# ishine/TTS-3

Measured on AMD Instinct MI355X. Metric: audio samples/sec + RTF, HiFiGAN-v1 22.05kHz 80-mel, batch 32 @ 1/2/4/8 GPU, higher is better.
Workload: dtype fp32 (power-of-2 scaled fp16 hi/lo split on fp16 MFMA, fp32 accumulate); 1 GPU; HiFiGAN-v1 22.05kHz inference, [32,80,1024] mel per GPU (replicate pad 5), fp32; model=HiFiGAN-v1 (hifigan_config.py generator_model_params), global_batch=32, seq_len=1024, parallelism=dp1 (utterance sharding; no collectives)

## Files before the change

### tts-3_amd/csrc/abi.cpp

```cpp
#include <cmath>
#include <cstdio>
#include <cstring>
#include <new>
#include <string>
#include <vector>

#include "fft_attn.hpp"
#include "forward_tts.hpp"
#include "glow.hpp"
#include "handoff.hpp"
#include "hifigan.hpp"
#include "mas.hpp"
#include "melgan.hpp"
#include "stft.hpp"
#include "text.hpp"
#include "vits.hpp"
#include "tts_mi355x.h"

namespace {
thread_local std::string g_last_error;

template <class F>
int guarded(F&& f) {
  try {
    g_last_error.clear();
    f();
    return TTS_OK;
  } catch (const tts::Error& e) {
    g_last_error = e.what();
    return e.code;
  } catch (const std::bad_alloc&) {
    g_last_error = "host allocation failed";
    return TTS_ERR_OOM;
  } catch (const std::exception& e) {
    g_last_error = e.what();
    return TTS_ERR_INVALID;
  } catch (...) {
    g_last_error = "unknown error";
    return TTS_ERR_INVALID;
  }
}

void export_records(const tts::Profiler& prof, TtsLaunchRecord* records, int max_records, int* n_records) {
  *n_records = (int)prof.recs.size();
  for (int i = 0; i < (int)prof.recs.size() && i < max_records && records; ++i) {
    const auto& r = prof.recs[i];
    std::memset(records[i].name, 0, sizeof(records[i].name));
    std::strncpy(records[i].name, r.name.c_str(), sizeof(records[i].name) - 1);
    records[i].flops = r.flops;
    records[i].bytes = r.bytes;
    float ms = 0.f;
    TTS_HIP_CHECK(hipEventElapsedTime(&ms, r.a, r.b));
    records[i].ms = ms;
  }
}

tts::DeviceBuffer to_device(const float* host, size_t n) {
  tts::DeviceBuffer b;
  int dev = 0;
  TTS_HIP_CHECK(hipGetDevice(&dev));
  b.grow(dev, n * sizeof(float), "operand");
  if (host && n) TTS_HIP_CHECK(hipMemcpy(b.as<>(), host, n * sizeof(float), hipMemcpyHostToDevice));
  return b;
}

template <class Cfg, class Validate, class Shapes>
int num_weights(const Cfg* cfg, Validate validate, Shapes shapes) {
  int n = -1;
  int st = guarded([&] {
    TTS_REQUIRE(cfg, 1, "NULL cfg");
    validate(*cfg);
    n = (int)shapes(*cfg).size();
  });
  return st == TTS_OK ? n : -st;
}

template <class Cfg, class Validate, class Shapes>
int64_t weight_numel(const Cfg* cfg, int idx, Validate validate, Shapes shapes) {
  int64_t n = -1;
  guarded([&] {
    TTS_REQUIRE(cfg, 1, "NULL cfg");
    validate(*cfg);
    auto s = shapes(*cfg);
    TTS_REQUIRE(idx >= 0 && idx < (int)s.size(), 1, "weight index out of range");
    n = s[idx];
  });
  return n;
}

template <class T, class Cfg, class W>
int create(const Cfg* cfg, const W* host_weights, int device, void** handle) {
  return guarded([&] {
    TTS_REQUIRE(cfg && host_weights && handle, 1, "NULL argument");
    *handle = nullptr;
    *handle = new T(*cfg, host_weights, device);
  });
}

template <class T>
int destroy(void* handle) {
  return guarded([&] { delete static_cast<T*>(handle); });
}

template <class T, class Body>
int profiled(void* handle, void* hip_stream, TtsLaunchRecord* records, int max_records, int* n_records, Body body) {
  return guarded([&] {
    TTS_REQUIRE(handle && n_records, 1, "NULL argument");
    auto* h = static_cast<T*>(handle);
    auto s = static_cast<hipStream_t>(hip_stream);
    tts::Profiler prof;
    {
      tts::DeviceGuard g(h->device());
      body(*h, s, &prof);
      TTS_HIP_CHECK(hipStreamSynchronize(s));
    }
    export_records(prof, records, max_records, n_records);
  });
}
}

extern "C" {

const char* tts_last_error(void) { return g_last_error.c_str(); }
int tts_abi_version(void) { return 115; }
const char* tts_build_target(void) { return "gfx950"; }

int tts_hifigan_num_weights(const TtsHifiganCfg* cfg) {
  return num_weights(cfg, tts::hifigan_validate, tts::hifigan_weight_shapes);
}

int64_t tts_hifigan_weight_numel(const TtsHifiganCfg* cfg, int idx) {
  return weight_numel(cfg, idx, tts::hifigan_validate, tts::hifigan_weight_shapes);
}

int tts_hifigan_create(const TtsHifiganCfg* cfg, const float* const* host_weights, int device,
                       void** handle) {
  return create<tts::Hifigan>(cfg, host_weights, device, handle);
}

int tts_hifigan_destroy(void* handle) { return destroy<tts::Hifigan>(handle); }

int64_t tts_hifigan_output_length(const void* handle, int T, int pad) {
  if (!handle) return -1;
  return static_cast<const tts::Hifigan*>(handle)->out_len(T, pad);
}

int64_t tts_hifigan_workspace_bytes(const void* handle, int B, int T, int pad) {
  if (!handle) return -1;
  return static_cast<const tts::Hifigan*>(handle)->workspace_bytes(B, T, pad);
}

int tts_hifigan_reserve(void* handle, int B, int T, int pad) {
  return guarded([&] {
    TTS_REQUIRE(handle, 1, "NULL handle");
    TTS_REQUIRE(B >= 1 && T >= 1 && pad >= 0, 1, "bad shape");
    static_cast<tts::Hifigan*>(handle)->reserve(B, T, pad);
  });
}

int tts_hifigan_forward(void* handle, const float* d_mel, int B, int C, int T, int pad,
                        const float* d_g, float* d_wav, void* hip_stream) {
  return guarded([&] {
    TTS_REQUIRE(handle, 1, "NULL handle");
    static_cast<tts::Hifigan*>(handle)->forward(d_mel, B, C, T, pad, d_g, d_wav,
                                                static_cast<hipStream_t>(hip_stream), nullptr);
  });
}

int tts_hifigan_forward_profiled(void* handle, const float* d_mel, int B, int C, int T, int pad,
                                 const float* d_g, float* d_wav, void* hip_stream,
                                 TtsLaunchRecord* records, int max_records, int* n_records) {
  auto body = [&](tts::Hifigan& h, hipStream_t s, tts::Profiler* prof) {
    h.forward(d_mel, B, C, T, pad, d_g, d_wav, s, prof);
  };
  return profiled<tts::Hifigan>(handle, hip_stream, records, max_records, n_records, body);
}

static std::vector<int64_t> glow_encoder_shapes(const TtsGlowEncoderCfg& c) {
  return tts::glow_encoder_weight_shapes(c);
}

int tts_glow_encoder_num_weights(const TtsGlowEncoderCfg* cfg) {
  return num_weights(cfg, tts::glow_encoder_validate, glow_encoder_shapes);
}

int64_t tts_glow_encoder_weight_numel(const TtsGlowEncoderCfg* cfg, int idx) {
  return weight_numel(cfg, idx, tts::glow_encoder_validate, glow_encoder_shapes);
}

int tts_glow_encoder_create(const TtsGlowEncoderCfg* cfg, const float* const* host_weights, int device,
                            void** handle) {
  return create<tts::GlowEncoder>(cfg, host_weights, device, handle);
}

int tts_glow_encoder_destroy(void* handle) { return destroy<tts::GlowEncoder>(handle); }

int tts_glow_encoder_forward(void* handle, const int64_t* d_tokens, const int64_t* d_lengths, const float* d_g,
                             int B, int T, float* d_x_m, float* d_x_logs, float* d_logw, float* d_x_mask,
                             void* hip_stream) {
  return guarded([&] {
    TTS_REQUIRE(handle, 1, "NULL handle");
    static_cast<tts::GlowEncoder*>(handle)->forward(d_tokens, d_lengths, d_g, B, T, d_x_m, d_x_logs, d_logw,
                                                    d_x_mask, static_cast<hipStream_t>(hip_stream));
  });
}

int tts_glow_encoder_forward_profiled(void* handle, const int64_t* d_tokens, const int64_t* d_lengths,
                                      const float* d_g, int B, int T, float* d_x_m, float* d_x_logs, float* d_logw,
                                      float* d_x_mask,
                                      void* hip_stream, TtsLaunchRecord* records, int max_records,
                                      int* n_records) {
  auto body = [&](tts::GlowEncoder& h, hipStream_t s, tts::Profiler* prof) {
    h.forward(d_tokens, d_lengths, d_g, B, T, d_x_m, d_x_logs, d_logw, d_x_mask, s, prof);
  };
  return profiled<tts::GlowEncoder>(handle, hip_stream, records, max_records, n_records, body);
}

int tts_glow_durations(const float* d_logw, const float* d_x_mask, int B, int T_x, float length_scale,
                       float* d_w_ceil, int64_t* d_y_lengths, float* d_o_attn_dur, void* hip_stream) {
  return guarded([&] {
    TTS_REQUIRE(d_logw && d_x_mask && d_w_ceil && d_y_lengths, 1, "NULL argument");
    TTS_REQUIRE(B >= 1 && T_x >= 1, 1, "batch and token count must be >= 1");
    tts::launch_durations(d_logw, d_x_mask, d_w_ceil, d_y_lengths, d_o_attn_dur, B, T_x, length_scale,
                          static_cast<hipStream_t>(hip_stream));
    TTS_HIP_CHECK(hipGetLastError());
  });
}

int tts_glow_expand(const float* d_w_ceil, const float* d_x_mask, const int64_t* d_y_lengths,
                    const float* d_o_mean, const float* d_o_log_scale, const float* d_noise, float noise_scale,
                    int B, int C, int T_x, int T_y, float* d_z, float* d_y_mask, float* d_y_mean,
                    float* d_y_log_scale, float* d_attn, void* hip_stream) {
  return guarded([&] {
    TTS_REQUIRE(d_w_ceil && d_x_mask && d_y_lengths && d_o_mean && d_z && d_y_mask, 1, "NULL argument");
    TTS_REQUIRE(B >= 1 && C >= 1 && T_x >= 1 && T_y >= 1, 1, "bad expand shape");
    tts::ExpandArgs a{};
    a.w_ceil = d_w_ceil; a.x_mask = d_x_mask; a.y_len = d_y_lengths; a.o_mean = d_o_mean;
    a.o_log_scale = d_o_log_scale; a.noise = d_noise; a.noise_scale = noise_scale;
    a.C = C; a.T_x = T_x; a.T_y = T_y;
    a.z = d_z; a.y_mask = d_y_mask; a.y_mean = d_y_mean; a.y_log_scale = d_y_log_scale; a.attn = d_attn;
    tts::launch_expand(a, B, static_cast<hipStream_t>(hip_stream));
    TTS_HIP_CHECK(hipGetLastError());
  });
}

int tts_glow_mas_logp(const float* d_o_mean, const float* d_o_log_scale, const float* d_z, int B, int C, int T_en,
                      int T_de, float* d_logp, void* hip_stream) {
  return guarded([&] {
    TTS_REQUIRE(d_o_mean && d_z && d_logp, 1, "NULL argument");
    TTS_REQUIRE(B >= 1 && C >= 1 && T_en >= 1 && T_de >= 1, 1, "bad logp shape");
    tts::launch_mas_logp(d_o_mean, d_o_log_scale, d_z, B, C, T_en, T_de, d_logp, static_cast<hipStream_t>(hip_stream));
  });
}

int64_t tts_maximum_path_workspace_bytes(int B, int T_en, int T_de) {
  if (B < 1 || T_en < 1 || T_de < 1 || T_en > tts::MAS_MAX_TEN) return -1;
  return (int64_t)tts::mas_workspace_bytes(B, T_en, T_de);
}

int tts_maximum_path(const float* d_value, const float* d_mask, const int64_t* d_t_x, const int64_t* d_t_y, int B,
                     int T_en, int T_de, void* d_workspace, float* d_path, float* d_durations, float* d_log_dur,
                     void* hip_stream) {
  return guarded([&] {
    TTS_REQUIRE(d_value && d_t_x && d_t_y && d_workspace, 1, "NULL argument");
    TTS_REQUIRE(B >= 1 && T_en >= 1 && T_de >= 1, 1, "bad maximum_path shape");
    tts::launch_maximum_path(d_value, d_mask, d_t_x, d_t_y, B, T_en, T_de, d_workspace, d_path, d_durations, d_log_dur,
                             static_cast<hipStream_t>(hip_stream));
  });
}

int tts_vits_text_encoder_num_weights(const TtsVitsTextEncoderCfg* cfg) {
  return num_weights(cfg, tts::vits_text_encoder_validate, tts::vits_text_encoder_weight_shapes);
}

int64_t tts_vits_text_encoder_weight_numel(const TtsVitsTextEncoderCfg* cfg, int idx) {
  return weight_numel(cfg, idx, tts::vits_text_encoder_validate, tts::vits_text_encoder_weight_shapes);
}

int tts_vits_text_encoder_create(const TtsVitsTextEncoderCfg* cfg, const float* const* host_weights, int device,
                                 void** handle) {
  return create<tts::VitsTextEncoder>(cfg, host_weights, device, handle);
}

int tts_vits_text_encoder_destroy(void* handle) { return destroy<tts::VitsTextEncoder>(handle); }

int tts_vits_text_encoder_forward(void* handle, const int64_t* d_tokens, const int64_t* d_lengths,
                                  const float* d_lang_emb, int B, int T, float* d_x, float* d_m, float* d_logs,
                                  float* d_x_mask, void* hip_stream) {
  return guarded([&] {
    TTS_REQUIRE(handle, 1, "NULL handle");
    static_cast<tts::VitsTextEncoder*>(handle)->forward(d_tokens, d_lengths, d_lang_emb, B, T, d_x, d_m, d_logs,
                                                        d_x_mask, static_cast<hipStream_t>(hip_stream));
  });
}

int tts_vits_text_encoder_forward_profiled(void* handle, const int64_t* d_tokens, const int64_t* d_lengths,
                                           const float* d_lang_emb, int B, int T, float* d_x, float* d_m,
                                           float* d_logs, float* d_x_mask, void* hip_stream,
                                           TtsLaunchRecord* records, int max_records, int* n_records) {
  auto body = [&](tts::VitsTextEncoder& h, hipStream_t s, tts::Profiler* prof) {
    h.forward(d_tokens, d_lengths, d_lang_emb, B, T, d_x, d_m, d_logs, d_x_mask, s, prof);
  };
  return profiled<tts::VitsTextEncoder>(handle, hip_stream, records, max_records, n_records, body);
}

int tts_vits_sdp_num_weights(const TtsVitsSdpCfg* cfg) {
  return num_weights(cfg, tts::vits_sdp_validate, tts::vits_sdp_weight_shapes);
}

int64_t tts_vits_sdp_weight_numel(const TtsVitsSdpCfg* cfg, int idx) {
  return weight_numel(cfg, idx, tts::vits_sdp_validate, tts::vits_sdp_weight_shapes);
}

int tts_vits_sdp_create(const TtsVitsSdpCfg* cfg, const float* const* host_weights, int device, void** handle) {
  return create<tts::VitsSdp>(cfg, host_weights, device, handle);
}

int tts_vits_sdp_destroy(void* handle) { return destroy<tts::VitsSdp>(handle); }

int tts_vits_sdp_reverse(void* handle, const float* d_x, const float* d_x_mask, const float* d_g,
                         const float* d_lang_emb, const float* d_noise, float noise_scale, int B, int T,
                         float* d_logw, void* hip_stream) {
  return guarded([&] {
    TTS_REQUIRE(handle, 1, "NULL handle");
    static_cast<tts::VitsSdp*>(handle)->reverse(d_x, d_x_mask, d_g, d_lang_emb, d_noise, noise_scale, B, T, d_logw,
                                                static_cast<hipStream_t>(hip_stream));
  });
}

int tts_vits_sdp_reverse_profiled(void* handle, const float* d_x, const float* d_x_mask, const float* d_g,
                                  const float* d_lang_emb, const float* d_noise, float noise_scale, int B, int T,
                                  float* d_logw, void* hip_stream, TtsLaunchRecord* records, int max_records,
                                  int* n_records) {
  auto body = [&](tts::VitsSdp& h, hipStream_t s, tts::Profiler* prof) {
    h.reverse(d_x, d_x_mask, d_g, d_lang_emb, d_noise, noise_scale, B, T, d_logw, s, prof);
  };
  return profiled<tts::VitsSdp>(handle, hip_stream, records, max_records, n_records, body);
}

int tts_vits_dp_num_weights(const TtsVitsDpCfg* cfg) {
  return num_weights(cfg, tts::vits_dp_validate, tts::vits_dp_weight_shapes);
}

int64_t tts_vits_dp_weight_numel(const TtsVitsDpCfg* cfg, int idx) {
  return weight_numel(cfg, idx, tts::vits_dp_validate, tts::vits_dp_weight_shapes);
}

int tts_vits_dp_create(const TtsVitsDpCfg* cfg, const float* const* host_weights, int device, void** handle) {
  return create<tts::VitsDp>(cfg, host_weights, device, handle);
}

int tts_vits_dp_destroy(void* handle) { return destroy<tts::VitsDp>(handle); }

int tts_vits_dp_forward(void* handle, const float* d_x, const float* d_x_mask, const float* d_g,
                        const float* d_lang_emb, int B, int T, float* d_logw, void* hip_stream) {
  return guarded([&] {
    TTS_REQUIRE(handle, 1, "NULL handle");
    static_cast<tts::VitsDp*>(handle)->forward(d_x, d_x_mask, d_g, d_lang_emb, B, T, d_logw,
                                               static_cast<hipStream_t>(hip_stream));
  });
}

int tts_vits_dp_forward_profiled(void* handle, const float* d_x, const float* d_x_mask, const float* d_g,
                                 const float* d_lang_emb, int B, int T, float* d_logw, void* hip_stream,
                                 TtsLaunchRecord* records, int max_records, int* n_records) {
  auto body = [&](tts::VitsDp& h, hipStream_t s, tts::Profiler* prof) {
    h.forward(d_x, d_x_mask, d_g, d_lang_emb, B, T, d_logw, s, prof);
  };
  return profiled<tts::VitsDp>(handle, hip_stream, records, max_records, n_records, body);
}

int tts_vits_durations(const float* d_logw, const float* d_x_mask, int B, int T_x, float length_scale,
                       float* d_w_ceil, int64_t* d_y_lengths, void* hip_stream) {
  return guarded([&] {
    TTS_REQUIRE(d_logw && d_x_mask && d_w_ceil && d_y_lengths, 1, "NULL argument");
    TTS_REQUIRE(B >= 1 && T_x >= 1, 1, "batch and token count must be >= 1");
    tts::launch_durations(d_logw, d_x_mask, d_w_ceil, d_y_lengths, nullptr, B, T_x, length_scale,
                          static_cast<hipStream_t>(hip_stream), 1);
    TTS_HIP_CHECK(hipGetLastError());
  });
}

int tts_vits_expand(const float* d_w_ceil, const float* d_x_mask, const int64_t* d_y_lengths, const float* d_m_p,
                    const float* d_logs_p, const float* d_noise, float noise_scale, int B, int C, int T_x, int T_y,
                    float* d_z_p, float* d_y_mask, float* d_m_p_out, float* d_logs_p_out, float* d_attn,
                    void* hip_stream) {
  return guarded([&] {
    TTS_REQUIRE(d_w_ceil && d_x_mask && d_y_lengths && d_m_p && d_logs_p && d_z_p && d_y_mask, 1, "NULL argument");
    TTS_REQUIRE(B >= 1 && C >= 1 && T_x >= 1 && T_y >= 1, 1, "bad expand shape");
    tts::ExpandArgs a{};
    a.w_ceil = d_w_ceil; a.x_mask = d_x_mask; a.y_len = d_y_lengths; a.o_mean = d_m_p;
    a.o_log_scale = d_logs_p; a.noise = d_noise; a.noise_scale = noise_scale;
    a.C = C; a.T_x = T_x; a.T_y = T_y;
    a.z = d_z_p; a.y_mask = d_y_mask; a.y_mean = d_m_p_out; a.y_log_scale = d_logs_p_out; a.attn = d_attn;
    a.vits = 1;
    tts::launch_expand(a, B, static_cast<hipStream_t>(hip_stream));
    TTS_HIP_CHECK(hipGetLastError());
  });
}

int tts_vits_durations_given(const float* d_durations, int64_t dur_bstride, int B, int T_x, float* d_w_ceil,
                             int64_t* d_y_lengths, void* hip_stream) {
  return guarded([&] {
    TTS_REQUIRE(d_durations && d_w_ceil && d_y_lengths, 1, "NULL argument");
    TTS_REQUIRE(B >= 1 && T_x >= 1 && (dur_bstride == 0 || dur_bstride >= T_x), 1, "bad durations shape");
    tts::launch_given_durations(d_durations, dur_bstride, d_w_ceil, d_y_lengths, B, T_x,
                                static_cast<hipStream_t>(hip_stream));
  });
}

int tts_vits_mask_slice(const float* d_z, const float* d_y_mask, int B, int C, int T, int T_out, float* d_out,
                        void* hip_stream) {
  return guarded([&] {
    TTS_REQUIRE(d_z && d_y_mask && d_out, 1, "NULL argument");
    tts::launch_mask_slice(d_z, d_y_mask, d_out, B, C, T, T_out, static_cast<hipStream_t>(hip_stream));
  });
}

int tts_vits_upsample_z(const float* d_z, const int64_t* d_y_lengths, int B, int C, int T, double factor, int T2,
                        float* d_z2, float* d_y_mask2, void* hip_stream) {
  return guarded([&] {
    TTS_REQUIRE(d_z && d_z2 && (d_y_lengths || !d_y_mask2), 1, "NULL argument");
    TTS_REQUIRE(factor > 0.0 && T2 == (int)std::floor((double)T * factor), 1,
                "upsample_z: T2 must be floor(T * factor) (F.interpolate's output length)");
    tts::launch_upsample_z(d_z, d_y_lengths, d_z2, d_y_mask2, B, C, T, T2, factor,
                           static_cast<hipStream_t>(hip_stream));
  });
}

int tts_embedding_rows(const float* d_table, int num, int dim, const int64_t* d_ids, int64_t id_stride, int B,
                       float* d_out, void* hip_stream) {
  return guarded([&] {
    TTS_REQUIRE(d_table && d_ids && d_out, 1, "NULL argument");
    tts::launch_embedding_rows(d_table, d_ids, id_stride, d_out, B, dim, num, static_cast<hipStream_t>(hip_stream));
  });
}

int tts_l2_normalize_rows(const float* d_in, int B, int C, float* d_out, void* hip_stream) {
  return guarded([&] {
    TTS_REQUIRE(d_in && d_out, 1, "NULL argument");
    tts::launch_l2_normalize(d_in, d_out, B, C, static_cast<hipStream_t>(hip_stream));
  });
}

namespace {
tts::AudioNormDev to_dev(const TtsAudioNormCfg* c) {
  tts::AudioNormDev d{};
  if (!c || !c->signal_norm) return d;
  TTS_REQUIRE((c->d_mel_mean == nullptr) == (c->d_mel_scale == nullptr), 1,
              "mel_scaler needs both d_mel_mean and d_mel_scale");
  d.signal_norm = 1;
  d.symmetric_norm = c->symmetric_norm;
  d.clip_norm = c->clip_norm;
  d.max_norm = (float)c->max_norm;
  d.two_max_norm = (float)(2.0 * c->max_norm);
  d.min_level_db = (float)c->min_level_db;
  d.neg_min_level_db = (float)(-c->min_level_db);
  d.ref_level_db = (float)c->ref_level_db;
  d.mean = c->d_mel_mean;
  d.scale = c->d_mel_scale;
  return d;
}
}

int tts_mel_handoff(const float* d_in, int B, int T, int C, int time_major, const TtsAudioNormCfg* denorm,
                    const TtsAudioNormCfg* norm, int T_out, float src_scale, float* d_out, void* hip_stream) {
  return guarded([&] {
    TTS_REQUIRE(d_in && d_out, 1, "NULL argument");
    TTS_REQUIRE(B >= 1 && T >= 1 && C >= 1 && T_out >= 1, 1, "bad hand-off shape");
    TTS_REQUIRE(C <= 65535 && B <= 65535, 3, "hand-off: C and B must be <= 65535");
    tts::HandoffArgs a{};
    a.in = d_in; a.out = d_out; a.T = T; a.C = C; a.T_out = T_out; a.time_major = time_major ? 1 : 0;
    a.src_scale = src_scale;
    a.de = to_dev(denorm);
    a.no = to_dev(norm);
    tts::launch_handoff(a, B, static_cast<hipStream_t>(hip_stream));
    TTS_HIP_CHECK(hipGetLastError());
  });
}

int tts_wav_to_int16(const float* d_wav, int B, int64_t n, const int64_t* d_lengths, unsigned* d_scratch,
                     int16_t* d_out, void* hip_stream) {
  return guarded([&] {
    TTS_REQUIRE(d_wav && d_scratch && d_out, 1, "NULL argument");
    TTS_REQUIRE(B >= 1 && B <= 65535 && n >= 1, 1, "bad wav shape");
    tts::launch_wav_int16(d_wav, B, n, d_lengths, d_scratch, d_out, static_cast<hipStream_t>(hip_stream));
    TTS_HIP_CHECK(hipGetLastError());
  });
}

int tts_glow_decoder_num_weights(const TtsGlowDecoderCfg* cfg) {
  return num_weights(cfg, tts::glow_validate, tts::glow_weight_shapes);
}

int64_t tts_glow_decoder_weight_numel(const TtsGlowDecoderCfg* cfg, int idx) {
  return weight_numel(cfg, idx, tts::glow_validate, tts::glow_weight_shapes);
}

int tts_glow_decoder_create(const TtsGlowDecoderCfg* cfg, const float* const* host_weights,
                            int device, void** handle) {
  return create<tts::GlowDecoder>(cfg, host_weights, device, handle);
}

int tts_glow_decoder_destroy(void* handle) { return destroy<tts::GlowDecoder>(handle); }

int tts_glow_decoder_forward(void* handle, const float* d_x, const float* d_mask, const float* d_g, int B,
                             int C, int T, int reverse, float* d_y, float* d_logdet, void* hip_stream) {
  return guarded([&] {
    TTS_REQUIRE(handle, 1, "NULL handle");
    TTS_REQUIRE(reverse == 0 || reverse == 1, 1, "reverse must be 0 or 1");
    auto* h = static_cast<tts::GlowDecoder*>(handle);
    if (reverse) h->reverse(d_x, d_mask, d_g, B, C, T, d_y, static_cast<hipStream_t>(hip_stream));
    else h->forward(d_x, d_mask, d_g, B, C, T, d_y, d_logdet, static_cast<hipStream_t>(hip_stream));
  });
}

int tts_glow_decoder_forward_profiled(void* handle, const float* d_x, const float* d_mask, const float* d_g,
                                      int B, int C, int T, int reverse, float* d_y, float* d_logdet,
                                      void* hip_stream, TtsLaunchRecord* records, int max_records, int* n_records) {
  auto body = [&](tts::GlowDecoder& h, hipStream_t s, tts::Profiler* prof) {
    TTS_REQUIRE(reverse == 0 || reverse == 1, 1, "reverse must be 0 or 1");
    if (reverse) h.reverse(d_x, d_mask, d_g, B, C, T, d_y, s, prof);
    else h.forward(d_x, d_mask, d_g, B, C, T, d_y, d_logdet, s, prof);
  };
  return profiled<tts::GlowDecoder>(handle, hip_stream, records, max_records, n_records, body);
}

int tts_vits_flow_num_weights(const TtsVitsFlowCfg* cfg) {
  return num_weights(cfg, tts::vits_flow_validate, tts::vits_flow_weight_shapes);
}

int64_t tts_vits_flow_weight_numel(const TtsVitsFlowCfg* cfg, int idx) {
  return weight_numel(cfg, idx, tts::vits_flow_validate, tts::vits_flow_weight_shapes);
}

int tts_vits_flow_create(const TtsVitsFlowCfg* cfg, const float* const* host_weights, int device, void** handle) {
  return create<tts::VitsFlow>(cfg, host_weights, device, handle);
}

int tts_vits_flow_destroy(void* handle) { return destroy<tts::VitsFlow>(handle); }

int tts_vits_flow_forward(void* handle, const float* d_x, const float* d_mask, const float* d_g, int B, int C,
                          int T, int reverse, float* d_y, void* hip_stream) {
  return guarded([&] {
    TTS_REQUIRE(handle, 1, "NULL handle");
    TTS_REQUIRE(reverse == 0 || reverse == 1, 1, "reverse must be 0 or 1");
    auto* h = static_cast<tts::VitsFlow*>(handle);
    if (reverse) h->reverse(d_x, d_mask, d_g, B, C, T, d_y, static_cast<hipStream_t>(hip_stream));
    else h->forward(d_x, d_mask, d_g, B, C, T, d_y, static_cast<hipStream_t>(hip_stream));
  });
}

int tts_vits_flow_forward_profiled(void* handle, const float* d_x, const float* d_mask, const float* d_g, int B,
                                   int C, int T, int reverse, float* d_y, void* hip_stream,
                                   TtsLaunchRecord* records, int max_records, int* n_records) {
  auto body = [&](tts::VitsFlow& h, hipStream_t s, tts::Profiler* prof) {
    TTS_REQUIRE(reverse == 0 || reverse == 1, 1, "reverse must be 0 or 1");
    if (reverse) h.reverse(d_x, d_mask, d_g, B, C, T, d_y, s, prof);
    else h.forward(d_x, d_mask, d_g, B, C, T, d_y, s, prof);
  };
  return profiled<tts::VitsFlow>(handle, hip_stream, records, max_records, n_records, body);
}

int tts_vits_posterior_num_weights(const TtsVitsPosteriorCfg* cfg) {
  return num_weights(cfg, tts::vits_posterior_validate, tts::vits_posterior_weight_shapes);
}

int64_t tts_vits_posterior_weight_numel(const TtsVitsPosteriorCfg* cfg, int idx) {
  return weight_numel(cfg, idx, tts::vits_posterior_validate, tts::vits_posterior_weight_shapes);
}

int tts_vits_posterior_create(const TtsVitsPosteriorCfg* cfg, const float* const* host_weights, int device,
                              void** handle) {
  return create<tts::VitsPosterior>(cfg, host_weights, device, handle);
}

int tts_vits_posterior_destroy(void* handle) { return destroy<tts::VitsPosterior>(handle); }

int tts_vits_posterior_forward(void* handle, const float* d_x, const float* d_mask, const float* d_g,
                               const float* d_eps, int B, int C, int T, float* d_z, float* d_m, float* d_logs,
                               void* hip_stream) {
  return guarded([&] {
    TTS_REQUIRE(handle, 1, "NULL handle");
    static_cast<tts::VitsPosterior*>(handle)->forward(d_x, d_mask, d_g, d_eps, B, C, T, d_z, d_m, d_logs,
                                                      static_cast<hipStream_t>(hip_stream));
  });
}

int tts_vits_posterior_forward_profiled(void* handle, const float* d_x, const float* d_mask, const float* d_g,
                                        const float* d_eps, int B, int C, int T, float* d_z, float* d_m,
                                        float* d_logs, void* hip_stream, TtsLaunchRecord* records,
                                        int max_records, int* n_records) {
  auto body = [&](tts::VitsPosterior& h, hipStream_t s, tts::Profiler* prof) {
    h.forward(d_x, d_mask, d_g, d_eps, B, C, T, d_z, d_m, d_logs, s, prof);
  };
  return profiled<tts::VitsPosterior>(handle, hip_stream, records, max_records, n_records, body);
}

int tts_stft_create(const TtsStftCfg* cfg, const float* h_window, int device, void** handle) {
  return create<tts::Stft>(cfg, h_window, device, handle);
}

int tts_stft_destroy(void* handle) { return destroy<tts::Stft>(handle); }

int tts_stft_num_frames(const TtsStftCfg* cfg, int64_t N) {
  int n = -1;
  int st = guarded([&] {
    TTS_REQUIRE(cfg, 1, "NULL cfg");
    n = tts::stft_num_frames(*cfg, N);
  });
  return st == TTS_OK ? n : -st;
}

int tts_stft_forward(void* handle, const float* d_wav, int B, int64_t N, int64_t wav_bstride, float* d_spec,
                     void* hip_stream) {
  return guarded([&] {
    TTS_REQUIRE(handle, 1, "NULL handle");
    static_cast<tts::Stft*>(handle)->forward(d_wav, B, N, wav_bstride, d_spec, static_cast<hipStream_t>(hip_stream));
  });
}

int tts_stft_forward_profiled(void* handle, const float* d_wav, int B, int64_t N, int64_t wav_bstride,
                              float* d_spec, void* hip_stream, TtsLaunchRecord* records, int max_records,
                              int* n_records) {
  auto body = [&](tts::Stft& h, hipStream_t s, tts::Profiler* prof) {
    h.forward(d_wav, B, N, wav_bstride, d_spec, s, prof);
  };
  return profiled<tts::Stft>(handle, hip_stream, records, max_records, n_records, body);
}

static void op_conv1d_impl(const TtsConv1dDesc* d, const float* d_x, const float* h_w, const float* h_b,
                           const float* d_res, float* d_y, float* d_z, int tile, int reps, float* ms,
                           void* hip_stream) {
  TTS_REQUIRE(d && d_x && h_w && h_b, 1, "NULL argument");
  TTS_REQUIRE(d->B >= 1 && d->Cin >= 1 && d->Cout >= 1 && d->Tin >= 1 && d->K >= 1 && d->dil >= 1, 1,
              "bad conv1d shape");
  TTS_REQUIRE((d->K % 2) == 1, 3, "conv1d: only odd kernel sizes ('same' padding)");
  TTS_REQUIRE(d->zmode >= 0 && d->zmode <= 3, 1, "bad zmode");
  TTS_REQUIRE(d->zmode == 0 ? d_y != nullptr : d_z != nullptr, 1, "missing output pointer");
  const int mode = d->math_mode;
  TTS_REQUIRE(mode >= tts::MATH_FP32 && mode <= tts::MATH_LAST, 1, "unknown math_mode");
  if (tile < 0) tile = tts::conv_tile_for(mode, d->Cout, d->K, d->Cin, d->dil, d_res != nullptr);
  const tts::ConvTile t = tts::conv_tile(mode, tile);
  std::vector<float> packed(tts::packed_conv_numel(mode, d->Cout, d->Cin, d->K, t));
  const int w_exp = tts::pack_conv(mode, h_w, d->Cout, d->Cin, d->K, t, packed.data());
  std::vector<float> bias((size_t)tts::ceil_div(d->Cout, t.BM) * t.BM, 0.f);
  std::memcpy(bias.data(), h_b, sizeof(float) * d->Cout);
  const tts::DeviceBuffer w = to_device(packed.data(), packed.size()), b = to_device(bias.data(), bias.size());
  tts::Conv1dArgs a{};
  a.x = d_x; a.w = w.as<>(); a.bias = b.as<>(); a.res = d_res; a.y = d_y; a.z = d_z; a.cvec = nullptr;
  a.Cin = d->Cin; a.Cout = d->Cout; a.Tin = d->Tin; a.Tout = d->Tin + 2 * d->rep_pad;
  a.dil = d->dil; a.pad = d->dil * (d->K - 1) / 2; a.rep_pad = d->rep_pad;
  a.n_chunks = tts::ceil_div(d->Cin, t.CK);
  a.in_slope = d->in_slope; a.out_slope = d->out_slope; a.zmode = d->zmode; a.zdiv = d->zdiv;
  a.w_exp = w_exp;
  auto s = static_cast<hipStream_t>(hip_stream);
  tts::DeviceBuffer slots;
  if (mode == tts::MATH_FP32_F16X3) {
    slots = to_device(nullptr, (size_t)d->B * 64);
    TTS_HIP_CHECK(hipMemsetAsync(slots.as<>(), 0, (size_t)d->B * 64 * sizeof(float), s));
    tts::launch_amax(d_x, (int64_t)d->Cin * d->Tin, d->B, slots.as<unsigned>(), s);
    a.amax_in = slots.as<unsigned>();
  }
  if (reps <= 0) {
    tts::launch_conv(mode, a, d->B, d->K, tile, s);
  } else {
    tts::launch_conv(mode, a, d->B, d->K, tile, s);
    hipEvent_t e0, e1;
    TTS_HIP_CHECK(hipEventCreate(&e0));
    TTS_HIP_CHECK(hipEventCreate(&e1));
    TTS_HIP_CHECK(hipEventRecord(e0, s));
    for (int r = 0; r < reps; ++r) tts::launch_conv(mode, a, d->B, d->K, tile, s);
    TTS_HIP_CHECK(hipEventRecord(e1, s));
    TTS_HIP_CHECK(hipEventSynchronize(e1));
    float total = 0.f;
    TTS_HIP_CHECK(hipEventElapsedTime(&total, e0, e1));
    (void)hipEventDestroy(e0);
    (void)hipEventDestroy(e1);
    if (ms) *ms = total / reps;
  }
  TTS_HIP_CHECK(hipStreamSynchronize(s));
}

int tts_op_conv1d(const TtsConv1dDesc* d, const float* d_x, const float* h_w, const float* h_b,
                  const float* d_res, float* d_y, float* d_z, void* hip_stream) {
  return guarded([&] { op_conv1d_impl(d, d_x, h_w, h_b, d_res, d_y, d_z, -1, 0, nullptr, hip_stream); });
}

int tts_op_conv1d_bench(const TtsConv1dDesc* d, const float* d_x, const float* h_w, const float* h_b,
                        const float* d_res, float* d_y, float* d_z, int tile, int reps, float* ms,
                        void* hip_stream) {
  return guarded([&] { op_conv1d_impl(d, d_x, h_w, h_b, d_res, d_y, d_z, tile, reps, ms, hip_stream); });
}

int tts_op_conv1d_num_tiles(int math_mode) {
  if (math_mode < tts::MATH_FP32 || math_mode > tts::MATH_LAST) {
    g_last_error = "unknown math_mode";
    return -TTS_ERR_INVALID;
  }
  return tts::conv_num_tiles(math_mode);
}

int tts_op_conv_transpose1d(const float* d_x, int B, int Cin, int Tin, const float* h_w,
                            const float* h_b, int Cout, int K, int stride, float in_slope,
                            int math_mode, float* d_y, void* hip_stream) {
  return guarded([&] {
    TTS_REQUIRE(d_x && h_w && h_b && d_y, 1, "NULL argument");
    TTS_REQUIRE(B >= 1 && Cin >= 1 && Cout >= 1 && Tin >= 1, 1, "bad conv_transpose1d shape");
    TTS_REQUIRE(K == 2 * stride, 3, "conv_transpose1d: requires kernel_size == 2*stride");
    TTS_REQUIRE(stride == 2 || stride == 4 || stride == 8, 3, "conv_transpose1d: stride must be 2, 4 or 8");
    TTS_REQUIRE(math_mode >= tts::MATH_FP32 && math_mode <= tts::MATH_LAST, 1, "unknown math_mode");
    auto s = static_cast<hipStream_t>(hip_stream);
    if (tts::is_split_mode(math_mode)) {
      const int tile = tts::conv_tile_for(math_mode, stride * Cout, 2, Cin, 1, false);
      const tts::ConvTile t = tts::conv_tile(math_mode, tile);
      std::vector<float> packed(tts::packed_conv_numel(math_mode, stride * Cout, Cin, 2, t));
      const int w_exp = tts::pack_convT_split(math_mode, h_w, Cin, Cout, stride, t, packed.data());
      std::vector<float> bias((size_t)tts::ceil_div(stride * Cout, t.BM) * t.BM, 0.f);
      for (int co = 0; co < Cout; ++co)
        for (int ph = 0; ph < stride; ++ph) bias[(size_t)co * stride + ph] = h_b[co];
      const tts::DeviceBuffer w = to_device(packed.data(), packed.size()), b = to_device(bias.data(), bias.size());
      tts::Conv1dArgs a{};
      a.x = d_x; a.w = w.as<>(); a.bias = b.as<>(); a.y = d_y;
      a.Cin = Cin; a.Cout = stride * Cout; a.Tin = Tin; a.Tout = Tin + 1;
      a.dil = 1; a.pad = 1; a.n_chunks = tts::ceil_div(Cin, t.CK);
      a.in_slope = in_slope; a.out_slope = 1.f; a.zdiv = 1.f; a.w_exp = w_exp; a.ups = stride;
      tts::DeviceBuffer slots;
      if (math_mode == tts::MATH_FP32_F16X3) {
        slots = to_device(nullptr, (size_t)B * 64);
        TTS_HIP_CHECK(hipMemsetAsync(slots.as<>(), 0, (size_t)B * 64 * sizeof(float), s));
        tts::launch_amax(d_x, (int64_t)Cin * Tin, B, slots.as<unsigned>(), s);
        a.amax_in = slots.as<unsigned>();
      }
      tts::launch_conv(math_mode, a, B, 2, tile, s);
      TTS_HIP_CHECK(hipStreamSynchronize(s));
      return;
    }
    const int tile = tts::convT_tile_for(Cout, stride);
    const tts::ConvTile t = tts::convT_tile(tile, stride);
    std::vector<float> packed(tts::packed_convT_numel(Cin, Cout, stride, t));
    tts::pack_convT(h_w, Cin, Cout, stride, t, packed.data());
    std::vector<float> bias((size_t)tts::ceil_div(Cout, t.BM) * t.BM, 0.f);
    std::memcpy(bias.data(), h_b, sizeof(float) * Cout);
    const tts::DeviceBuffer w = to_device(packed.data(), packed.size()), b = to_device(bias.data(), bias.size());
    tts::ConvTArgs a{};
    a.x = d_x; a.w = w.as<>(); a.bias = b.as<>(); a.y = d_y;
    a.Cin = Cin; a.Cout = Cout; a.Tin = Tin; a.n_chunks = tts::ceil_div(Cin, t.CK); a.in_slope = in_slope;
    tts::launch_convT(a, B, stride, tile, s);
    TTS_HIP_CHECK(hipStreamSynchronize(s));
  });
}

int tts_op_conv_post(const float* d_z, int B, int Cin, int T, const float* h_w, const float* h_b,
                     float in_slope, float* d_y, void* hip_stream) {
  return guarded([&] {
    TTS_REQUIRE(d_z && h_w && d_y, 1, "NULL argument");
    TTS_REQUIRE(B >= 1 && Cin >= 1 && T >= 1, 1, "bad conv_post shape");
    const tts::DeviceBuffer w = to_device(h_w, (size_t)Cin * 7);
    tts::PostArgs a{};
    a.z = d_z; a.w = w.as<>(); a.bias = h_b ? h_b[0] : 0.f; a.y = d_y; a.Cin = Cin; a.T = T; a.in_slope = in_slope;
    auto s = static_cast<hipStream_t>(hip_stream);
    tts::launch_conv_post(a, B, s);
    TTS_HIP_CHECK(hipStreamSynchronize(s));
  });
}

int tts_melgan_num_weights(const TtsMelganCfg* cfg) {
  return num_weights(cfg, [](const TtsMelganCfg&) {}, tts::melgan_weight_shapes);
}

int64_t tts_melgan_weight_numel(const TtsMelganCfg* cfg, int idx) {
  return weight_numel(cfg, idx, [](const TtsMelganCfg&) {}, tts::melgan_weight_shapes);
}

int tts_melgan_create(const TtsMelganCfg* cfg, const float* const* host_weights, int device, void** handle) {
  return create<tts::Melgan>(cfg, host_weights, device, handle);
}

int tts_melgan_destroy(void* handle) { return destroy<tts::Melgan>(handle); }

int64_t tts_melgan_output_length(const void* handle, int T, int pad, int synth) {
  int64_t n = -1;
  int st = guarded([&] {
    TTS_REQUIRE(handle, 1, "NULL handle");
    n = static_cast<const tts::Melgan*>(handle)->out_len(T, pad, synth);
  });
  return st == TTS_OK ? n : -st;
}

int64_t tts_melgan_workspace_bytes(const void* handle, int B, int T, int pad) {
  int64_t n = -1;
  int st = guarded([&] {
    TTS_REQUIRE(handle, 1, "NULL handle");
    n = static_cast<const tts::Melgan*>(handle)->workspace_bytes(B, T, pad);
  });
  return st == TTS_OK ? n : -st;
}

int tts_melgan_forward(void* handle, const float* d_mel, int B, int C, int T, int pad, int synth, float* d_out,
                       void* hip_stream) {
  return guarded([&] {
    TTS_REQUIRE(handle, 1, "NULL handle");
    static_cast<tts::Melgan*>(handle)->forward(d_mel, B, C, T, pad, synth, d_out, static_cast<hipStream_t>(hip_stream));
  });
}

int tts_melgan_forward_profiled(void* handle, const float* d_mel, int B, int C, int T, int pad, int synth,
                                float* d_out, void* hip_stream, TtsLaunchRecord* records, int max_records,
                                int* n_records) {
  auto body = [&](tts::Melgan& h, hipStream_t s, tts::Profiler* prof) {
    h.forward(d_mel, B, C, T, pad, synth, d_out, s, prof);
  };
  return profiled<tts::Melgan>(handle, hip_stream, records, max_records, n_records, body);
}

int tts_op_melgan_block(const float* d_x, int B, int C, int L, int dilation, const float* h_w1, const float* h_b1,
                        const float* h_w2, const float* h_b2, const float* h_ws, const float* h_bs, int math_mode,
                        float* d_out, void* hip_stream) {
  return guarded([&] {
    TTS_REQUIRE(d_x && h_w1 && h_b1 && h_w2 && h_b2 && h_ws && h_bs && d_out, 1, "NULL argument");
    TTS_REQUIRE(math_mode >= tts::MATH_FP32 && math_mode <= tts::MATH_LAST, 1, "unknown math_mode");
    TTS_REQUIRE(B >= 1 && C >= 1 && L >= 1 && dilation >= 1, 1, "bad melgan block shape");
    const int mode = math_mode == tts::MATH_BF16 ? tts::MATH_BF16 : tts::MATH_FP32_X6;
    TTS_REQUIRE(C <= tts::kMelganMaxC, 3, "melgan block: channels must lie in [1, 256]");
    const int64_t n1 = tts::packed_melgan_a1_numel16(mode, C), n2 = tts::packed_melgan_a2_numel16(mode, C);
    const size_t nb = (size_t)32 * tts::melgan_mblocks(C);
    std::vector<float> a1((size_t)n1 / 2), a2((size_t)n2 / 2), bias1(nb), bias2(nb);
    tts::pack_melgan_block(mode, h_w1, h_b1, h_w2, h_b2, h_ws, h_bs, C, reinterpret_cast<uint16_t*>(a1.data()),
                           reinterpret_cast<uint16_t*>(a2.data()), bias1.data(), bias2.data());
    const tts::DeviceBuffer da1 = to_device(a1.data(), a1.size()), da2 = to_device(a2.data(), a2.size());
    const tts::DeviceBuffer db1 = to_device(bias1.data(), nb), db2 = to_device(bias2.data(), nb);
    tts::MelganBlockArgs a{};
    a.x = d_x; a.y = d_out; a.a1 = da1.as<>(); a.a2 = da2.as<>(); a.bias1 = db1.as<>(); a.bias2 = db2.as<>();
    a.a1_bytes = (unsigned)(n1 * 2); a.a2_bytes = (unsigned)(n2 * 2);
    a.C = C; a.L = L; a.dil = dilation;
    auto s = static_cast<hipStream_t>(hip_stream);
    tts::launch_melgan_block(mode, a, B, s);
    TTS_HIP_CHECK(hipStreamSynchronize(s));
  });
}

int tts_op_melgan_block_tile(void) { return tts::kMelganBlockTile; }

int tts_pqmf_synthesis(const float* d_x, int B, int bands, int L, const float* d_G, int taps, float* d_out,
                       void* hip_stream) {
  return guarded([&] {
    tts::launch_pqmf_synthesis(d_x, B, bands, L, d_G, taps, d_out, static_cast<hipStream_t>(hip_stream));
  });
}

int tts_op_mha(const float* d_qkv, const int64_t* d_key_lengths, int B, int E, int heads, int T, int math_mode,
               float* d_out, void* hip_stream) {
  return guarded([&] {
    TTS_REQUIRE(d_qkv && d_out, 1, "NULL argument");
    TTS_REQUIRE(math_mode >= tts::MATH_FP32 && math_mode <= tts::MATH_LAST, 1, "unknown math_mode");
    const int mode = math_mode == tts::MATH_BF16 ? tts::MATH_BF16 : tts::MATH_FP32_X6;
    tts::launch_mha(mode, d_qkv, d_key_lengths, d_out, B, E, heads, T, static_cast<hipStream_t>(hip_stream));
  });
}

int tts_op_mha_tile(void) { return tts::kMhaTile; }

int tts_forward_tts_num_weights(const TtsForwardTtsCfg* cfg) {
  return num_weights(cfg, tts::forward_tts_validate, tts::forward_tts_weight_shapes);
}

int64_t tts_forward_tts_weight_numel(const TtsForwardTtsCfg* cfg, int idx) {
  return weight_numel(cfg, idx, tts::forward_tts_validate, tts::forward_tts_weight_shapes);
}

int tts_forward_tts_create(const TtsForwardTtsCfg* cfg, const float* const* host_weights, int device, void** handle) {
  return create<tts::ForwardTts>(cfg, host_weights, device, handle);
}

int tts_forward_tts_destroy(void* handle) { return destroy<tts::ForwardTts>(handle); }

int tts_forward_tts_encode(void* handle, const int64_t* d_tokens, const int64_t* d_x_lengths,
                           const int64_t* d_speaker_ids, const float* d_given_durations, int B, int T_en,
                           float length_scale, float* d_o_en, float* d_x_mask, float* d_durations_log, float* d_pitch,
                           float* d_durations, int64_t* d_y_lengths, void* hip_stream) {
  return guarded([&] {
    TTS_REQUIRE(handle, 1, "NULL handle");
    static_cast<tts::ForwardTts*>(handle)->encode(d_tokens, d_x_lengths, d_speaker_ids, d_given_durations, B, T_en,
                                                  length_scale, d_o_en, d_x_mask, d_durations_log, d_pitch,
                                                  d_durations, d_y_lengths, static_cast<hipStream_t>(hip_stream));
  });
}

int tts_forward_tts_encode_profiled(void* handle, const int64_t* d_tokens, const int64_t* d_x_lengths,
                                    const int64_t* d_speaker_ids, const float* d_given_durations, int B, int T_en,
                                    float length_scale, float* d_o_en, float* d_x_mask, float* d_durations_log,
                                    float* d_pitch, float* d_durations, int64_t* d_y_lengths, void* hip_stream,
                                    TtsLaunchRecord* records, int max_records, int* n_records) {
  auto body = [&](tts::ForwardTts& h, hipStream_t s, tts::Profiler* prof) {
    h.encode(d_tokens, d_x_lengths, d_speaker_ids, d_given_durations, B, T_en, length_scale, d_o_en, d_x_mask,
             d_durations_log, d_pitch, d_durations, d_y_lengths, s, prof);
  };
  return profiled<tts::ForwardTts>(handle, hip_stream, records, max_records, n_records, body);
}

int tts_forward_tts_decode(void* handle, const float* d_o_en, const float* d_durations, const float* d_x_mask,
                           const int64_t* d_y_lengths, int B, int T_en, int T_de, int mask_decoder_keys, float* d_out,
                           float* d_attn, float* d_y_mask, void* hip_stream) {
  return guarded([&] {
    TTS_REQUIRE(handle, 1, "NULL handle");
    static_cast<tts::ForwardTts*>(handle)->decode(d_o_en, d_durations, d_x_mask, d_y_lengths, B, T_en, T_de,
                                                  mask_decoder_keys != 0, d_out, d_attn, d_y_mask,
                                                  static_cast<hipStream_t>(hip_stream));
  });
}

int tts_forward_tts_decode_profiled(void* handle, const float* d_o_en, const float* d_durations, const float* d_x_mask,
                                    const int64_t* d_y_lengths, int B, int T_en, int T_de, int mask_decoder_keys,
                                    float* d_out, float* d_attn, float* d_y_mask, void* hip_stream,
                                    TtsLaunchRecord* records, int max_records, int* n_records) {
  auto body = [&](tts::ForwardTts& h, hipStream_t s, tts::Profiler* prof) {
    h.decode(d_o_en, d_durations, d_x_mask, d_y_lengths, B, T_en, T_de, mask_decoder_keys != 0, d_out, d_attn,
             d_y_mask, s, prof);
  };
  return profiled<tts::ForwardTts>(handle, hip_stream, records, max_records, n_records, body);
}

int tts_forward_tts_block(void* handle, int decoder, const float* d_x, const int64_t* d_key_lengths, int B, int T,
                          float* d_y, void* hip_stream) {
  return guarded([&] {
    TTS_REQUIRE(handle, 1, "NULL handle");
    static_cast<tts::ForwardTts*>(handle)->block(decoder != 0, d_x, d_key_lengths, B, T, d_y,
                                                 static_cast<hipStream_t>(hip_stream));
  });
}

}
```

### tts-3_amd/csrc/common.hpp

```cpp
#pragma once

#include <hip/hip_runtime.h>

#include <cstdint>
#include <stdexcept>
#include <string>

namespace tts {

struct Error : std::runtime_error {
  int code;
  Error(int c, const std::string& m) : std::runtime_error(m), code(c) {}
};

#define TTS_HIP_CHECK(expr)                                                               \
  do {                                                                                    \
    hipError_t _e = (expr);                                                               \
    if (_e != hipSuccess)                                                                 \
      throw ::tts::Error(2, std::string(#expr) + " failed: " + hipGetErrorString(_e));    \
  } while (0)

#define TTS_REQUIRE(cond, code, msg)                    \
  do {                                                  \
    if (!(cond)) throw ::tts::Error((code), (msg));     \
  } while (0)

typedef float f32x4 __attribute__((ext_vector_type(4)));
typedef float f32x16 __attribute__((ext_vector_type(16)));

__device__ __forceinline__ float lrelu(float x, float slope) { return x > 0.f ? x : x * slope; }

constexpr int kPlaneXB16 = 1;
constexpr int kPlaneYB16 = 2;

struct Conv1dArgs {
  const float* x;
  const float* w;
  const float* bias;
  const float* res;
  float* y;
  float* z;
  const float* cvec;
  const float* mask;
  int64_t x_bstride;
  int Cin, Cout, Tin, Tout;
  int dil, pad, rep_pad;
  int n_chunks;
  float in_slope, out_slope;
  int zmode;
  float zdiv;
  const unsigned* amax_in;
  unsigned* amax_out;
  int w_exp;
  int ups;
  int64_t o_bstride;
  int64_t cvec_bstride;
  int mask_res;
  int wn_rows;
  int gate;
  int planes;
};

constexpr int kSplitGateTile = 20;
constexpr int kSplitWinoTile = 21;
bool wino_supported(int mode, int Cout, int Cin, int K, int dil);
bool wino_enabled();
void launch_wino(int mode, const Conv1dArgs& a, int B, int K, hipStream_t s);
inline int gate_row_order(int rho, int H) {
  const int j = rho / 128, r = rho % 128;
  return r < 64 ? 64 * j + r : H + 64 * j + (r - 64);
}

struct ResPairArgs {
  Conv1dArgs c1;
  Conv1dArgs c2;
  const float* post_w;
  float post_bias;
  float post_slope;
  float* wav;
};
bool resblock_pair_supported(int mode, int C, int K, int dil);
bool resblock_pair_preferred(int mode, int C, int K, int dil);
bool resblock_pair128(int mode, int C, int K);
void launch_resblock_pair(int mode, const ResPairArgs& a, int B, int K, int C, hipStream_t s);

struct ResBlock3Args {
  const float* x;
  const unsigned* amax_in;
  const float* w[6];
  const float* bias[6];
  int w_exp[6];
  int dil[3];
  float* z;
  int zmode;
  float zdiv;
  unsigned* amax_out;
  int T;
  int planes;
};
bool resblock3_supported(int mode, int C, int K, const int* dil);
void launch_resblock3(int mode, const ResBlock3Args& a, int B, int C, int K, hipStream_t s);
bool resblock2_supported(int mode, int C, int K, const int* dil);
bool resblock2_preferred(int mode, int C, int K, const int* dil);
int resblock2_geo64(int mode);
void launch_resblock2(int mode, const ResBlock3Args& a, int B, int C, int K, int geo64, hipStream_t s);

struct ConvTile {
  int BM, BN, TM, TN, CK;
  int PD = 1;
  int WINO = 0;
};

struct ConvTArgs {
  const float* x;
  const float* w;
  const float* bias;
  float* y;
  int Cin, Cout, Tin;
  int n_chunks;
  float in_slope;
  unsigned* amax_out;
  const float* cvec;
};

struct PostArgs {
  const float* z;
  const float* w;
  float bias;
  float* y;
  int Cin, T;
  float in_slope;
  int z_b16;
};

int conv1d_tile_for(int Cout, int K, int Cin, int dil, bool res);
ConvTile conv1d_tile(int idx);
int conv1d_num_tiles();
void launch_conv1d(const Conv1dArgs& a, int B, int K, int tile_idx, hipStream_t s);
int convT_tile_for(int Cout, int U);
ConvTile convT_tile(int idx, int U);
void launch_convT(const ConvTArgs& a, int B, int U, int tile_idx, hipStream_t s);
void launch_conv_post(const PostArgs& a, int B, hipStream_t s);
void launch_mel_window(const float* mel, int B, int C, int T, int pad, int64_t w0, int W, float* out, hipStream_t s);
void launch_cond_vec(const float* g, const float* Wc, const float* bc, float* cvec, int B, int Cc,
                     int C0, hipStream_t s);

constexpr int MATH_FP32 = 0;
constexpr int MATH_FP32_X6 = 1;
constexpr int MATH_FP32_F16X3 = 2;
constexpr int MATH_BF16 = 3;
constexpr int MATH_LAST = MATH_BF16;

ConvTile conv1d_split_tile(int mode, int idx);
int conv1d_split_num_tiles(int mode);
int conv1d_split_tile_for(int mode, int Cout, int K, int Cin, int dil, bool res);
void launch_conv1d_split(int mode, const Conv1dArgs& a, int B, int K, int tile_idx, hipStream_t s);
bool convT_res_supported(int mode, const Conv1dArgs& a);
void launch_convT_res(int mode, const Conv1dArgs& a, int B, hipStream_t s);
void launch_amax(const float* x, int64_t n, int B, unsigned* slots, hipStream_t s, int64_t stride = 0);

inline bool is_split_mode(int mode) { return mode == MATH_FP32_X6 || mode == MATH_FP32_F16X3 || mode == MATH_BF16; }
inline ConvTile conv_tile(int mode, int idx) {
  return is_split_mode(mode) ? conv1d_split_tile(mode, idx) : conv1d_tile(idx);
}
inline int conv_tile_for(int mode, int Cout, int K, int Cin, int dil, bool res) {
  return is_split_mode(mode) ? conv1d_split_tile_for(mode, Cout, K, Cin, dil, res)
                             : conv1d_tile_for(Cout, K, Cin, dil, res);
}
inline int conv_num_tiles(int mode) { return is_split_mode(mode) ? conv1d_split_num_tiles(mode) : conv1d_num_tiles(); }
inline void launch_conv(int mode, const Conv1dArgs& a, int B, int K, int tile, hipStream_t s) {
  if (is_split_mode(mode)) launch_conv1d_split(mode, a, B, K, tile, s);
  else launch_conv1d(a, B, K, tile, s);
}

void pack_conv1d(const float* w, int Cout, int Cin, int K, const ConvTile& t, float* out);
int64_t packed_conv1d_numel(int Cout, int Cin, int K, const ConvTile& t);
void pack_convT(const float* w, int Cin, int Cout, int U, const ConvTile& t, float* out);
int64_t packed_convT_numel(int Cin, int Cout, int U, const ConvTile& t);
__host__ __device__ constexpr int quad_pos(int q) { return q == 1 ? 2 : (q == 2 ? 1 : q); }
int pack_conv1d_split(int mode, const float* w, int Cout, int Cin, int K, const ConvTile& t, float* out,
                      bool quad_perm = true);
int64_t packed_conv1d_split_numel(int mode, int Cout, int Cin, int K, const ConvTile& t);
int pack_convT_split(int mode, const float* w, int Cin, int Cout, int U, const ConvTile& t, float* out);
int pack_conv1d_wino(int mode, const float* w, int Cout, int Cin, int K, const ConvTile& t, float* out);
inline int64_t packed_conv_numel(int mode, int Cout, int Cin, int K, const ConvTile& t) {
  if (t.WINO) return packed_conv1d_split_numel(mode, Cout, Cin, 7 * ((K + 3) / 4), t);
  return is_split_mode(mode) ? packed_conv1d_split_numel(mode, Cout, Cin, K, t) : packed_conv1d_numel(Cout, Cin, K, t);
}
inline int pack_conv(int mode, const float* w, int Cout, int Cin, int K, const ConvTile& t, float* out) {
  if (t.WINO) return pack_conv1d_wino(mode, w, Cout, Cin, K, t, out);
  if (is_split_mode(mode)) return pack_conv1d_split(mode, w, Cout, Cin, K, t, out);
  pack_conv1d(w, Cout, Cin, K, t, out);
  return 0;
}

inline int ceil_div(int a, int b) { return (a + b - 1) / b; }

}
```

### tts-3_amd/csrc/conv_device.hpp

```cpp
#pragma once

#include "common.hpp"

namespace tts {

typedef __amdgpu_buffer_rsrc_t rsrc_t;
typedef unsigned u32x4_t __attribute__((ext_vector_type(4)));
typedef unsigned u32x2_t __attribute__((ext_vector_type(2)));
typedef float f32x2 __attribute__((ext_vector_type(2)));
constexpr unsigned OOB_OFF = 0x80000000u;

#ifndef ACT_ABLATE
#define ACT_ABLATE 0
#endif
__device__ __forceinline__ unsigned act_range(unsigned bytes) {
  return (ACT_ABLATE && bytes != 0xFFFFFFFFu && bytes > 65536u) ? 65536u : bytes;
}
__device__ __forceinline__ rsrc_t make_rsrc(const void* p, unsigned bytes) {
  return __builtin_amdgcn_make_buffer_rsrc(const_cast<void*>(p), (short)0, (int)act_range(bytes), 0x00020000);
}
__device__ __forceinline__ float bload(rsrc_t r, unsigned voff, unsigned soff) {
  return __builtin_bit_cast(float, __builtin_amdgcn_raw_buffer_load_b32(r, (int)voff, (int)soff, 0));
}
__device__ __forceinline__ f32x4 bload4(rsrc_t r, unsigned voff, unsigned soff) {
  return __builtin_bit_cast(f32x4, __builtin_amdgcn_raw_buffer_load_b128(r, (int)voff, (int)soff, 0));
}
#ifndef TTS_ST_POL
#define TTS_ST_POL 0
#endif
#ifndef TTS_LDX_POL
#define TTS_LDX_POL 0
#endif
template <int POL = TTS_LDX_POL>
__device__ __forceinline__ float bload_x(rsrc_t r, unsigned voff, unsigned soff) {
  return __builtin_bit_cast(float, __builtin_amdgcn_raw_buffer_load_b32(r, (int)voff, (int)soff, POL));
}
__device__ __forceinline__ void bstore(rsrc_t r, float v, unsigned voff, unsigned soff) {
  __builtin_amdgcn_raw_buffer_store_b32(__builtin_bit_cast(unsigned, v), r, (int)voff, (int)soff, TTS_ST_POL);
}
__device__ __forceinline__ unsigned short f32_to_bf16_bits(float v) {
  return __builtin_bit_cast(unsigned short, (__bf16)v);
}
__device__ __forceinline__ float bf16_bits_to_f32(unsigned b) { return __builtin_bit_cast(float, b << 16); }
__device__ __forceinline__ float bf16_round(float v) { return bf16_bits_to_f32(f32_to_bf16_bits(v)); }
template <bool B16>
struct PlaneT {
  static constexpr unsigned ES = 4u;
  __device__ static __forceinline__ float ld(rsrc_t r, unsigned voff, unsigned soff) { return bload(r, voff, soff); }
  __device__ static __forceinline__ void st(rsrc_t r, float v, unsigned voff, unsigned soff) { bstore(r, v, voff, soff); }
  __device__ static __forceinline__ float rt(float v) { return v; }
};
template <>
struct PlaneT<true> {
  static constexpr unsigned ES = 2u;
  __device__ static __forceinline__ float ld(rsrc_t r, unsigned voff, unsigned soff) {
    return bf16_bits_to_f32((unsigned)__builtin_amdgcn_raw_buffer_load_b16(r, (int)voff, (int)soff, 0));
  }
  __device__ static __forceinline__ void st(rsrc_t r, float v, unsigned voff, unsigned soff) {
    __builtin_amdgcn_raw_buffer_store_b16(f32_to_bf16_bits(v), r, (int)voff, (int)soff, TTS_ST_POL);
  }
  __device__ static __forceinline__ float rt(float v) { return bf16_round(v); }
};
template <bool B16>
__device__ __forceinline__ const void* plane_at(const float* p, size_t e) {
  return reinterpret_cast<const char*>(p) + e * PlaneT<B16>::ES;
}
template <bool B16>
__device__ __forceinline__ f32x4 pload4(rsrc_t r, unsigned voff, unsigned soff) {
  if constexpr (B16) {
    const u32x2_t w = __builtin_bit_cast(u32x2_t, __builtin_amdgcn_raw_buffer_load_b64(r, (int)voff, (int)soff, 0));
    return f32x4{bf16_bits_to_f32(w[0] & 0xffffu), bf16_bits_to_f32(w[0] >> 16), bf16_bits_to_f32(w[1] & 0xffffu),
                 bf16_bits_to_f32(w[1] >> 16)};
  } else {
    return bload4(r, voff, soff);
  }
}
template <bool B16>
__device__ __forceinline__ void pstore4(rsrc_t r, f32x4 v, unsigned voff, unsigned soff) {
  if constexpr (B16) {
    const u32x2_t w = {(unsigned)f32_to_bf16_bits(v[0]) | ((unsigned)f32_to_bf16_bits(v[1]) << 16),
                       (unsigned)f32_to_bf16_bits(v[2]) | ((unsigned)f32_to_bf16_bits(v[3]) << 16)};
    __builtin_amdgcn_raw_buffer_store_b64(__builtin_bit_cast(u32x2_t, w), r, (int)voff, (int)soff, TTS_ST_POL);
  } else {
    __builtin_amdgcn_raw_buffer_store_b128(__builtin_bit_cast(u32x4_t, v), r, (int)voff, (int)soff, TTS_ST_POL);
  }
}

__device__ __forceinline__ void lds_dma_b128(const void* base, unsigned bytes, unsigned voff, const void* lds) {
  const unsigned long long p = reinterpret_cast<unsigned long long>(base);
  const u32x4_t d = {(unsigned)__builtin_amdgcn_readfirstlane((int)(unsigned)p),
                     (unsigned)__builtin_amdgcn_readfirstlane((int)((unsigned)(p >> 32) & 0xffffu)),
                     (unsigned)__builtin_amdgcn_readfirstlane((int)act_range(bytes)), 0x00020000u};
  const unsigned m =
      (unsigned)__builtin_amdgcn_readfirstlane((int)(unsigned)(unsigned long)(__attribute__((address_space(3))) const void*)lds);
#pragma clang diagnostic push
#pragma clang diagnostic ignored "-Winline-asm"
  asm volatile("s_mov_b32 m0, %2\n\ts_nop 0\n\tbuffer_load_dwordx4 %0, %1, 0 offen lds" ::"v"(voff), "s"(d), "s"(m)
               : "memory", "m0");
#pragma clang diagnostic pop
}

__device__ __forceinline__ void l2_touch_dma(const void* base, unsigned bytes, unsigned voff, const void* lds) {
  const unsigned long long p = reinterpret_cast<unsigned long long>(base);
  const u32x4_t d = {(unsigned)__builtin_amdgcn_readfirstlane((int)(unsigned)p),
                     (unsigned)__builtin_amdgcn_readfirstlane((int)((unsigned)(p >> 32) & 0xffffu)),
                     (unsigned)__builtin_amdgcn_readfirstlane((int)act_range(bytes)), 0x00020000u};
  const unsigned m =
      (unsigned)__builtin_amdgcn_readfirstlane((int)(unsigned)(unsigned long)(__attribute__((address_space(3))) const void*)lds);
#pragma clang diagnostic push
#pragma clang diagnostic ignored "-Winline-asm"
  asm volatile("s_mov_b32 m0, %2\n\ts_nop 0\n\tbuffer_load_dword %0, %1, 0 offen lds" ::"v"(voff), "s"(d), "s"(m)
               : "memory", "m0");
#pragma clang diagnostic pop
}

__device__ __forceinline__ float lrelu2(float x, float slope) { return fmaxf(x, x * slope); }
__device__ __forceinline__ int wave_id() { return __builtin_amdgcn_readfirstlane((int)(threadIdx.x >> 6)); }

__device__ __forceinline__ int xlds_off(int g, int r, int q, int xrows) {
  return (g * xrows + r) * 8 + 4 * (q ^ ((r >> 3) & 1));
}

template <int CTRL, int ROWS>
__device__ __forceinline__ float dpp_max_step(float v) {
  const int o = __builtin_amdgcn_update_dpp(__builtin_bit_cast(int, v), __builtin_bit_cast(int, v), CTRL, ROWS, 0xF, false);
  return fmaxf(v, __builtin_bit_cast(float, o));
}
__device__ __forceinline__ float wave_max(float v) {
  v = dpp_max_step<0xB1, 0xF>(v);
  v = dpp_max_step<0x4E, 0xF>(v);
  v = dpp_max_step<0x141, 0xF>(v);
  v = dpp_max_step<0x140, 0xF>(v);
  v = dpp_max_step<0x142, 0xA>(v);
  v = dpp_max_step<0x143, 0xC>(v);
  return __builtin_bit_cast(float, __builtin_amdgcn_readlane(__builtin_bit_cast(int, v), 63));
}

__device__ __forceinline__ void publish_amax(unsigned* slots, int b, float v) {
  v = wave_max(v);
  if ((threadIdx.x & 63) == 0) atomicMax(slots + (size_t)b * 64 + (blockIdx.x & 63), __float_as_uint(v));
}

__device__ __forceinline__ void publish_amax_block(unsigned* slots, int b, float v) {
  __shared__ float red[4];
  v = wave_max(v);
  if ((threadIdx.x & 63) == 0) red[threadIdx.x >> 6] = v;
  __syncthreads();
  if (threadIdx.x == 0)
    atomicMax(slots + (size_t)b * 64 + (blockIdx.x & 63),
              __float_as_uint(fmaxf(fmaxf(red[0], red[1]), fmaxf(red[2], red[3]))));
}

template <int TM, int TN, bool RES, int ZM, bool AMAX, bool YB = false>
__device__ __forceinline__ void conv_epilogue_impl(const Conv1dArgs& a, const f32x16 (&acc)[TM][TN], int b,
                                                   int tbase, int cobase, int lane, int tend,
                                                   const float* sbias, int sbase) {
  using PY = PlaneT<YB>;
  const int half = lane >> 5;
  const int l32 = lane & 31;
  const int Cout = a.Cout;
  const int Tout = a.Tout;
  const unsigned plane = (unsigned)Cout * (unsigned)Tout * PY::ES;
  const size_t item = (size_t)b * (a.o_bstride ? a.o_bstride : (int64_t)Cout * Tout);
  const rsrc_t rres = make_rsrc(RES ? plane_at<YB>(a.res, item) : a.bias, RES ? plane : 0u);
  const rsrc_t rz = make_rsrc(ZM >= 2 ? plane_at<YB>(a.z, item) : a.bias, ZM >= 2 ? plane : 0u);
  const rsrc_t rout = make_rsrc(plane_at<YB>(a.zmode == 0 ? a.y : a.z, item), plane);
  const rsrc_t rcv = make_rsrc(a.cvec ? a.cvec + (size_t)b * (a.cvec_bstride ? a.cvec_bstride : (int64_t)Cout) : a.bias,
                               a.cvec ? (unsigned)Cout * 4u : 0u);
  const rsrc_t rmask = make_rsrc(a.mask ? a.mask + (size_t)b * Tout : a.bias, a.mask ? (unsigned)Tout * 4u : 0u);
  const rsrc_t rbias = make_rsrc(a.bias, (unsigned)Cout * 4u);
  const bool has_mask = a.mask != nullptr;
  const bool mask_res = RES && a.mask_res && has_mask;
  const float oslope = a.out_slope;
  const float zdiv = a.zdiv;
  const unsigned rowb = (unsigned)Tout * PY::ES;
  float vmax = 0.f;
#pragma unroll
  for (int m = 0; m < TM; ++m) {
    float bv[16];
#pragma unroll
    for (int r = 0; r < 16; ++r) {
      const unsigned co = (unsigned)(cobase + m * 32 + (r & 3) + 8 * (r >> 2) + 4 * half);
      bv[r] = sbias ? sbias[(int)co - sbase] : bload(rbias, co * 4u, 0u) + bload(rcv, co * 4u, 0u);
    }
#pragma unroll
    for (int n = 0; n < TN; ++n) {
      const int t = tbase + n * 32 + l32;
      const int row0 = cobase + m * 32 + 4 * half;
      const bool tok = t < Tout && t < tend;
      const unsigned voff = tok ? ((unsigned)row0 * (unsigned)Tout + (unsigned)t) * PY::ES : OOB_OFF;
      const float mv = has_mask ? bload(rmask, (tok ? (unsigned)t * 4u : OOB_OFF), 0u) : 1.f;
      const float mv2 = mask_res ? mv : 1.f;
      unsigned vo[16];
      float rv[16], zv[16];
#pragma unroll
      for (int r = 0; r < 16; ++r) {
        vo[r] = voff + (unsigned)((r & 3) + 8 * (r >> 2)) * rowb;
        if (RES) rv[r] = PY::ld(rres, vo[r], 0u);
        if (ZM >= 2) zv[r] = PY::ld(rz, vo[r], 0u);
      }
      float vm = 0.f;
#pragma unroll
      for (int r = 0; r < 16; ++r) {
        float v = (acc[m][n][r] + bv[r]) * mv;
        v = lrelu2(v, oslope);
        if (RES) v = (v + rv[r]) * mv2;
        if (ZM == 2) v = zv[r] + v;
        if (ZM == 3) v = (zv[r] + v) / zdiv;
        if (AMAX) vm = fmaxf(vm, fabsf(v));
        PY::st(rout, v, vo[r], 0u);
      }
      if (AMAX && tok) vmax = fmaxf(vmax, vm);
    }
  }
  if (AMAX && a.amax_out) publish_amax(a.amax_out, b, vmax);
}

template <int TM, int TN, bool AMAX>
__device__ __forceinline__ void conv_epilogue_wn(const Conv1dArgs& args, const f32x16 (&acc)[TM][TN], int b,
                                                 int tbase, int cobase, int lane, const float* sbias, int sbase) {
  const Conv1dArgs a = args;
  const int half = lane >> 5;
  const int l32 = lane & 31;
  const int H = a.wn_rows;
  const int T = a.Tout;
  const size_t item = (size_t)b * H * T;
  const unsigned plane = (unsigned)H * (unsigned)T * 4u;
  const rsrc_t rh = make_rsrc(a.y + item, plane);
  const rsrc_t rsk = make_rsrc(a.z + item, plane);
  const rsrc_t rmask = make_rsrc(a.mask + (size_t)b * T, (unsigned)T * 4u);
  const rsrc_t rbias = make_rsrc(a.bias, (unsigned)(2 * H) * 4u);
  const bool first = a.zmode == 1;
  const unsigned rowb = (unsigned)T * 4u;
  float vmax = 0.f;
#pragma unroll
  for (int m = 0; m < TM; ++m) {
    const int rb0 = cobase + m * 32;
    if (rb0 >= 2 * H) continue;
    const bool hrow = rb0 < H;
    float bv[16];
#pragma unroll
    for (int r = 0; r < 16; ++r) {
      const unsigned co = (unsigned)(rb0 + (r & 3) + 8 * (r >> 2) + 4 * half);
      bv[r] = sbias ? sbias[(int)co - sbase] : bload(rbias, co * 4u, 0u);
    }
    const rsrc_t rdst = hrow ? rh : rsk;
    const int prow0 = (hrow ? rb0 : rb0 - H) + 4 * half;
#pragma unroll
    for (int n = 0; n < TN; ++n) {
      const int t = tbase + n * 32 + l32;
      const bool tok = t < T;
      const unsigned voff = tok ? ((unsigned)prow0 * (unsigned)T + (unsigned)t) * 4u : OOB_OFF;
      const float mv = bload(rmask, tok ? (unsigned)t * 4u : OOB_OFF, 0u);
      float ov[16];
#pragma unroll
      for (int r = 0; r < 16; ++r)
        ov[r] = (hrow || !first) ? bload(rdst, voff + (unsigned)((r & 3) + 8 * (r >> 2)) * rowb, 0u) : 0.f;
      float vm = 0.f;
#pragma unroll
      for (int r = 0; r < 16; ++r) {
        const float v = acc[m][n][r] + bv[r];
        float o;
        if (hrow) {
          o = (ov[r] + v) * mv;
          vm = fmaxf(vm, fabsf(o));
        } else {
          o = first ? v : ov[r] + v;
        }
        bstore(rdst, o, voff + (unsigned)((r & 3) + 8 * (r >> 2)) * rowb, 0u);
      }
      if (AMAX && tok) vmax = fmaxf(vmax, vm);
    }
  }
  if (AMAX && a.amax_out) publish_amax(a.amax_out, b, vmax);
}

template <int TM, int TN, bool AMAX, bool YB = false>
__device__ __forceinline__ void convT_epilogue(const Conv1dArgs& a, const f32x16 (&acc)[TM][TN], int b, int tbase,
                                               int cobase, int lane, const float* sb = nullptr,
                                               const float* scv = nullptr, int sbase = 0) {
  using PY = PlaneT<YB>;
  const int half = lane >> 5;
  const int l32 = lane & 31;
  const int U = a.ups;
  const int lgU = __builtin_ctz(U);
  const int Cr = a.Cout >> lgU;
  const int Tin = a.Tin;
  const int To = Tin << lgU;
  const unsigned plane = (unsigned)Cr * (unsigned)To * PY::ES;
  const rsrc_t rout = make_rsrc(plane_at<YB>(a.y, (size_t)b * Cr * To), plane);
  const rsrc_t rbias = make_rsrc(a.bias, (unsigned)a.Cout * 4u);
  const rsrc_t rcv = make_rsrc(a.cvec ? a.cvec + (size_t)b * Cr : a.bias, a.cvec ? (unsigned)Cr * 4u : 0u);
  float vmax = 0.f;
#pragma unroll
  for (int m = 0; m < TM; ++m) {
    float bv[16], cv[16];
#pragma unroll
    for (int r = 0; r < 16; ++r) {
      const unsigned rho = (unsigned)(cobase + m * 32 + (r & 3) + 8 * (r >> 2) + 4 * half);
      bv[r] = sb ? sb[(int)rho - sbase] : bload(rbias, rho * 4u, 0u);
      cv[r] = sb ? scv[(int)rho - sbase] : bload(rcv, (rho >> lgU) * 4u, 0u);
    }
#pragma unroll
    for (int n = 0; n < TN; ++n) {
      const int mm = tbase + n * 32 + l32;
      if (U == 8) {
#pragma unroll
        for (int i = 0; i < 4; ++i) {
          const int rho = cobase + m * 32 + 8 * i + 4 * half;
          const int co = rho >> 3;
          const int t0 = (mm << 3) + 4 * half - 4;
          const unsigned off = (t0 >= 0 && t0 < To) ? ((unsigned)co * (unsigned)To + (unsigned)t0) * PY::ES : OOB_OFF;
          f32x4 v;
#pragma unroll
          for (int j = 0; j < 4; ++j) {
            v[j] = (acc[m][n][4 * i + j] + bv[4 * i + j]) + cv[4 * i + j];
            if (AMAX && off != OOB_OFF && co < Cr) vmax = fmaxf(vmax, fabsf(v[j]));
          }
          pstore4<YB>(rout, v, off, 0u);
        }
        continue;
      }
      if (U == 2) {
#pragma unroll
        for (int r = 0; r < 16; r += 2) {
          const int rho = cobase + m * 32 + (r & 3) + 8 * (r >> 2) + 4 * half;
          const int co = rho >> 1;
          const int t = 2 * mm - 1;
          const float v0 = (acc[m][n][r] + bv[r]) + cv[r];
          const float v1 = (acc[m][n][r + 1] + bv[r + 1]) + cv[r + 1];
          const unsigned rowoff = (unsigned)co * (unsigned)To;
          if (!YB && t >= 0 && t + 1 < To) {
            if (AMAX && co < Cr) vmax = fmaxf(vmax, fmaxf(fabsf(v0), fabsf(v1)));
            const f32x2 v = {v0, v1};
            __builtin_amdgcn_raw_buffer_store_b64(__builtin_bit_cast(u32x2_t, v), rout, (int)((rowoff + (unsigned)t) * 4u), 0, TTS_ST_POL);
          } else {
            const unsigned off0 = (t >= 0 && t < To) ? (rowoff + (unsigned)t) * PY::ES : OOB_OFF;
            const unsigned off1 = (t + 1 >= 0 && t + 1 < To) ? (rowoff + (unsigned)t + 1u) * PY::ES : OOB_OFF;
            if (AMAX && co < Cr) {
              if (off0 != OOB_OFF) vmax = fmaxf(vmax, fabsf(v0));
              if (off1 != OOB_OFF) vmax = fmaxf(vmax, fabsf(v1));
            }
            PY::st(rout, v0, off0, 0u);
            PY::st(rout, v1, off1, 0u);
          }
        }
        continue;
      }
#pragma unroll
      for (int r = 0; r < 16; ++r) {
        const int rho = cobase + m * 32 + (r & 3) + 8 * (r >> 2) + 4 * half;
        const int co = rho >> lgU;
        const int t = (mm << lgU) + (rho & (U - 1)) - (U >> 1);
        const unsigned off = (t >= 0 && t < To) ? ((unsigned)co * (unsigned)To + (unsigned)t) * PY::ES : OOB_OFF;
        const float v = (acc[m][n][r] + bv[r]) + cv[r];
        if (AMAX && off != OOB_OFF && co < Cr) vmax = fmaxf(vmax, fabsf(v));
        PY::st(rout, v, off, 0u);
      }
    }
  }
  if (AMAX && a.amax_out) publish_amax(a.amax_out, b, vmax);
}

template <int TM, int TN, bool AMAX = false, bool YB = false>
__device__ __forceinline__ void conv_epilogue(const Conv1dArgs& args, const f32x16 (&acc)[TM][TN], int b,
                                              int tbase, int cobase, int lane, int tend = 0x7fffffff,
                                              const float* sbias = nullptr, int sbase = 0) {
  const Conv1dArgs a = args;
  const int zm = a.zmode <= 1 ? 0 : a.zmode;
#define TTS_EPI(RES, ZM) conv_epilogue_impl<TM, TN, RES, ZM, AMAX, YB>(a, acc, b, tbase, cobase, lane, tend, sbias, sbase)
  if (a.res) {
    if (zm == 0) TTS_EPI(true, 0);
    else if (zm == 2) TTS_EPI(true, 2);
    else TTS_EPI(true, 3);
  } else {
    if (zm == 0) TTS_EPI(false, 0);
    else if (zm == 2) TTS_EPI(false, 2);
    else TTS_EPI(false, 3);
  }
#undef TTS_EPI
}

}
```

### tts-3_amd/csrc/hifigan.cpp

```cpp
#include "hifigan.hpp"

#include <algorithm>
#include <cmath>
#include <cstdlib>
#include <vector>

namespace tts {

namespace {
bool valid_conv_k(int k) { return k == 1 || k == 3 || k == 5 || k == 7 || k == 11; }
}

std::vector<int64_t> hifigan_weight_shapes(const TtsHifiganCfg& c) {
  std::vector<int64_t> n;
  const int C0 = c.upsample_initial_channel;
  n.push_back((int64_t)C0 * c.in_channels * 7);
  n.push_back(C0);
  for (int i = 0; i < c.num_upsamples; ++i) {
    const int ci = C0 >> i, co = C0 >> (i + 1);
    n.push_back((int64_t)ci * co * c.upsample_kernel_sizes[i]);
    n.push_back(co);
  }
  for (int i = 0; i < c.num_upsamples; ++i) {
    const int ch = C0 >> (i + 1);
    for (int j = 0; j < c.num_kernels; ++j) {
      const int k = c.resblock_kernel_sizes[j];
      const int nconv = (c.resblock_type == 1) ? 6 : 2;
      for (int m = 0; m < nconv; ++m) {
        n.push_back((int64_t)ch * ch * k);
        n.push_back(ch);
      }
    }
  }
  const int cl = C0 >> c.num_upsamples;
  n.push_back((int64_t)c.out_channels * cl * 7);
  if (c.conv_post_bias) n.push_back(c.out_channels);
  if (c.cond_channels > 0) {
    n.push_back((int64_t)C0 * c.cond_channels);
    n.push_back(C0);
  }
  if (c.cond_in_each_up_layer) {
    for (int i = 0; i < c.num_upsamples; ++i) {
      n.push_back((int64_t)(C0 >> (i + 1)) * c.cond_channels);
      n.push_back(C0 >> (i + 1));
    }
  }
  return n;
}

void hifigan_validate(const TtsHifiganCfg& c) {
  TTS_REQUIRE(c.in_channels >= 1, 1, "in_channels must be >= 1");
  TTS_REQUIRE(c.out_channels == 1, 3, "only out_channels == 1 is implemented");
  TTS_REQUIRE(c.resblock_type == 1 || c.resblock_type == 2, 1, "resblock_type must be '1' or '2'");
  TTS_REQUIRE(c.num_kernels >= 1 && c.num_kernels <= TTS_MAX_KERNELS, 1, "bad num_kernels");
  TTS_REQUIRE(c.num_upsamples >= 1 && c.num_upsamples <= TTS_MAX_UPSAMPLES, 1, "bad num_upsamples");
  const int need_d = c.resblock_type == 1 ? 3 : 2;
  TTS_REQUIRE(c.num_dilations >= need_d && c.num_dilations <= TTS_MAX_DILATIONS, 1,
              "resblock_dilation_sizes too short for the resblock type");
  for (int j = 0; j < c.num_kernels; ++j) {
    TTS_REQUIRE(valid_conv_k(c.resblock_kernel_sizes[j]), 3,
                "resblock kernel size " + std::to_string(c.resblock_kernel_sizes[j]) +
                    " not implemented (1,3,5,7,11)");
    for (int m = 0; m < need_d; ++m) {
      const int d = c.resblock_dilation_sizes[j][m];
      TTS_REQUIRE(d >= 1 && (c.resblock_kernel_sizes[j] - 1) * d <= 96, 3,
                  "resblock (kernel_size-1)*dilation must be <= 96");
    }
  }
  int C = c.upsample_initial_channel;
  for (int i = 0; i < c.num_upsamples; ++i) {
    const int u = c.upsample_factors[i];
    TTS_REQUIRE(u == 2 || u == 4 || u == 8, 3, "upsample factor must be 2, 4 or 8");
    TTS_REQUIRE(c.upsample_kernel_sizes[i] == 2 * u, 3,
                "upsample kernel size must equal 2*factor (polyphase kernel)");
    C >>= 1;
    TTS_REQUIRE(C >= 1, 1, "upsample_initial_channel too small for the number of upsamples");
  }
  TTS_REQUIRE(c.inference_padding >= 0, 1, "inference_padding must be >= 0");
  TTS_REQUIRE(c.cond_channels >= 0, 1, "cond_channels must be >= 0");
  TTS_REQUIRE(!c.cond_in_each_up_layer || c.cond_channels > 0, 1, "cond_in_each_up_layer needs cond_channels > 0");
  TTS_REQUIRE(c.math_mode >= MATH_FP32 && c.math_mode <= MATH_LAST, 1, "unknown math_mode");
}

Hifigan::Hifigan(const TtsHifiganCfg& cfg, const float* const* hw, int device)
    : cfg_(cfg), device_(device) {
  hifigan_validate(cfg_);
  DeviceGuard g(device_);
  const auto shapes = hifigan_weight_shapes(cfg_);
  for (size_t i = 0; i < shapes.size(); ++i)
    TTS_REQUIRE(hw[i] != nullptr, 1, "weight pointer " + std::to_string(i) + " is NULL");

  const int C0 = cfg_.upsample_initial_channel;
  const int mode = cfg_.math_mode;
  const char* nf = std::getenv("TTS_MI355X_NO_PAIR_FUSION");
  const bool pair_fusion = !(nf && nf[0] == '1');
  const char* pf = std::getenv("TTS_MI355X_POST_FUSION");
  post_fusion_ = !(pf && pf[0] == '0');
  const char* ms = std::getenv("TTS_MI355X_MRF_STREAMS");
  nbs_ = ms ? std::max(1, std::min(std::atoi(ms), cfg.num_kernels)) : cfg.num_kernels;
  nbs_env_ = ms != nullptr;
  const char* sb = std::getenv("TTS_MI355X_SUBBATCH");
  n_lanes_ = sb ? std::max(1, std::min(std::atoi(sb), 8)) : 2;
  rb2_geo64_ = resblock2_geo64(mode);
  const char* bp = std::getenv("TTS_MI355X_BF16_PLANES");
  planes16_ = mode == MATH_BF16 && !(bp && bp[0] == '0') && cfg_.num_upsamples >= 1 &&
              cfg_.upsample_factors[0] % 8 == 0;
  size_t wi = 0;
  std::vector<std::pair<const float*, const float*>> src;
  auto add_conv = [&](int Cin, int Cout, int K, int dil, const char* fam, bool res, int lmode, bool pair128 = false) {
    ConvLayer L;
    L.Cin = Cin; L.Cout = Cout; L.K = K; L.dil = dil; L.pad = dil * (K - 1) / 2;
    L.mode = lmode;
    L.tile = conv_tile_for(lmode, Cout, K, Cin, dil, res);
    if (pair128) {
      L.tile = 7;
      L.name = std::string(fam) + "_k" + std::to_string(K) + "_c" + std::to_string(Cout);
      return L;
    }
    const bool wino_k3 = [] {
      const char* e = std::getenv("TTS_MI355X_WINO_K3");
      return e && e[0] == '1';
    }();
    const bool k_ok = K >= 7 || (K == 3 && Cout >= 256 && wino_k3);
    if (std::string(fam) == "mrf_conv" && k_ok && wino_enabled() && wino_supported(lmode, Cout, Cin, K, dil)) {
      L.tile = kSplitWinoTile;
      fam = "mrf_wino";
    }
    L.name = std::string(fam) + "_k" + std::to_string(K) + "_c" + std::to_string(Cout);
    return L;
  };

  pre_ = add_conv(cfg_.in_channels, C0, 7, 1, "conv_pre", false, mode);
  src.push_back({hw[wi], hw[wi + 1]}); wi += 2;
  for (int i = 0; i < cfg_.num_upsamples; ++i) {
    ConvTLayer L;
    L.Cin = C0 >> i; L.Cout = C0 >> (i + 1); L.U = cfg_.upsample_factors[i];
    L.mode = mode;
    L.tile = is_split_mode(mode) ? conv_tile_for(mode, L.U * L.Cout, 2, L.Cin, 1, false) : convT_tile_for(L.Cout, L.U);
    L.name = "ups_u" + std::to_string(L.U) + "_c" + std::to_string(L.Cout);
    ups_.push_back(L);
  }
  std::vector<std::pair<const float*, const float*>> usrc;
  for (int i = 0; i < cfg_.num_upsamples; ++i) { usrc.push_back({hw[wi], hw[wi + 1]}); wi += 2; }

  for (int i = 0; i < cfg_.num_upsamples; ++i) {
    const int ch = C0 >> (i + 1);
    for (int j = 0; j < cfg_.num_kernels; ++j) {
      const int k = cfg_.resblock_kernel_sizes[j];
      ResBlock rb;
      if (cfg_.resblock_type == 1) {
        const float* w1[3]; const float* b1[3]; const float* w2[3]; const float* b2[3];
        for (int m = 0; m < 3; ++m) { w1[m] = hw[wi]; b1[m] = hw[wi + 1]; wi += 2; }
        for (int m = 0; m < 3; ++m) { w2[m] = hw[wi]; b2[m] = hw[wi + 1]; wi += 2; }
        rb.fused = pair_fusion;
        const bool p128 = pair_fusion && resblock_pair128(mode, ch, k);
        bool tiles_ok = true;
        for (int m = 0; m < 3; ++m) {
          rb.convs.push_back(add_conv(ch, ch, k, cfg_.resblock_dilation_sizes[j][m], "mrf_conv", false, mode, p128));
          src.push_back({w1[m], b1[m]});
          rb.convs.push_back(add_conv(ch, ch, k, 1, "mrf_conv", true, mode, p128));
          src.push_back({w2[m], b2[m]});
          for (int c = 0; c < 2; ++c) {
            const ConvTile t = conv_tile(mode, rb.convs[2 * m + c].tile);
            const int dil = rb.convs[2 * m].dil;
            tiles_ok = tiles_ok && !t.WINO && t.CK % 16 == 0 && ch % t.CK == 0 && ch % t.BM == 0;
            rb.fused = rb.fused && !t.WINO && t.CK == 16 && ceil_div(ch, t.BM) * t.BM == ch &&
                       resblock_pair_preferred(mode, ch, k, dil);
          }
        }
        rb.fused3 = pair_fusion && tiles_ok;
      } else {
        bool tiles_ok = true;
        for (int m = 0; m < 2; ++m) {
          rb.convs.push_back(add_conv(ch, ch, k, cfg_.resblock_dilation_sizes[j][m], "mrf_conv", true, mode));
          src.push_back({hw[wi], hw[wi + 1]}); wi += 2;
          const ConvTile t = conv_tile(mode, rb.convs[m].tile);
          tiles_ok = tiles_ok && !t.WINO && t.CK % 16 == 0 && ch % t.CK == 0 && ch % t.BM == 0;
        }
        rb.fused2 = pair_fusion && tiles_ok;
      }
      if (rb.fused2 || (cfg_.resblock_type == 1 && rb.fused3)) {
        const int policy = [] {
          const char* e = std::getenv("TTS_MI355X_RESBLOCK3");
          if (!e) return 1 << 30;
          if (std::string(e) == "all") return 1 << 30;
          return std::atoi(e);
        }();
        const std::string wk = [] {
          const char* e = std::getenv("TTS_MI355X_RB1_WHOLE_K");
          return std::string(e ? e : "");
        }();
        const bool k_ok = k == 3 || wk.find(std::to_string(k)) != std::string::npos;
        if (cfg_.resblock_type == 1)
          rb.fused3 = ch <= policy && k_ok && resblock3_supported(mode, ch, k, cfg_.resblock_dilation_sizes[j]);
        else
          rb.fused2 = ch <= policy && resblock2_preferred(mode, ch, k, cfg_.resblock_dilation_sizes[j]);
      }
      res_.push_back(rb);
    }
  }
  const float* post_w = hw[wi]; wi += 1;
  post_bias_ = cfg_.conv_post_bias ? hw[wi][0] : 0.f;
  if (cfg_.conv_post_bias) wi += 1;

  HostArena arena;
  std::vector<ConvLayer*> convs;
  convs.push_back(&pre_);
  for (auto& rb : res_) for (auto& c : rb.convs) convs.push_back(&c);
  for (size_t i = 0; i < convs.size(); ++i) {
    ConvLayer& c = *convs[i];
    arena.put_conv(c, c.mode, conv_tile(c.mode, c.tile), src[i].first, src[i].second);
  }
  for (size_t i = 0; i < ups_.size(); ++i) {
    auto& u = ups_[i];
    if (is_split_mode(u.mode)) {
      const ConvTile t = conv_tile(u.mode, u.tile);
      u.n_chunks = ceil_div(u.Cin, t.CK);
      const size_t o = arena.alloc(packed_conv_numel(u.mode, u.U * u.Cout, u.Cin, 2, t), &u.w);
      u.w_exp = pack_convT_split(u.mode, usrc[i].first, u.Cin, u.Cout, u.U, t, arena.at(o));
      std::vector<float> bias((size_t)u.U * u.Cout);
      for (int co = 0; co < u.Cout; ++co)
        for (int ph = 0; ph < u.U; ++ph) bias[(size_t)co * u.U + ph] = usrc[i].second[co];
      arena.put_bias(bias.data(), u.U * u.Cout, t, &u.b);
    } else {
      const ConvTile t = convT_tile(u.tile, u.U);
      u.n_chunks = ceil_div(u.Cin, t.CK);
      const size_t o = arena.alloc(packed_convT_numel(u.Cin, u.Cout, u.U, t), &u.w);
      pack_convT(usrc[i].first, u.Cin, u.Cout, u.U, t, arena.at(o));
      arena.put_bias(usrc[i].second, u.Cout, t, &u.b);
    }
  }
  arena.put(post_w, (size_t)(C0 >> cfg_.num_upsamples) * 7, &post_wd_);
  if (cfg_.cond_channels > 0) {
    arena.put(hw[wi], (size_t)C0 * cfg_.cond_channels, &cond_wd_);
    arena.put(hw[wi + 1], C0, &cond_bd_);
    wi += 2;
  }
  if (cfg_.cond_in_each_up_layer) {
    up_cond_.resize(cfg_.num_upsamples);
    for (int i = 0; i < cfg_.num_upsamples; ++i) {
      const size_t ci = C0 >> (i + 1);
      arena.put(hw[wi], ci * cfg_.cond_channels, &up_cond_[i].first);
      arena.put(hw[wi + 1], ci, &up_cond_[i].second);
      wi += 2;
    }
  }
  arena.upload(device_, arena_);
  hop_ = 1;
  for (int i = 0; i < cfg_.num_upsamples; ++i) hop_ *= cfg_.upsample_factors[i];
}

Hifigan::~Hifigan() {
  DeviceGuard g(device_);
  for (Lane& ln : lanes_) {
    for (hipStream_t st : ln.branch) (void)hipStreamDestroy(st);
    if (ln.own) (void)hipStreamDestroy(ln.own);
    for (hipEvent_t e : ln.ev_z) (void)hipEventDestroy(e);
    if (ln.ev_ups) (void)hipEventDestroy(ln.ev_ups);
    if (ln.ev_done) (void)hipEventDestroy(ln.ev_done);
  }
  if (ev_start_) (void)hipEventDestroy(ev_start_);
}

int64_t Hifigan::out_len(int T, int pad) const { return (int64_t)hop_ * (T + 2 * pad); }

int64_t Hifigan::plane_floats(int B, int T, int pad) const {
  const int64_t L = T + 2 * pad;
  int64_t best = (int64_t)cfg_.upsample_initial_channel * L;
  int64_t len = L;
  for (int i = 0; i < cfg_.num_upsamples; ++i) {
    len *= cfg_.upsample_factors[i];
    const int64_t c = (int64_t)(cfg_.upsample_initial_channel >> (i + 1)) * len;
    if (c > best) best = c;
  }
  return ((best * B + 63) / 64) * 64;
}

int Hifigan::n_planes(int nbs) const { return 2 + 2 * nbs; }

int Hifigan::split_nbs() const { return nbs_env_ ? nbs_ : 1; }

void Hifigan::ensure_lanes() {
  if (!lanes_.empty()) return;
  auto stream = [] {
    hipStream_t st;
    TTS_HIP_CHECK(hipStreamCreateWithFlags(&st, hipStreamNonBlocking));
    return st;
  };
  auto event = [] {
    hipEvent_t e;
    TTS_HIP_CHECK(hipEventCreateWithFlags(&e, hipEventDisableTiming));
    return e;
  };
  lanes_.resize(n_lanes_);
  for (int i = 0; i < n_lanes_; ++i) {
    Lane& ln = lanes_[i];
    if (i > 0) ln.own = stream();
    for (int j = 1; j < nbs_; ++j) ln.branch.push_back(stream());
    ln.ev_ups = event();
    ln.ev_done = event();
    for (int j = 0; j < cfg_.num_kernels; ++j) ln.ev_z.push_back(event());
  }
  ev_start_ = event();
}

int64_t Hifigan::lane_bytes(int B, int64_t L, int nbs) const {
  const int64_t cond = cond_floats(B);
  const int64_t amax = cfg_.math_mode == MATH_FP32_F16X3 ? (int64_t)amax_groups() * B * 64 : 0;
  return ((n_planes(nbs) * plane_floats(B, (int)L, 0) + cond + amax + 63) / 64 * 64) * (int64_t)sizeof(float);
}

int Hifigan::amax_groups() const { return 2 + cfg_.num_upsamples * (2 + cfg_.num_kernels * 6); }
int Hifigan::stage_group(int i) const { return 2 + i * (2 + cfg_.num_kernels * 6); }

int64_t Hifigan::cond_floats(int B) const {
  if (cfg_.cond_channels <= 0) return 0;
  int64_t n = (((int64_t)B * cfg_.upsample_initial_channel + 63) / 64) * 64;
  if (cfg_.cond_in_each_up_layer)
    for (int i = 0; i < cfg_.num_upsamples; ++i)
      n += (((int64_t)B * (cfg_.upsample_initial_channel >> (i + 1)) + 63) / 64) * 64;
  return n;
}

int Hifigan::window_halo() const {
  double r = 3.0, rate = 1.0;
  for (int i = 0; i < cfg_.num_upsamples; ++i) {
    r += 1.5 / rate;
    rate *= cfg_.upsample_factors[i];
    int widest = 0;
    for (int j = 0; j < cfg_.num_kernels; ++j) {
      const int h = (cfg_.resblock_kernel_sizes[j] - 1) / 2;
      int w = 0;
      for (int m = 0; m < (cfg_.resblock_type == 1 ? 3 : 2); ++m)
        w += h * cfg_.resblock_dilation_sizes[j][m] + (cfg_.resblock_type == 1 ? h : 0);
      widest = std::max(widest, w);
    }
    r += widest / rate;
  }
  r += 3.0 / rate;
  return (int)std::ceil(r) + 2;
}

int64_t Hifigan::max_window_frames() const {
  int64_t cr = cfg_.upsample_initial_channel, rate = 1;
  for (int i = 0; i < cfg_.num_upsamples; ++i) {
    rate *= cfg_.upsample_factors[i];
    cr = std::max(cr, (int64_t)(cfg_.upsample_initial_channel >> (i + 1)) * rate);
  }
  return ((int64_t(1) << 29) - 1) / cr;
}

int64_t Hifigan::window_payload() const {
  const char* e = std::getenv("TTS_MI355X_WINDOW_FRAMES");
  const int64_t cap = max_window_frames() - 2 * window_halo();
  if (e && std::atoll(e) > 0) return std::min<int64_t>(std::atoll(e), cap);
  return cap;
}

bool Hifigan::windowed(int64_t L) const {
  const char* e = std::getenv("TTS_MI355X_WINDOW_FRAMES");
  return L > max_window_frames() || (e && std::atoll(e) > 0 && L > std::atoll(e));
}

int64_t Hifigan::plain_workspace_bytes(int B, int64_t L, bool window) const {
  const int nl = std::min(n_lanes_, B);
  if (window || nl == 1) return lane_bytes(B, L, nbs_);
  int64_t lanes = 0;
  for (int i = 0; i < nl; ++i) lanes += lane_bytes(lane_batch(B, i), L, split_nbs());
  return std::max(lane_bytes(B, L, 1), lanes);
}

int64_t Hifigan::window_buffer_bytes(int B, int64_t W) const {
  return ((((int64_t)B * cfg_.in_channels * W + 63) / 64) * 64 + (int64_t)B * hop_ * W) * (int64_t)sizeof(float);
}

int64_t Hifigan::workspace_bytes(int B, int T, int pad) const {
  const int64_t L = (int64_t)T + 2 * pad;
  if (!windowed(L)) return plain_workspace_bytes(B, L, false);
  const int64_t W = std::min<int64_t>(L, window_payload() + 2 * window_halo());
  return plain_workspace_bytes(B, W, true) + window_buffer_bytes(B, W);
}

void Hifigan::reserve_plain(int B, int64_t L, bool window) {
  const int64_t need = plain_workspace_bytes(B, L, window);
  ws_.grow(device_, (size_t)need, "workspace");
}

void Hifigan::reserve(int B, int T, int pad) {
  const int64_t L = (int64_t)T + 2 * pad;
  if (!windowed(L)) {
    reserve_plain(B, L);
    return;
  }
  const int64_t W = std::min<int64_t>(L, window_payload() + 2 * window_halo());
  reserve_plain(B, W, true);
  win_.grow(device_, (size_t)window_buffer_bytes(B, W), "window buffers");
}

void Hifigan::forward(const float* mel, int B, int C, int T, int pad, const float* gvec, float* wav,
                      hipStream_t s, Profiler* prof) {
  TTS_REQUIRE(mel && wav, 1, "NULL input/output pointer");
  TTS_REQUIRE(B >= 1, 1, "batch must be >= 1");
  TTS_REQUIRE(C == cfg_.in_channels, 1,
              "mel has " + std::to_string(C) + " channels, generator expects " + std::to_string(cfg_.in_channels));
  TTS_REQUIRE(T >= 1, 1, "T must be >= 1");
  TTS_REQUIRE(pad >= 0, 1, "pad must be >= 0");
  TTS_REQUIRE(cfg_.cond_channels == 0 || gvec != nullptr, 1, "cond_channels > 0 requires g");
  const int64_t L = (int64_t)T + 2 * pad;
  if (!windowed(L)) {
    DeviceGuard dg(device_);
    reserve_plain(B, L);
    if (prof) {
      forward_plain(mel, B, C, T, pad, gvec, wav, s, prof, ws_.as<>(), nullptr);
      return;
    }
    ensure_lanes();
    const int nl = std::min(n_lanes_, B);
    for (Lane& ln : lanes_) ln.nbs = nl > 1 ? split_nbs() : nbs_;
    if (nl == 1) {
      forward_plain(mel, B, C, T, pad, gvec, wav, s, nullptr, ws_.as<>(), &lanes_[0]);
      return;
    }
    TTS_HIP_CHECK(hipEventRecord(ev_start_, s));
    float* ws = ws_.as<>();
    int b0 = 0;
    for (int i = 0; i < nl; ++i) {
      const int Bi = lane_batch(B, i);
      Lane& ln = lanes_[i];
      const hipStream_t si = i == 0 ? s : ln.own;
      if (i > 0) TTS_HIP_CHECK(hipStreamWaitEvent(si, ev_start_, 0));
      forward_plain(mel + (int64_t)b0 * C * T, Bi, C, T, pad,
                    gvec ? gvec + (int64_t)b0 * cfg_.cond_channels : nullptr, wav + (int64_t)b0 * out_len(T, pad), si,
                    nullptr, ws, &ln);
      if (i > 0) {
        TTS_HIP_CHECK(hipEventRecord(ln.ev_done, si));
        TTS_HIP_CHECK(hipStreamWaitEvent(s, ln.ev_done, 0));
      }
      ws += lane_bytes(Bi, L, ln.nbs) / (int64_t)sizeof(float);
      b0 += Bi;
    }
    return;
  }
  DeviceGuard dg(device_);
  reserve(B, T, pad);
  const int h = window_halo();
  const int64_t P = window_payload();
  TTS_REQUIRE(P >= 1, 3, "window payload must be >= 1 frame");
  const int64_t Wmax = std::min<int64_t>(L, P + 2 * h);
  float* melw = win_.as<>();
  float* outw = melw + (((int64_t)B * C * Wmax + 63) / 64) * 64;
  for (int64_t s0 = 0; s0 < L; s0 += P) {
    const int64_t s1 = std::min(L, s0 + P);
    const int64_t w0 = std::max<int64_t>(0, s0 - h), w1 = std::min(L, s1 + h);
    const int W = (int)(w1 - w0);
    run(prof, s, "mel_window", 0.0, 8.0 * B * C * (double)W,
        [&] { launch_mel_window(mel, B, C, T, pad, w0, W, melw, s); });
    if (!prof) {
      ensure_lanes();
      lanes_[0].nbs = nbs_;
    }
    forward_plain(melw, B, C, W, 0, gvec, outw, s, prof, ws_.as<>(), prof ? nullptr : &lanes_[0]);
    TTS_HIP_CHECK(hipMemcpy2DAsync(wav + hop_ * s0, sizeof(float) * hop_ * L, outw + hop_ * (s0 - w0),
                                   sizeof(float) * hop_ * W, sizeof(float) * hop_ * (s1 - s0), B,
                                   hipMemcpyDeviceToDevice, s));
  }
}

void Hifigan::forward_plain(const float* mel, int B, int C, int T, int pad, const float* gvec, float* wav,
                            hipStream_t s, Profiler* prof, float* ws, Lane* lane) {
  DeviceGuard g(device_);

  const int64_t plane = plane_floats(B, T, pad);
  float* bufZ = ws;
  float* bufO = ws + plane;
  const int np = n_planes(lane ? lane->nbs : 1);
  float* cvec = cfg_.cond_channels > 0 ? ws + np * plane : nullptr;
  const bool h3 = cfg_.math_mode == MATH_FP32_F16X3;
  unsigned* amax = h3 ? reinterpret_cast<unsigned*>(ws + np * plane + cond_floats(B)) : nullptr;
  const int nbs = lane ? lane->nbs : 1;
  const bool conc = nbs > 1;
  const int K = cfg_.num_kernels;
  auto bstream = [&](int j) { return std::max(0, j - (K - nbs)); };
  auto slots = [&](int grp) -> unsigned* { return amax ? amax + (size_t)grp * B * 64 : nullptr; };
  if (h3) TTS_HIP_CHECK(hipMemsetAsync(amax, 0, (size_t)amax_groups() * B * 64 * sizeof(unsigned), s));

  const int L = T + 2 * pad;
  const int C0 = cfg_.upsample_initial_channel;
  bool post_done = false;
  if (cvec) {
    run(prof, s, "cond_layer", 2.0 * B * C0 * cfg_.cond_channels, 4.0 * (B * cfg_.cond_channels + C0 * cfg_.cond_channels + B * C0),
        [&] { launch_cond_vec(gvec, cond_wd_, cond_bd_, cvec, B, cfg_.cond_channels, C0, s); });
  }

  auto conv = [&](const ConvLayer& Ld, const float* x, int Tin, int Tout, int rep, float in_slope,
                  float out_slope, const float* res, float* y, int zmode, const float* cv,
                  const unsigned* amax_in = nullptr, unsigned* amax_out = nullptr, hipStream_t st = nullptr) {
    if (!st) st = s;
    Conv1dArgs a{};
    a.amax_in = amax_in; a.amax_out = amax_out; a.w_exp = Ld.w_exp;
    a.x = x; a.w = Ld.w; a.bias = Ld.b; a.res = res; a.y = y; a.z = bufZ; a.cvec = cv;
    a.Cin = Ld.Cin; a.Cout = Ld.Cout; a.Tin = Tin; a.Tout = Tout;
    a.dil = Ld.dil; a.pad = Ld.pad; a.rep_pad = rep; a.n_chunks = Ld.n_chunks;
    a.in_slope = in_slope; a.out_slope = out_slope; a.zmode = zmode; a.zdiv = (float)cfg_.num_kernels;
    a.planes = planes16_ ? (x == mel ? kPlaneYB16 : kPlaneXB16 | kPlaneYB16) : 0;
    const double ex = (planes16_ && x != mel) ? 2.0 : 4.0, ey = planes16_ ? 2.0 : 4.0;
    const double flops = 2.0 * B * Ld.Cout * (double)Ld.Cin * Ld.K * Tout;
    double bytes = ex * B * Ld.Cin * Tin + 4.0 * Ld.Cout * Ld.Cin * Ld.K + ey * B * Ld.Cout * Tout;
    if (res) bytes += ey * B * Ld.Cout * (double)Tout;
    if (zmode >= 2) bytes += ey * B * Ld.Cout * (double)Tout;
    run(prof, st, Ld.name.c_str(), flops, bytes, [&] { launch_conv(Ld.mode, a, B, Ld.K, Ld.tile, st); });
  };

  if (h3)
    run(prof, s, "amax_mel", 0.0, 4.0 * B * C * (double)T,
        [&] { launch_amax(mel, (int64_t)C * T, B, slots(0), s); });
  conv(pre_, mel, T, L, pad, 1.f, 1.f, nullptr, bufZ, 0, cvec, slots(0), slots(1));

  int len = L;
  const float* cur = bufZ;
  float* upvec = cvec ? cvec + (((int64_t)B * C0 + 63) / 64) * 64 : nullptr;
  for (int i = 0; i < cfg_.num_upsamples; ++i) {
    const ConvTLayer& U = ups_[i];
    const int g0 = stage_group(i);
    const float* ucv = nullptr;
    if (cfg_.cond_in_each_up_layer) {
      const int ci = U.Cout;
      run(prof, s, "cond_up", 2.0 * B * ci * cfg_.cond_channels, 4.0 * (B * cfg_.cond_channels + ci * cfg_.cond_channels + B * ci),
          [&] { launch_cond_vec(gvec, up_cond_[i].first, up_cond_[i].second, upvec, B, cfg_.cond_channels, ci, s); });
      ucv = upvec;
      upvec += (((int64_t)B * ci + 63) / 64) * 64;
    }
    const unsigned* z_amax = slots(i == 0 ? 1 : stage_group(i - 1) + 1 + cfg_.num_kernels * 6);
    const int lout = len * U.U;
    const double uflops = 2.0 * B * U.Cout * (double)U.Cin * 2 * lout;
    const double es = planes16_ ? 2.0 : 4.0;
    const double ubytes = es * ((double)B * U.Cin * len + (double)B * U.Cout * lout) + 4.0 * U.Cin * U.Cout * 2 * U.U;
    if (is_split_mode(U.mode)) {
      Conv1dArgs a{};
      a.planes = planes16_ ? kPlaneXB16 | kPlaneYB16 : 0;
      a.x = cur; a.w = U.w; a.bias = U.b; a.y = bufO;
      a.Cin = U.Cin; a.Cout = U.U * U.Cout; a.Tin = len; a.Tout = len + 1;
      a.dil = 1; a.pad = 1; a.n_chunks = U.n_chunks;
      a.in_slope = 0.1f; a.out_slope = 1.f; a.zdiv = 1.f;
      a.amax_in = z_amax; a.amax_out = slots(g0); a.w_exp = U.w_exp; a.ups = U.U;
      a.cvec = ucv;
      run(prof, s, U.name.c_str(), uflops, ubytes, [&] { launch_conv(U.mode, a, B, 2, U.tile, s); });
    } else {
      ConvTArgs ta{};
      ta.x = cur; ta.w = U.w; ta.bias = U.b; ta.y = bufO;
      ta.Cin = U.Cin; ta.Cout = U.Cout; ta.Tin = len; ta.n_chunks = U.n_chunks; ta.in_slope = 0.1f;
      ta.cvec = ucv;
      run(prof, s, U.name.c_str(), uflops, ubytes, [&] { launch_convT(ta, B, U.U, U.tile, s); });
    }
    len = lout;
    if (conc) TTS_HIP_CHECK(hipEventRecord(lane->ev_ups, s));
    for (int j = 0; j < K; ++j) {
      const ResBlock& rb = res_[i * K + j];
      const int bj = conc ? bstream(j) : 0;
      const hipStream_t sj = bj > 0 ? lane->branch[bj - 1] : s;
      float* bufX = ws + (2 + 2 * bj) * plane;
      float* bufT = bufX + plane;
      if (bj > 0) TTS_HIP_CHECK(hipStreamWaitEvent(sj, lane->ev_ups, 0));
      auto zorder = [&] {
        if (bj > 0 && bstream(j - 1) != bj) TTS_HIP_CHECK(hipStreamWaitEvent(sj, lane->ev_z[j - 1], 0));
      };
      auto zdone = [&] {
        if (conc) TTS_HIP_CHECK(hipEventRecord(lane->ev_z[j], sj));
      };
      const int zlast = (cfg_.num_kernels == 1 || j == 0) ? 1 : (j == cfg_.num_kernels - 1 ? 3 : 2);
      const int gj = g0 + 1 + j * 6;
      const int gz = g0 + 1 + cfg_.num_kernels * 6;
      if (cfg_.resblock_type == 1 && rb.fused3) {
        ResBlock3Args ra{};
        ra.x = bufO; ra.amax_in = slots(g0);
        ra.planes = planes16_ ? kPlaneXB16 | kPlaneYB16 : 0;
        for (int c = 0; c < 6; ++c) { ra.w[c] = rb.convs[c].w; ra.bias[c] = rb.convs[c].b; ra.w_exp[c] = rb.convs[c].w_exp; }
        for (int m = 0; m < 3; ++m) ra.dil[m] = rb.convs[2 * m].dil;
        ra.z = bufZ; ra.zmode = zlast; ra.zdiv = (float)cfg_.num_kernels;
        ra.amax_out = j == cfg_.num_kernels - 1 ? slots(gz) : nullptr;
        ra.T = len;
        const ConvLayer& L1 = rb.convs[0];
        const double flops = 12.0 * B * L1.Cout * (double)L1.Cin * L1.K * len;
        const double bytes = (planes16_ ? 2.0 : 4.0) * B * L1.Cout * len * (zlast >= 2 ? 3 : 2) +
                             4.0 * 6.0 * L1.Cout * L1.Cin * L1.K;
        const std::string nm = "mrf_block_k" + std::to_string(L1.K) + "_c" + std::to_string(L1.Cout);
        zorder();
        run(prof, sj, nm.c_str(), flops, bytes, [&] { launch_resblock3(L1.mode, ra, B, L1.Cout, L1.K, sj); });
        zdone();
      } else if (cfg_.resblock_type == 1 && rb.fused) {
        for (int m = 0; m < 3; ++m) {
          const ConvLayer& L1 = rb.convs[2 * m];
          const ConvLayer& L2 = rb.convs[2 * m + 1];
          const float* xin = (m == 0) ? bufO : (m == 1 ? bufX : bufT);
          float* xout = (m == 1) ? bufT : bufX;
          const bool last = (m == 2);
          ResPairArgs pa{};
          Conv1dArgs& c1 = pa.c1;
          c1.x = xin; c1.w = L1.w; c1.bias = L1.b; c1.Cin = L1.Cin; c1.Cout = L1.Cout; c1.Tin = len; c1.Tout = len;
          c1.dil = L1.dil; c1.pad = L1.pad; c1.n_chunks = L1.n_chunks; c1.in_slope = 0.1f; c1.out_slope = 0.1f;
          c1.zdiv = 1.f; c1.w_exp = L1.w_exp;
          c1.planes = planes16_ ? kPlaneXB16 | kPlaneYB16 : 0;
          c1.amax_in = (m == 0) ? slots(g0) : slots(gj + 2 * m - 1);
          Conv1dArgs& c2 = pa.c2;
          c2.x = nullptr; c2.w = L2.w; c2.bias = L2.b; c2.res = xin; c2.y = xout; c2.z = bufZ;
          c2.Cin = L2.Cin; c2.Cout = L2.Cout; c2.Tin = len; c2.Tout = len; c2.dil = 1; c2.pad = L2.pad;
          c2.n_chunks = L2.n_chunks; c2.in_slope = 1.f; c2.out_slope = 1.f; c2.zmode = last ? zlast : 0;
          c2.zdiv = (float)cfg_.num_kernels; c2.w_exp = L2.w_exp;
          c2.planes = c1.planes;
          c2.amax_out = last ? (j == cfg_.num_kernels - 1 ? slots(gz) : nullptr) : slots(gj + 2 * m + 1);
          const bool post = last && zlast == 3 && i == cfg_.num_upsamples - 1 && post_fusion_ &&
                            cfg_.out_channels == 1;
          if (post) {
            pa.post_w = post_wd_; pa.post_bias = post_bias_; pa.post_slope = 0.01f; pa.wav = wav;
            c2.amax_out = nullptr;
            post_done = true;
          }
          double flops = 4.0 * B * L1.Cout * (double)L1.Cin * L1.K * len;
          const double es = planes16_ ? 2.0 : 4.0;
          double bytes = es * B * L1.Cout * len * (last ? (zlast >= 2 ? 4 : 3) : 3) + 4.0 * 2.0 * L1.Cout * L1.Cin * L1.K;
          if (post) {
            flops += 2.0 * B * len * (double)L1.Cout * 7;
            bytes += 4.0 * B * len - es * B * L1.Cout * len;
          }
          const std::string nm = std::string(post ? "mrf_pair_post_k" : "mrf_pair_k") + std::to_string(L1.K) +
                                 "_c" + std::to_string(L1.Cout);
          if (last) zorder();
          run(prof, sj, nm.c_str(), flops, bytes, [&] { launch_resblock_pair(L1.mode, pa, B, L1.K, L1.Cout, sj); });
          if (last) zdone();
        }
      } else if (cfg_.resblock_type == 1) {
        for (int m = 0; m < 3; ++m) {
          const float* xin = (m == 0) ? bufO : bufX;
          const unsigned* xin_amax = (m == 0) ? slots(g0) : slots(gj + 2 * m - 1);
          const bool last = (m == 2);
          conv(rb.convs[2 * m], xin, len, len, 0, 0.1f, 0.1f, nullptr, bufT, 0, nullptr, xin_amax, slots(gj + 2 * m),
               sj);
          if (last) zorder();
          conv(rb.convs[2 * m + 1], bufT, len, len, 0, 1.f, 1.f, xin, bufX, last ? zlast : 0, nullptr,
               slots(gj + 2 * m), last ? (j == cfg_.num_kernels - 1 ? slots(gz) : nullptr) : slots(gj + 2 * m + 1), sj);
          if (last) zdone();
        }
      } else if (rb.fused2) {
        ResBlock3Args ra{};
        ra.x = bufO; ra.amax_in = slots(g0);
        ra.planes = planes16_ ? kPlaneXB16 | kPlaneYB16 : 0;
        for (int c = 0; c < 2; ++c) {
          ra.w[c] = rb.convs[c].w; ra.bias[c] = rb.convs[c].b; ra.w_exp[c] = rb.convs[c].w_exp;
          ra.dil[c] = rb.convs[c].dil;
        }
        ra.z = bufZ; ra.zmode = zlast; ra.zdiv = (float)cfg_.num_kernels;
        ra.amax_out = j == cfg_.num_kernels - 1 ? slots(gz) : nullptr;
        ra.T = len;
        const ConvLayer& L1 = rb.convs[0];
        const double flops = 4.0 * B * L1.Cout * (double)L1.Cin * L1.K * len;
        const double bytes = (planes16_ ? 2.0 : 4.0) * B * L1.Cout * len * (zlast >= 2 ? 3 : 2) +
                             4.0 * 2.0 * L1.Cout * L1.Cin * L1.K;
        const std::string nm = "mrf_block2_k" + std::to_string(L1.K) + "_c" + std::to_string(L1.Cout);
        zorder();
        run(prof, sj, nm.c_str(), flops, bytes,
            [&] { launch_resblock2(L1.mode, ra, B, L1.Cout, L1.K, rb2_geo64_, sj); });
        zdone();
      } else {
        for (int m = 0; m < 2; ++m) {
          const float* xin = (m == 0) ? bufO : bufX;
          const unsigned* xin_amax = (m == 0) ? slots(g0) : slots(gj + m - 1);
          const bool last = (m == 1);
          if (last) zorder();
          conv(rb.convs[m], xin, len, len, 0, 0.1f, 1.f, xin, bufX, last ? zlast : 0, nullptr, xin_amax,
               last ? (j == cfg_.num_kernels - 1 ? slots(gz) : nullptr) : slots(gj + m), sj);
          if (last) zdone();
        }
      }
    }
    if (conc && bstream(K - 1) > 0) TTS_HIP_CHECK(hipStreamWaitEvent(s, lane->ev_z[K - 1], 0));
    cur = bufZ;
  }
  if (post_done) return;
  PostArgs pa{};
  pa.z = bufZ; pa.w = post_wd_; pa.bias = post_bias_; pa.y = wav;
  pa.Cin = C0 >> cfg_.num_upsamples; pa.T = len; pa.in_slope = 0.01f;
  pa.z_b16 = planes16_ ? 1 : 0;
  run(prof, s, "conv_post", 2.0 * B * len * (double)pa.Cin * 7,
      (planes16_ ? 2.0 : 4.0) * B * pa.Cin * len + 4.0 * B * len, [&] { launch_conv_post(pa, B, s); });
}

}
```

### tts-3_amd/csrc/hifigan.hpp

```cpp
#pragma once

#include <string>
#include <vector>

#include "arena.hpp"
#include "common.hpp"
#include "tts_mi355x.h"

namespace tts {

struct Profiler {
  struct Rec {
    std::string name;
    double flops, bytes;
    hipEvent_t a, b;
  };
  std::vector<Rec> recs;
  ~Profiler() {
    for (auto& r : recs) {
      (void)hipEventDestroy(r.a);
      (void)hipEventDestroy(r.b);
    }
  }
};

template <class F>
void run(Profiler* p, hipStream_t s, const char* name, double flops, double bytes, F&& launch) {
  if (!p) {
    launch();
    return;
  }
  Profiler::Rec r{name, flops, bytes, nullptr, nullptr};
  TTS_HIP_CHECK(hipEventCreate(&r.a));
  TTS_HIP_CHECK(hipEventCreate(&r.b));
  TTS_HIP_CHECK(hipEventRecord(r.a, s));
  launch();
  TTS_HIP_CHECK(hipEventRecord(r.b, s));
  p->recs.push_back(r);
}

std::vector<int64_t> hifigan_weight_shapes(const TtsHifiganCfg& c);
void hifigan_validate(const TtsHifiganCfg& c);

class Hifigan {
 public:
  Hifigan(const TtsHifiganCfg& cfg, const float* const* host_weights, int device);
  ~Hifigan();
  Hifigan(const Hifigan&) = delete;
  Hifigan& operator=(const Hifigan&) = delete;

  int64_t out_len(int T, int pad) const;
  int64_t workspace_bytes(int B, int T, int pad) const;
  void reserve(int B, int T, int pad);
  void forward(const float* mel, int B, int C, int T, int pad, const float* g, float* wav,
               hipStream_t s, Profiler* prof);
  int device() const { return device_; }
  int window_halo() const;
  int64_t max_window_frames() const;
  int64_t window_payload() const;

 private:
  struct ConvLayer : PackedConv {
    int mode = 0;
    std::string name;
  };
  struct ConvTLayer : PackedConv {
    int U = 0;
    int mode = 0;
    std::string name;
  };
  struct ResBlock {
    std::vector<ConvLayer> convs;
    bool fused = false;
    bool fused3 = false;
    bool fused2 = false;
  };

  struct Lane {
    hipStream_t own = nullptr;
    std::vector<hipStream_t> branch;
    hipEvent_t ev_ups = nullptr, ev_done = nullptr;
    std::vector<hipEvent_t> ev_z;
    int nbs = 1;
  };
  void forward_plain(const float* mel, int B, int C, int T, int pad, const float* g, float* wav, hipStream_t s,
                     Profiler* prof, float* ws, Lane* lane);
  void ensure_lanes();
  int64_t lane_bytes(int B, int64_t L, int nbs) const;
  int lane_batch(int B, int i) const { return B / n_lanes_ + (i < B % n_lanes_ ? 1 : 0); }
  bool windowed(int64_t L) const;
  int64_t plain_workspace_bytes(int B, int64_t L, bool window) const;
  int64_t window_buffer_bytes(int B, int64_t W) const;
  void reserve_plain(int B, int64_t L, bool window = false);
  int64_t plane_floats(int B, int T, int pad) const;
  int64_t cond_floats(int B) const;
  int amax_groups() const;
  int stage_group(int i) const;
  int n_planes(int nbs) const;
  int split_nbs() const;

  TtsHifiganCfg cfg_;
  int device_;
  int hop_ = 1;
  int rb2_geo64_ = 0;
  bool post_fusion_ = true;
  bool planes16_ = false;
  int nbs_ = 1;
  int n_lanes_ = 2;
  bool nbs_env_ = false;
  std::vector<Lane> lanes_;
  hipEvent_t ev_start_ = nullptr;
  ConvLayer pre_;
  std::vector<ConvTLayer> ups_;
  std::vector<ResBlock> res_;
  float post_bias_ = 0.f;
  float* post_wd_ = nullptr;
  float* cond_wd_ = nullptr;
  float* cond_bd_ = nullptr;
  std::vector<std::pair<float*, float*>> up_cond_;
  DeviceBuffer arena_, ws_;
  DeviceBuffer win_;
};

}
```

### tts-3_amd/csrc/kernels_conv_wino.hip

```cpp
#include <cmath>
#include <cstdlib>
#include <vector>

#include "wino8_kernel.hpp"

namespace tts {

bool wino_supported(int mode, int Cout, int Cin, int K, int dil) {
  bool m = mode == MATH_FP32_F16X3;
  if (mode == MATH_BF16) {
    const char* e = std::getenv("TTS_MI355X_WINO_BF16");
    m = !(e && e[0] == '0');
  }
  return m && Cout % 128 == 0 && Cin % 16 == 0 && (K == 3 || K == 7 || K == 11) && (dil == 1 || dil == 3 || dil == 5);
}

bool wino_enabled() {
  const char* e = std::getenv("TTS_MI355X_WINO");
  return !(e && e[0] == '0');
}


void launch_wino(int mode, const Conv1dArgs& a, int B, int K, hipStream_t s) {
  TTS_REQUIRE(wino_supported(mode, a.Cout, a.Cin, K, a.dil), 3, "conv1d(winograd): unsupported configuration");
  TTS_REQUIRE((int64_t)a.Cin * a.Tin * 4 < (int64_t(1) << 31) && (int64_t)a.Cout * a.Tout * 4 < (int64_t(1) << 31), 3,
              "conv1d: a batch item's channel plane exceeds 2 GiB");
  TTS_REQUIRE(a.planes == 0 || (mode == MATH_BF16 && a.Tin % 8 == 0), 3,
              "conv1d(winograd): bf16 planes need the bf16 scheme and T % 8 == 0");
  if (mode == MATH_BF16) {
    if (a.Tin % 4 == 0) wino8_detail::launch_s<SchemeB1>(a, B, K, s);
    else wino_detail::launch_wino_s<SchemeB1>(a, B, K, s);
  } else {
    if (a.Tin % 4 == 0) wino8_detail::launch_s<SchemeH3>(a, B, K, s);
    else wino_detail::launch_wino_s<SchemeH3>(a, B, K, s);
  }
  TTS_HIP_CHECK(hipGetLastError());
}

}
```

### tts-3_amd/csrc/split_device.hpp

```cpp
#pragma once

#include "conv_device.hpp"

namespace tts {

typedef __bf16 bf16x8 __attribute__((ext_vector_type(8)));
typedef _Float16 f16x8 __attribute__((ext_vector_type(8)));
typedef unsigned short u16x4 __attribute__((ext_vector_type(4)));
typedef unsigned u32x2 __attribute__((ext_vector_type(2)));

__device__ __forceinline__ unsigned short bf16_bits(__bf16 h) { return __builtin_bit_cast(unsigned short, h); }
__device__ __forceinline__ unsigned short f16_bits(_Float16 h) { return __builtin_bit_cast(unsigned short, h); }

struct SchemeX6 {
  static constexpr int NP = 3;
  static constexpr int ROWB = 112;
  static constexpr int NACC = 1;
  static constexpr int NPROD = 6;
  static constexpr int PA[6] = {2, 1, 0, 1, 0, 0};
  static constexpr int PB[6] = {0, 1, 2, 0, 1, 0};
  static constexpr int PACC[6] = {0, 0, 0, 0, 0, 0};
  static constexpr bool SCALED = false;
  __device__ static __forceinline__ void split(float x, unsigned short (&p)[3]) {
    const __bf16 a0 = (__bf16)x;
    const float r1 = x - (float)a0;
    const __bf16 a1 = (__bf16)r1;
    const float r2 = r1 - (float)a1;
    p[0] = bf16_bits(a0);
    p[1] = bf16_bits(a1);
    p[2] = bf16_bits((__bf16)r2);
  }
  __device__ static __forceinline__ void split2(float x0, float x1, unsigned (&w)[3]) {
    unsigned short a[3], b[3];
    split(x0, a);
    split(x1, b);
#pragma unroll
    for (int p = 0; p < 3; ++p) w[p] = (unsigned)a[p] | ((unsigned)b[p] << 16);
  }
  __device__ static __forceinline__ f32x16 mfma(f32x4 a, f32x4 b, f32x16 c) {
    return __builtin_amdgcn_mfma_f32_32x32x16_bf16(__builtin_bit_cast(bf16x8, a), __builtin_bit_cast(bf16x8, b), c, 0, 0, 0);
  }
};

struct SchemeH3 {
  static constexpr int NP = 2;
  static constexpr int ROWB = 80;
  static constexpr int NACC = 1;
  static constexpr int NPROD = 3;
  static constexpr int PA[3] = {1, 0, 0};
  static constexpr int PB[3] = {0, 1, 0};
  static constexpr int PACC[3] = {0, 0, 0};
  static constexpr bool SCALED = true;
  __device__ static __forceinline__ void split(float x, unsigned short (&p)[2]) {
    const _Float16 h = (_Float16)x;
    p[0] = f16_bits(h);
    p[1] = f16_bits((_Float16)(x - (float)h));
  }
  __device__ static __forceinline__ void split2(float x0, float x1, unsigned (&w)[2]) {
    typedef float f2 __attribute__((ext_vector_type(2)));
    typedef _Float16 h2 __attribute__((ext_vector_type(2)));
    const h2 h = __builtin_convertvector((f2){x0, x1}, h2);
    const unsigned hb = __builtin_bit_cast(unsigned, h);
    float r0, r1;
    asm("v_fma_mix_f32 %0, -%1, 1.0, %2 op_sel_hi:[1,0,0]" : "=v"(r0) : "v"(hb), "v"(x0));
    asm("v_fma_mix_f32 %0, -%1, 1.0, %2 op_sel:[1,0,0] op_sel_hi:[1,0,0]" : "=v"(r1) : "v"(hb), "v"(x1));
    w[0] = hb;
    w[1] = __builtin_bit_cast(unsigned, __builtin_convertvector((f2){r0, r1}, h2));
  }
  __device__ static __forceinline__ f32x16 mfma(f32x4 a, f32x4 b, f32x16 c) {
    return __builtin_amdgcn_mfma_f32_32x32x16_f16(__builtin_bit_cast(f16x8, a), __builtin_bit_cast(f16x8, b), c, 0, 0, 0);
  }
};

struct SchemeB1 {
  static constexpr int NP = 1;
  static constexpr int ROWB = 48;
  static constexpr int NACC = 1;
  static constexpr int NPROD = 1;
  static constexpr int PA[1] = {0};
  static constexpr int PB[1] = {0};
  static constexpr int PACC[1] = {0};
  static constexpr bool SCALED = false;
  __device__ static __forceinline__ void split(float x, unsigned short (&p)[1]) { p[0] = bf16_bits((__bf16)x); }
  __device__ static __forceinline__ void split2(float x0, float x1, unsigned (&w)[1]) {
    w[0] = (unsigned)bf16_bits((__bf16)x0) | ((unsigned)bf16_bits((__bf16)x1) << 16);
  }
  __device__ static __forceinline__ f32x16 mfma(f32x4 a, f32x4 b, f32x16 c) {
    return __builtin_amdgcn_mfma_f32_32x32x16_bf16(__builtin_bit_cast(bf16x8, a), __builtin_bit_cast(bf16x8, b), c, 0, 0, 0);
  }
};

template <class S>
__device__ __forceinline__ void split_store4(unsigned char* dst, float v0, float v1, float v2, float v3) {
  unsigned w0[S::NP], w1[S::NP];
  S::split2(v0, v1, w0);
  S::split2(v2, v3, w1);
#pragma unroll
  for (int p = 0; p < S::NP; ++p) *reinterpret_cast<u32x2*>(dst + 32 * p) = u32x2{w0[p], w1[p]};
}

template <class S, class V>
__device__ __forceinline__ void store_xt8(unsigned char* dst, const V& acc, int r0, float scale) {
  unsigned w[4][S::NP];
#pragma unroll
  for (int k = 0; k < 4; ++k) S::split2(acc[r0 + 2 * k] * scale, acc[r0 + 2 * k + 1] * scale, w[k]);
#pragma unroll
  for (int p = 0; p < S::NP; ++p)
    *reinterpret_cast<u32x4_t*>(dst + 32 * p) = u32x4_t{w[0][p], w[1][p], w[2][p], w[3][p]};
}

__device__ __forceinline__ int amax_exp(const unsigned* slots, int b) {
  if (!slots) return 0;
  float m = __uint_as_float(slots[(size_t)b * 64 + (threadIdx.x & 63)]);
  m = wave_max(m);
  int e = 0;
  if (m > 0.f && m < INFINITY) {
    int E;
    (void)frexpf(m, &E);
    e = E - 14;
  }
  return __builtin_amdgcn_readfirstlane(e);
}

}
```

### tts-3_amd/csrc/wino8_kernel.hpp

```cpp
#pragma once

#include <type_traits>

#include "wino_kernel.hpp"

namespace tts {

__device__ __forceinline__ void lds_sync() { asm volatile("s_waitcnt lgkmcnt(0)\n\ts_barrier" ::: "memory"); }

#ifndef WINO_STAMPS
#define WINO_STAMPS 0
#endif
#define WSTAMP(i)                                                                                            \
  do {                                                                                                       \
    if (WINO_STAMPS && (threadIdx.x & 63) == 0) {                                                            \
      const size_t wg = blockIdx.x + (size_t)gridDim.x * (blockIdx.y + (size_t)gridDim.y * blockIdx.z);      \
      reinterpret_cast<unsigned long long*>(a.z)[(wg * 8 + (threadIdx.x >> 6)) * 32 + (i)] =                   \
          __builtin_amdgcn_s_memtime();                                                                      \
    }                                                                                                        \
  } while (0)

template <class S, int K, int D, bool XB = false>
struct Wino8Cfg {
  static constexpr int ES = XB ? 2 : 4;
  static constexpr int AL = 16 / ES;
  static constexpr int NCH = wino_chunks(K);
  static constexpr int NS = kWinoPoints * NCH;
  static constexpr int PAD = D * (K - 1) / 2;
  static constexpr int BNT = 64;
  static constexpr int J = BNT / D;
  static constexpr int TW = 4 * D * J;
  static constexpr int XROWS = BNT + (NCH - 1) * D;
  static constexpr int PLANE = XROWS * S::ROWB;
  static constexpr int TSZ = kWinoPoints * PLANE;
  static constexpr bool RT_ROFF = XB && TW % 8 != 0;
  static constexpr int ROFF = RT_ROFF ? 7 : (AL - PAD % AL) % AL;
  static constexpr int RSPAN = (XROWS - 1) % D + 4 * D * ((XROWS - 1) / D) + 6 * D + ROFF + 1;
  static constexpr int RSPAN4 = (RSPAN + AL - 1) / AL * AL;
  static constexpr int RPITCH = RSPAN4 % (2 * AL) == AL ? RSPAN4 : RSPAN4 + AL;
  static constexpr int RF4 = (16 * RPITCH / AL + 63) / 64 * 64;
  static constexpr int RSZ = RF4 * 16;
  static constexpr int NDMA = RF4 / 64;
  static constexpr int UNITS = XROWS * 4;
  static constexpr int UPW = (UNITS + 7) / 8;
  static constexpr int PITCH = 256;
  static_assert(UPW <= 64 && UNITS <= 256 + 64 && 3 * NCH >= 3, "one transform round per wave; the DMA spreads over 3 steps");
  static_assert(2 * (UNITS - 256) <= 4 * 64, "spread leftover jobs: one per lane of waves 4-7");
  static_assert(TW <= PITCH, "");
  static constexpr int EPI = 4 * 16 * PITCH * 4 > 8 * 8 * 4 * 64 * 4 ? 4 * 16 * PITCH * 4 : 8 * 8 * 4 * 64 * 4;
  static constexpr int TSM = 2 * TSZ > EPI ? 2 * TSZ : EPI;
};

template <class S, int K, int D, bool LRELU, int PL = 0>
__global__ __launch_bounds__(512) void conv1d_wino8_kernel(Conv1dArgs a) {
  constexpr bool XB = (PL & kPlaneXB16) != 0, YB = (PL & kPlaneYB16) != 0;
  using C = Wino8Cfg<S, K, D, XB>;
  constexpr int NP = S::NP;
  constexpr int NCH = C::NCH;
  constexpr bool H3 = S::SCALED;
  static_assert(PL == 0 || !H3, "bf16 planes: the bf16 scheme only");
#ifndef WINO8_PD
#define WINO8_PD 3
#endif
#ifndef WINO8_EARLY_W
#define WINO8_EARLY_W 0
#endif
#ifndef WINO8_PD1
#define WINO8_PD1 4
#endif
#ifndef WINO8_PD11
#define WINO8_PD11 WINO8_PD
#endif
#ifndef WINO8_PD_B1
#define WINO8_PD_B1 3
#endif
#ifndef WINO8_PD1_B1
#define WINO8_PD1_B1 4
#endif
#ifndef WINO8_GAP7
#define WINO8_GAP7 1
#endif
#ifndef WINO8_GAP11
#define WINO8_GAP11 1
#endif
  __shared__ __attribute__((aligned(16))) unsigned char tsm[C::TSM];
  __shared__ __attribute__((aligned(16))) unsigned char rsm[2 * C::RSZ];
  __shared__ float wbias[128];

  const int tid = threadIdx.x;
  const int lane = tid & 63;
  const int wave = __builtin_amdgcn_readfirstlane(tid >> 6);
  const int wm = wave & 3;
  const int grp = wave >> 2;
  const int half = lane >> 5;
  const int l32 = lane & 31;
  const int bx = blockIdx.x, mt = blockIdx.y, b = blockIdx.z;
  const int t0 = bx * C::TW;
  const int Tin = a.Tin;
  const int Cin = a.Cin;
  const int nc = a.n_chunks;
  const int ex = H3 ? amax_exp(a.amax_in, b) + kWinoBtShift : 0;
  const float xscale = H3 ? ldexpf(1.f, -ex) : 1.f;
  const float slope = a.in_slope;
  const char* xb = static_cast<const char*>(plane_at<XB>(a.x, (size_t)b * (a.x_bstride ? a.x_bstride : (int64_t)Cin * Tin)));
  const unsigned chb = (unsigned)Tin * (unsigned)C::ES;

  const int roff = C::RT_ROFF ? (((t0 - C::PAD) % 8) + 8) % 8 : C::ROFF;
  const int ta = t0 - C::PAD - roff;
#ifndef WINO8_ASM_DMA
#define WINO8_ASM_DMA 1
#endif
  auto dma = [&](int c, int rb, int k0 = 0, int k1 = 64) {
    const int c0 = c * 16;
    const rsrc_t rx = make_rsrc(xb + (size_t)c0 * chb, (unsigned)(Cin - c0) * chb);
    for (int i = wm + 4 * k0; i < C::NDMA && i < wm + 4 * k1; i += 4) {
      const int f = i * 64 + lane;
      constexpr int UPR = C::RPITCH / C::AL;
      const int ch = f / UPR, t = ta + C::AL * (f - ch * UPR);
      const unsigned vo = (ch < 16 && t >= 0 && t < Tin) ? (unsigned)ch * chb + (unsigned)t * (unsigned)C::ES : OOB_OFF;
      if (WINO8_ASM_DMA) {
        lds_dma_b128(xb + (size_t)c0 * chb, (unsigned)(Cin - c0) * chb, vo, rsm + rb * C::RSZ + i * 1024);
      } else {
        __builtin_amdgcn_raw_ptr_buffer_load_lds(
            rx, (__attribute__((address_space(3))) void*)(rsm + rb * C::RSZ + i * 1024), 16, (int)vo, 0, 0, 0);
      }
    }
  };

#ifndef WINO8_DENSE
#define WINO8_DENSE 1
#endif
#ifndef WINO8_SPREAD
#define WINO8_SPREAD 1
#endif
#ifndef WINO8_TG_B1
#define WINO8_TG_B1 0
#endif
  constexpr int TG = S::NP == 1 ? WINO8_TG_B1 : 0;
  const int e = lane * 4 + wm;
  const int u = WINO8_DENSE ? (grp == TG ? wm * 64 + lane
                                         : (WINO8_SPREAD ? 256 + (e >> 1) : (wm == 0 ? 256 + lane : C::UNITS)))
                            : wave * C::UPW + lane;
  const bool uok = (WINO8_DENSE || lane < C::UPW) && u < C::UNITS;
  constexpr bool SPREAD = WINO8_DENSE && WINO8_SPREAD;
  const int jp = e & 1;
  float tkeep[7], jraw[7];
  constexpr int NU = (C::ROFF + 6) / 4 + 1;
  f32x4 jraw4[XB ? 1 : NU];
  u32x2_t jraw8[XB ? NU : 1];
  auto piece = [&](int j) { return SPREAD && grp != TG ? 2 * jp + j : j; };
  const int jrow0 = u >> 2, jq0 = u & 3;
#ifndef WINO8_REMAT
#define WINO8_REMAT 0
#endif
#ifndef WINO8_REMAT11
#define WINO8_REMAT11 1
#endif
  constexpr bool remat = K == 11 ? WINO8_REMAT11 : WINO8_REMAT;
  auto job_unit = [&](int& jrow, int& jq) {
    if (remat && WINO8_DENSE && grp == TG) {
      int ln;
      asm volatile("v_mbcnt_lo_u32_b32 %0, -1, 0\n\tv_mbcnt_hi_u32_b32 %0, -1, %0" : "=v"(ln));
      const int uu = wm * 64 + ln;
      jrow = uu >> 2;
      jq = uu & 3;
    } else {
      jrow = jrow0;
      jq = jq0;
    }
  };
  auto job_load = [&](int rb, int j) {
    if (SPREAD && grp != TG && j >= 2) return;
    if (!uok) return;
    int jrow, jq;
    job_unit(jrow, jq);
    if constexpr (D == 1 && XB) {
      const u32x2_t* raw8 =
          reinterpret_cast<const u32x2_t*>(rsm + rb * C::RSZ) + (4 * jq + piece(j)) * (C::RPITCH / 4) + jrow;
#pragma unroll
      for (int u4 = 0; u4 < NU; ++u4) jraw8[u4] = raw8[u4];
    } else if constexpr (D == 1) {
      const f32x4* raw4 =
          reinterpret_cast<const f32x4*>(rsm + rb * C::RSZ) + (4 * jq + piece(j)) * (C::RPITCH / 4) + jrow;
#pragma unroll
      for (int u4 = 0; u4 < NU; ++u4) jraw4[u4] = raw4[u4];
    } else if constexpr (XB) {
      const int jjj = jrow / D, jrho = jrow - jjj * D;
      const unsigned short* raw = reinterpret_cast<const unsigned short*>(rsm + rb * C::RSZ) +
                                  (4 * jq + piece(j)) * C::RPITCH + jrho + 4 * D * jjj + roff;
#pragma unroll
      for (int k = 0; k < 7; ++k) jraw[k] = bf16_bits_to_f32(raw[D * k]);
    } else {
      const int jjj = jrow / D, jrho = jrow - jjj * D;
      const float* raw = reinterpret_cast<const float*>(rsm + rb * C::RSZ) + (4 * jq + piece(j)) * C::RPITCH +
                         jrho + 4 * D * jjj + C::ROFF;
#pragma unroll
      for (int k = 0; k < 7; ++k) jraw[k] = raw[D * k];
    }
  };
  auto job_finish = [&](int tb, int j) {
    if (SPREAD && grp != TG && j >= 2) return;
    if (!uok) return;
    int jrow, jq;
    job_unit(jrow, jq);
    float v[7], t[7];
#pragma unroll
    for (int k = 0; k < 7; ++k) {
      float x;
      if constexpr (D == 1 && XB) {
        const unsigned w = jraw8[(C::ROFF + k) / 4][((C::ROFF + k) % 4) / 2];
        x = bf16_bits_to_f32((C::ROFF + k) % 2 ? w >> 16 : w & 0xffffu);
      } else {
        x = D == 1 ? jraw4[(C::ROFF + k) / 4][(C::ROFF + k) % 4] : jraw[k];
      }
      if (LRELU) x = lrelu2(x, slope);
      v[k] = H3 ? x * xscale : x;
    }
    wino_bt(v, t);
    if ((j & 1) == 0) {
#pragma unroll
      for (int k = 0; k < 7; ++k) tkeep[k] = t[k];
      return;
    }
    unsigned char* base = tsm + tb * C::TSZ + jrow * S::ROWB + 4 * jq + 16 * (piece(j) >> 1);
#pragma unroll
    for (int p = 0; p < kWinoPoints; ++p) {
      unsigned w[NP];
      split_pair<S>(tkeep[p], t[p], w);
#pragma unroll
      for (int q = 0; q < NP; ++q) *reinterpret_cast<unsigned*>(base + p * C::PLANE + 32 * q) = w[q];
    }
  };

  const int mb = mt * 4 + wm;
  const rsrc_t ra = make_rsrc(a.w + ((size_t)mb * nc * C::NS) * (NP * 256), 0xFFFFFFFFu);
  const unsigned avoff = (unsigned)lane * 16u;

#ifndef WINO8_NOXCH
#define WINO8_NOXCH 0
#endif
  constexpr bool NX = WINO8_NOXCH != 0;
  constexpr int NA = NX ? 7 : 4, NB = NX ? 1 : 2;
  f32x16 acc[NA][NB];
#pragma unroll
  for (int p = 0; p < NA; ++p)
#pragma unroll
    for (int n = 0; n < NB; ++n) acc[p][n] = f32x16{};
  WSTAMP(0);

  float bpre = 0.f;
  if (tid < 128) {
    const int co = mt * 128 + tid;
    if (co < a.Cout) {
      bpre = a.bias[co];
      const float cv = a.cvec ? a.cvec[(size_t)b * (a.cvec_bstride ? a.cvec_bstride : (int64_t)a.Cout) + co] : 0.f;
      bpre = bpre + cv;
    }
  }
  if (grp == 1) {
    dma(0, 0);
    if (nc > 1) dma(1, 1);
  }
  auto prologue = [&](auto wl_tag) {
    constexpr int WL = decltype(wl_tag)::value;
    if (grp == 1) {
      if (nc > 1) asm volatile("s_waitcnt vmcnt(%0)" ::"n"(C::NDMA / 4 + WL) : "memory");
      else asm volatile("s_waitcnt vmcnt(%0)" ::"n"(WL) : "memory");
    }
    WSTAMP(1);
    if (tid < 128) wbias[tid] = bpre;
    lds_sync();
#pragma unroll
    for (int j = 0; j < 4; ++j) {
      job_load(0, j);
      job_finish(0, j);
    }
    if (grp == 1) asm volatile("s_waitcnt vmcnt(0)" ::: "memory");
    lds_sync();
    WSTAMP(2);
  };
  if (!WINO8_EARLY_W) prologue(std::integral_constant<int, 0>{});

  auto run = [&](auto npg_tag, auto p0_tag, auto g1_tag) {
    constexpr int NPG = decltype(npg_tag)::value;
    constexpr int P0 = decltype(p0_tag)::value;
    constexpr bool G1 = decltype(g1_tag)::value;
    constexpr int NV = NPG * NCH;
    constexpr int PD = NP == 1 ? (G1 ? WINO8_PD1_B1 : WINO8_PD_B1)
                               : (G1 ? WINO8_PD1 : (K == 11 ? WINO8_PD11 : WINO8_PD));
    constexpr int GAP0 = K == 11 ? WINO8_GAP11 : WINO8_GAP7;
    constexpr int GAP = GAP0 < NV / 4 ? GAP0 : NV / 4;
    auto aoff = [&](int ck, int v) {
      const int ck2 = ck + v / NV, v2 = v % NV;
      return ck2 < nc ? (unsigned)((ck2 * C::NS + (v2 / NPG) * 7 + P0 + v2 % NPG) * NP) * 1024u : 0u;
    };
    f32x4 ar[PD + 1][NP], bcur[NB][NP], bnext[NB][NP];
#pragma unroll
    for (int v = 0; v < PD; ++v)
#pragma unroll
      for (int q = 0; q < NP; ++q) ar[v][q] = bload4(ra, avoff, aoff(0, v) + (unsigned)q * 1024u);
    if (WINO8_EARLY_W) prologue(std::integral_constant<int, PD * NP>{});
    auto read_b = [&](const unsigned char* tl, int v, f32x4 (*dst)[NP]) {
      const int p = P0 + v % NPG, c = v / NPG;
#pragma unroll
      for (int n = 0; n < NB; ++n) {
        const unsigned char* ptr = tl + p * C::PLANE + ((NX ? grp : n) * 32 + l32 + c * D) * S::ROWB + 16 * half;
#pragma unroll
        for (int q = 0; q < NP; ++q) dst[n][q] = *reinterpret_cast<const f32x4*>(ptr + 32 * q);
      }
    };
    for (int ck = 0; ck < nc; ++ck) {
      const int tb = ck & 1;
      const unsigned char* tl = tsm + tb * C::TSZ;
      const bool more = ck + 1 < nc;
      read_b(tl, 0, bcur);
      if (ck < 8) WSTAMP(3 + 2 * ck);
#pragma unroll
      for (int v = 0; v < NV; ++v) {
#pragma unroll
        for (int q = 0; q < NP; ++q)
          ar[PD][q] = (WINO_ABLATE & 4) ? ar[0][q]
                                        : bload4(ra, avoff, ((WINO_ABLATE & 64) ? 0u : aoff(ck, v + PD)) + (unsigned)q * 1024u);
        if (v + 1 < NV) read_b(tl, v + 1, bnext);
        if ((WINO_ABLATE & 32) == 0 && G1 && ck + 2 < nc && v < 3) dma(ck + 2, tb, 2 * v, v == 2 ? 64 : 2 * v + 2);
        __builtin_amdgcn_sched_barrier(0);
        const int p = v % NPG;
#pragma unroll
        for (int e = 0; e < S::NPROD; ++e)
#pragma unroll
          for (int n = 0; n < NB; ++n) {
            if (WINO_ABLATE & 8) acc[p][n][e] += ar[0][S::PA[e]][0] * bcur[n][S::PB[e]][0];
            else acc[p][n] = S::mfma(ar[0][S::PA[e]], bcur[n][S::PB[e]], acc[p][n]);
          }
#pragma unroll
        for (int pp = 0; pp < PD; ++pp)
#pragma unroll
          for (int q = 0; q < NP; ++q) ar[pp][q] = ar[pp + 1][q];
        if (v + 1 < NV) {
#pragma unroll
          for (int n = 0; n < NB; ++n)
#pragma unroll
            for (int q = 0; q < NP; ++q) bcur[n][q] = bnext[n][q];
        }
#pragma unroll
        for (int j = 0; j < 4; ++j) {
          const int vj = (j * NV) / 4;
          if ((WINO_ABLATE & 2) == 0 && more) {
            if (GAP > 0 && vj + GAP < NV && v == vj + GAP) job_finish(tb ^ 1, j);
            if (v == vj) {
              job_load(tb ^ 1, j);
              if (GAP == 0 || vj + GAP >= NV) job_finish(tb ^ 1, j);
            }
          }
        }
      }
      constexpr int NAFTER = (PD < NV - 3 ? PD : NV - 3) * NP;
      if (G1) asm volatile("s_waitcnt vmcnt(%0)" ::"n"(NAFTER) : "memory");
      if (ck < 8) WSTAMP(4 + 2 * ck);
      lds_sync();
    }
  };
#ifndef WINO8_PRIO
#define WINO8_PRIO 0
#endif
  if (WINO8_PRIO == 1 && grp == 1) __builtin_amdgcn_s_setprio(1);
  if (WINO8_PRIO == 2 && grp == 0) __builtin_amdgcn_s_setprio(1);
  if constexpr (NX) {
    if (grp == 0) run(std::integral_constant<int, 7>{}, std::integral_constant<int, 0>{}, std::false_type{});
    else run(std::integral_constant<int, 7>{}, std::integral_constant<int, 0>{}, std::true_type{});
  } else {
    if (grp == 0) run(std::integral_constant<int, 4>{}, std::integral_constant<int, 0>{}, std::false_type{});
    else run(std::integral_constant<int, 3>{}, std::integral_constant<int, 4>{}, std::true_type{});
  }

#ifndef WINO8_EPI_PF
#define WINO8_EPI_PF 0
#endif
  if constexpr (WINO8_EPI_PF && D == 1) {
    if (a.res || a.zmode >= 2) {
      constexpr unsigned YES = PlaneT<YB>::ES;
      constexpr int LPR = C::TW * (int)YES / 128;
      const unsigned plane = (unsigned)a.Cout * (unsigned)a.Tout * YES;
      const size_t item = (size_t)b * (a.o_bstride ? a.o_bstride : (int64_t)a.Cout * a.Tout);
      const void* pres = a.res ? plane_at<YB>(a.res, item) : nullptr;
      const void* pz = a.zmode >= 2 ? plane_at<YB>(a.z, item) : nullptr;
#pragma unroll
      for (int i = 0; i < (128 * LPR + 511) / 512; ++i) {
        const int l = tid + 512 * i;
        const int co = mt * 128 + l / LPR, ln = l % LPR;
        const int t = t0 + ln * (128 / (int)YES);
        const unsigned vo = (l < 128 * LPR && co < a.Cout && t < a.Tout) ? ((unsigned)co * (unsigned)a.Tout + (unsigned)t) * YES : OOB_OFF;
        if (pres) l2_touch_dma(pres, plane, vo, rsm);
        if (pz) l2_touch_dma(pz, plane, vo, rsm + 256);
      }
    }
  }

  if (WINO_ABLATE & 16) {
    float sum = 0.f;
#pragma unroll
    for (int p = 0; p < NA; ++p)
#pragma unroll
      for (int n = 0; n < NB; ++n)
#pragma unroll
        for (int r = 0; r < 16; ++r) sum += acc[p][n][r];
    if (sum == 1234.5f) a.y[threadIdx.x] = sum;
    return;
  }
  const float sc = H3 ? ldexpf(1.f, ex + a.w_exp) : 1.f;
  const int nk = grp;
  float y[4][16];
  if constexpr (NX) {
#pragma unroll
    for (int r = 0; r < 16; ++r) {
      const float m0 = acc[0][0][r], m1 = acc[1][0][r], m2 = acc[2][0][r], m3 = acc[3][0][r];
      const float m4 = acc[4][0][r], m5 = acc[5][0][r], m6 = acc[6][0][r];
      const float s12 = m1 + m2, d12 = m1 - m2;
      y[0][r] = ((m0 + s12) + m3) + (m4 + m5);
      y[1][r] = fmaf(2.f, m3, d12) + fmaf(-2.f, m4, 0.5f * m5);
      y[2][r] = fmaf(4.f, m3, s12) + fmaf(4.f, m4, 0.25f * m5);
      y[3][r] = fmaf(8.f, m3, d12) + (fmaf(-8.f, m4, 0.125f * m5) + m6);
    }
    WSTAMP(20);
  } else {
  float yp[2][4][16];
#pragma unroll
  for (int n = 0; n < 2; ++n)
#pragma unroll
    for (int r = 0; r < 16; ++r) {
      if (grp == 0) {
        const float m0 = acc[0][n][r], m1 = acc[1][n][r], m2 = acc[2][n][r], m3 = acc[3][n][r];
        const float s12 = m1 + m2, d12 = m1 - m2;
        yp[n][0][r] = (m0 + s12) + m3;
        yp[n][1][r] = fmaf(2.f, m3, d12);
        yp[n][2][r] = fmaf(4.f, m3, s12);
        yp[n][3][r] = fmaf(8.f, m3, d12);
      } else {
        const float m4 = acc[0][n][r], m5 = acc[1][n][r], m6 = acc[2][n][r];
        yp[n][0][r] = m4 + m5;
        yp[n][1][r] = fmaf(-2.f, m4, 0.5f * m5);
        yp[n][2][r] = fmaf(4.f, m4, 0.25f * m5);
        yp[n][3][r] = fmaf(-8.f, m4, 0.125f * m5) + m6;
      }
    }
  WSTAMP(20);
  f32x4* xch = reinterpret_cast<f32x4*>(tsm);
  lds_sync();
#pragma unroll
  for (int h = 0; h < 2; ++h) {
#pragma unroll
    for (int r = 0; r < 8; ++r) {
      f32x4 v;
#pragma unroll
      for (int i = 0; i < 4; ++i) v[i] = grp == 0 ? yp[1][i][8 * h + r] : yp[0][i][8 * h + r];
      xch[((wm * 2 + grp) * 8 + r) * 64 + lane] = v;
    }
    lds_sync();
#pragma unroll
    for (int r = 0; r < 8; ++r) {
      const f32x4 other = xch[((wm * 2 + (1 - grp)) * 8 + r) * 64 + lane];
#pragma unroll
      for (int i = 0; i < 4; ++i) y[i][8 * h + r] = (grp == 0 ? yp[0][i][8 * h + r] : yp[1][i][8 * h + r]) + other[i];
    }
    lds_sync();
  }
  }

  WSTAMP(21);
  const int zm = a.zmode <= 1 ? 0 : a.zmode;
  const int cobase = mt * 128 + wm * 32;
  auto finish = [&](auto res_tag, auto zm_tag) {
    constexpr bool RES = decltype(res_tag)::value;
    constexpr int ZM = decltype(zm_tag)::value;
    const int Cout = a.Cout;
    const int Tout = a.Tout;
    constexpr unsigned YES = PlaneT<YB>::ES;
    const unsigned plane = (unsigned)Cout * (unsigned)Tout * YES;
    const size_t item = (size_t)b * (a.o_bstride ? a.o_bstride : (int64_t)Cout * Tout);
    const rsrc_t rres = make_rsrc(RES ? plane_at<YB>(a.res, item) : a.bias, RES ? plane : 0u);
    const rsrc_t rz = make_rsrc(ZM >= 2 ? plane_at<YB>(a.z, item) : a.bias, ZM >= 2 ? plane : 0u);
    const rsrc_t rout = make_rsrc(plane_at<YB>(a.zmode == 0 ? a.y : a.z, item), plane);
    const float oslope = a.out_slope;
    const float zdiv = a.zdiv;
    float vmax = 0.f;
    if constexpr (D == 1) {
      const int t = t0 + 4 * (nk * 32 + l32);
      const int nvalid = Tout - t < 4 ? (Tout - t > 0 ? Tout - t : 0) : 4;
      const bool full = nvalid == 4 && (Tout & 3) == 0;
      constexpr int GR = (RES && ZM >= 2) ? 8 : 16;
#pragma unroll
      for (int r0 = 0; r0 < 16; r0 += GR) {
        float bias[GR];
        unsigned voff[GR];
        WinoIn gin[GR];
#pragma unroll
        for (int k = 0; k < GR; ++k) {
          const int r = r0 + k;
          const unsigned co = (unsigned)(cobase + (r & 3) + 8 * (r >> 2) + 4 * half);
          bias[k] = wbias[co - (unsigned)(mt * 128)];
          voff[k] = nvalid > 0 ? (co * (unsigned)Tout + (unsigned)t) * YES : OOB_OFF;
          gin[k] = wino_gather<RES, ZM, YB>(rres, rz, voff[k], full, nvalid);
        }
#pragma unroll
        for (int k = 0; k < GR; ++k) {
          const int r = r0 + k;
          const f32x4 yv = {y[0][r], y[1][r], y[2][r], y[3][r]};
          const f32x4 v = wino_apply<RES, ZM, H3>(yv, bias[k], oslope, zdiv, gin[k], nvalid, vmax, sc);
          wino_store<YB>(rout, v, voff[k], full, nvalid);
        }
      }
    } else {
      float* tile = reinterpret_cast<float*>(tsm) + wm * (16 * C::PITCH);
      const int nn = nk * 32 + l32;
      const int jj = nn / D, rho = nn - (nn / D) * D;
      const int tl = 4 * lane;
      const int t = t0 + tl;
      const int lim = (C::TW < Tout - t0 ? C::TW : Tout - t0) - tl;
      const int nvalid = lim < 4 ? (lim > 0 ? lim : 0) : 4;
      const bool full = nvalid == 4 && (Tout & 3) == 0;
#pragma unroll
      for (int ps = 0; ps < 2; ++ps) {
        if (jj < C::J) {
#pragma unroll
          for (int r = 8 * ps; r < 8 * ps + 8; ++r) {
            const int rl = (r & 3) + 8 * ((r >> 2) - 2 * ps) + 4 * half;
#pragma unroll
            for (int i = 0; i < 4; ++i) tile[rl * C::PITCH + rho + D * (4 * jj + i)] = y[i][r];
          }
        }
        lds_sync();
        float bias[8];
        unsigned voff[8];
        WinoIn gin[8];
#pragma unroll
        for (int rr = 0; rr < 8; ++rr) {
          const int co = cobase + 16 * ps + grp * 8 + rr;
          bias[rr] = wbias[co - mt * 128];
          voff[rr] = nvalid > 0 ? ((unsigned)co * (unsigned)Tout + (unsigned)t) * YES : OOB_OFF;
          gin[rr] = wino_gather<RES, ZM, YB>(rres, rz, voff[rr], full, nvalid);
        }
#pragma unroll
        for (int rr = 0; rr < 8; ++rr) {
          const f32x4 yv = *reinterpret_cast<const f32x4*>(tile + (grp * 8 + rr) * C::PITCH + tl);
          const f32x4 v = wino_apply<RES, ZM, H3>(yv, bias[rr], oslope, zdiv, gin[rr], nvalid, vmax, sc);
          wino_store<YB>(rout, v, voff[rr], full, nvalid);
        }
        lds_sync();
      }
    }
    if (H3 && a.amax_out) publish_amax(a.amax_out, b, vmax);
    WSTAMP(22);
  };
  using BT = std::true_type;
  using BF = std::false_type;
  using Z0 = std::integral_constant<int, 0>;
  using Z2 = std::integral_constant<int, 2>;
  using Z3 = std::integral_constant<int, 3>;
  if (a.res) {
    if (zm == 0) finish(BT{}, Z0{});
    else if (zm == 2) finish(BT{}, Z2{});
    else finish(BT{}, Z3{});
  } else {
    if (zm == 0) finish(BF{}, Z0{});
    else if (zm == 2) finish(BF{}, Z2{});
    else finish(BF{}, Z3{});
  }
}

namespace wino8_detail {
template <class S, int K, int D>
void launch_d(const Conv1dArgs& a, int B, hipStream_t s) {
  using C = Wino8Cfg<S, K, D>;
  const dim3 grid(ceil_div(a.Tout, C::TW), ceil_div(a.Cout, 128), B);
  if (a.planes != 0) {
    constexpr bool OK = std::is_same<S, SchemeB1>::value;
    TTS_REQUIRE(OK && a.planes == (kPlaneXB16 | kPlaneYB16) && a.Tin % 8 == 0, 3,
                "conv1d(winograd8): bf16 planes need the bf16 scheme and T % 8 == 0");
    if constexpr (OK) {
      constexpr int PL = kPlaneXB16 | kPlaneYB16;
      if constexpr (D == 1) {
        if (a.in_slope == 1.f) {
          hipLaunchKernelGGL((conv1d_wino8_kernel<S, K, D, false, PL>), grid, dim3(512), 0, s, a);
          return;
        }
      }
      hipLaunchKernelGGL((conv1d_wino8_kernel<S, K, D, true, PL>), grid, dim3(512), 0, s, a);
    }
    return;
  }
  if constexpr (D == 1) {
    if (a.in_slope == 1.f) {
      hipLaunchKernelGGL((conv1d_wino8_kernel<S, K, D, false>), grid, dim3(512), 0, s, a);
      return;
    }
  }
  hipLaunchKernelGGL((conv1d_wino8_kernel<S, K, D, true>), grid, dim3(512), 0, s, a);
}

template <class S, int K>
void launch_k(const Conv1dArgs& a, int B, hipStream_t s) {
  switch (a.dil) {
    case 1: launch_d<S, K, 1>(a, B, s); break;
    case 3: launch_d<S, K, 3>(a, B, s); break;
    case 5: launch_d<S, K, 5>(a, B, s); break;
    default: throw Error(3, "conv1d(winograd8): dilation must be 1, 3 or 5");
  }
}

template <class S>
void launch_s(const Conv1dArgs& a, int B, int K, hipStream_t s) {
  TTS_REQUIRE(a.mask == nullptr && a.ups == 0 && a.gate == 0 && a.rep_pad == 0 && a.Tin == a.Tout &&
                  a.pad == a.dil * (K - 1) / 2 && a.Tin % 4 == 0,
              1, "conv1d(winograd8): unsupported arguments");
  switch (K) {
    case 3: launch_k<S, 3>(a, B, s); break;
    case 7: launch_k<S, 7>(a, B, s); break;
    case 11: launch_k<S, 11>(a, B, s); break;
    default: throw Error(3, "conv1d(winograd8): kernel size must be 3, 7 or 11");
  }
}
}

}
```

Before: 167.3 million samples/s.

## Make Winograd8 conv kernel persistent with cross-tile input prefetch

The Winograd8 conv kernel changes from one workgroup per tile to a persistent grid capped at the CU count. Each workgroup loops over tiles in strided order and prefetches the next tile's input chunks during the current tile's tail, with double-buffered bias storage. The aim is to remove per-workgroup launch and prologue cost and to overlap the next tile's DMA with the current tile's compute. In exchange, the kernel gains loop state and register pressure, and with one workgroup per CU it may lose occupancy and latency hiding.

New measurement: 167.4 million samples/s, median of 6. Within noise of the previous version (+0.1%).

```diff
diff --git a/tts-3_amd/csrc/abi.cpp b/tts-3_amd/csrc/abi.cpp
--- a/tts-3_amd/csrc/abi.cpp
+++ b/tts-3_amd/csrc/abi.cpp
@@ -654,6 +654,7 @@
   a.n_chunks = tts::ceil_div(d->Cin, t.CK);
   a.in_slope = d->in_slope; a.out_slope = d->out_slope; a.zmode = d->zmode; a.zdiv = d->zdiv;
   a.w_exp = w_exp;
+  if (tile == tts::kSplitWinoTile) a.wino_wgs = tts::wino_wgs_cap();
   auto s = static_cast<hipStream_t>(hip_stream);
   tts::DeviceBuffer slots;
   if (mode == tts::MATH_FP32_F16X3) {
diff --git a/tts-3_amd/csrc/common.hpp b/tts-3_amd/csrc/common.hpp
--- a/tts-3_amd/csrc/common.hpp
+++ b/tts-3_amd/csrc/common.hpp
@@ -59,12 +59,15 @@
   int wn_rows;
   int gate;
   int planes;
+  int wino_wgs;
+  int wino_tiles;
 };
 
 constexpr int kSplitGateTile = 20;
 constexpr int kSplitWinoTile = 21;
 bool wino_supported(int mode, int Cout, int Cin, int K, int dil);
 bool wino_enabled();
+int wino_wgs_cap();
 void launch_wino(int mode, const Conv1dArgs& a, int B, int K, hipStream_t s);
 inline int gate_row_order(int rho, int H) {
   const int j = rho / 128, r = rho % 128;
diff --git a/tts-3_amd/csrc/conv_device.hpp b/tts-3_amd/csrc/conv_device.hpp
--- a/tts-3_amd/csrc/conv_device.hpp
+++ b/tts-3_amd/csrc/conv_device.hpp
@@ -136,9 +136,9 @@
   return __builtin_bit_cast(float, __builtin_amdgcn_readlane(__builtin_bit_cast(int, v), 63));
 }
 
-__device__ __forceinline__ void publish_amax(unsigned* slots, int b, float v) {
+__device__ __forceinline__ void publish_amax(unsigned* slots, int b, float v, int lane = (int)(threadIdx.x & 63)) {
   v = wave_max(v);
-  if ((threadIdx.x & 63) == 0) atomicMax(slots + (size_t)b * 64 + (blockIdx.x & 63), __float_as_uint(v));
+  if (lane == 0) atomicMax(slots + (size_t)b * 64 + (blockIdx.x & 63), __float_as_uint(v));
 }
 
 __device__ __forceinline__ void publish_amax_block(unsigned* slots, int b, float v) {
diff --git a/tts-3_amd/csrc/hifigan.cpp b/tts-3_amd/csrc/hifigan.cpp
--- a/tts-3_amd/csrc/hifigan.cpp
+++ b/tts-3_amd/csrc/hifigan.cpp
@@ -105,6 +105,7 @@
   const char* bp = std::getenv("TTS_MI355X_BF16_PLANES");
   planes16_ = mode == MATH_BF16 && !(bp && bp[0] == '0') && cfg_.num_upsamples >= 1 &&
               cfg_.upsample_factors[0] % 8 == 0;
+  wino_wgs_ = wino_wgs_cap();
   size_t wi = 0;
   std::vector<std::pair<const float*, const float*>> src;
   auto add_conv = [&](int Cin, int Cout, int K, int dil, const char* fam, bool res, int lmode, bool pair128 = false) {
@@ -503,6 +504,7 @@
     a.dil = Ld.dil; a.pad = Ld.pad; a.rep_pad = rep; a.n_chunks = Ld.n_chunks;
     a.in_slope = in_slope; a.out_slope = out_slope; a.zmode = zmode; a.zdiv = (float)cfg_.num_kernels;
     a.planes = planes16_ ? (x == mel ? kPlaneYB16 : kPlaneXB16 | kPlaneYB16) : 0;
+    a.wino_wgs = wino_wgs_;
     const double ex = (planes16_ && x != mel) ? 2.0 : 4.0, ey = planes16_ ? 2.0 : 4.0;
     const double flops = 2.0 * B * Ld.Cout * (double)Ld.Cin * Ld.K * Tout;
     double bytes = ex * B * Ld.Cin * Tin + 4.0 * Ld.Cout * Ld.Cin * Ld.K + ey * B * Ld.Cout * Tout;
diff --git a/tts-3_amd/csrc/hifigan.hpp b/tts-3_amd/csrc/hifigan.hpp
--- a/tts-3_amd/csrc/hifigan.hpp
+++ b/tts-3_amd/csrc/hifigan.hpp
@@ -105,6 +105,7 @@
   int rb2_geo64_ = 0;
   bool post_fusion_ = true;
   bool planes16_ = false;
+  int wino_wgs_ = 1;
   int nbs_ = 1;
   int n_lanes_ = 2;
   bool nbs_env_ = false;
diff --git a/tts-3_amd/csrc/kernels_conv_wino.hip b/tts-3_amd/csrc/kernels_conv_wino.hip
--- a/tts-3_amd/csrc/kernels_conv_wino.hip
+++ b/tts-3_amd/csrc/kernels_conv_wino.hip
@@ -1,3 +1,5 @@
+#include <algorithm>
+#include <atomic>
 #include <cmath>
 #include <cstdlib>
 #include <vector>
@@ -20,6 +22,24 @@
   return !(e && e[0] == '0');
 }
 
+int wino_wgs_cap() {
+  if (const char* e = std::getenv("TTS_MI355X_WINO_WGS")) {
+    const long long v = std::atoll(e);
+    if (v >= 1) return (int)std::min<long long>(v, 1 << 30);
+  }
+  constexpr int kMaxDev = 64;
+  static std::atomic<int> cus[kMaxDev];
+  int dev = 0;
+  TTS_HIP_CHECK(hipGetDevice(&dev));
+  TTS_REQUIRE(dev >= 0 && dev < kMaxDev, 3, "conv1d(winograd): device index out of range");
+  int n = cus[dev].load(std::memory_order_relaxed);
+  if (n == 0) {
+    TTS_HIP_CHECK(hipDeviceGetAttribute(&n, hipDeviceAttributeMultiprocessorCount, dev));
+    TTS_REQUIRE(n >= 1, 3, "conv1d(winograd): the device reports no compute units");
+    cus[dev].store(n, std::memory_order_relaxed);
+  }
+  return n;
+}
 
 void launch_wino(int mode, const Conv1dArgs& a, int B, int K, hipStream_t s) {
   TTS_REQUIRE(wino_supported(mode, a.Cout, a.Cin, K, a.dil), 3, "conv1d(winograd): unsupported configuration");
diff --git a/tts-3_amd/csrc/split_device.hpp b/tts-3_amd/csrc/split_device.hpp
--- a/tts-3_amd/csrc/split_device.hpp
+++ b/tts-3_amd/csrc/split_device.hpp
@@ -109,9 +109,7 @@
     *reinterpret_cast<u32x4_t*>(dst + 32 * p) = u32x4_t{w[0][p], w[1][p], w[2][p], w[3][p]};
 }
 
-__device__ __forceinline__ int amax_exp(const unsigned* slots, int b) {
-  if (!slots) return 0;
-  float m = __uint_as_float(slots[(size_t)b * 64 + (threadIdx.x & 63)]);
+__device__ __forceinline__ int amax_exp_of(float m) {
   m = wave_max(m);
   int e = 0;
   if (m > 0.f && m < INFINITY) {
@@ -121,5 +119,9 @@
   }
   return __builtin_amdgcn_readfirstlane(e);
 }
+__device__ __forceinline__ int amax_exp(const unsigned* slots, int b, int lane = (int)(threadIdx.x & 63)) {
+  if (!slots) return 0;
+  return amax_exp_of(__uint_as_float(slots[(size_t)b * 64 + lane]));
+}
 
 }
diff --git a/tts-3_amd/csrc/wino8_kernel.hpp b/tts-3_amd/csrc/wino8_kernel.hpp
--- a/tts-3_amd/csrc/wino8_kernel.hpp
+++ b/tts-3_amd/csrc/wino8_kernel.hpp
@@ -3,6 +3,7 @@
 #include <type_traits>
 
 #include "wino_kernel.hpp"
+#include "wino_tiles.hpp"
 
 namespace tts {
 
@@ -13,9 +14,8 @@
 #endif
 #define WSTAMP(i)                                                                                            \
   do {                                                                                                       \
-    if (WINO_STAMPS && (threadIdx.x & 63) == 0) {                                                            \
-      const size_t wg = blockIdx.x + (size_t)gridDim.x * (blockIdx.y + (size_t)gridDim.y * blockIdx.z);      \
-      reinterpret_cast<unsigned long long*>(a.z)[(wg * 8 + (threadIdx.x >> 6)) * 32 + (i)] =                   \
+    if (WINO_STAMPS && lane == 0) {                                                                          \
+      reinterpret_cast<unsigned long long*>(ka->z)[((size_t)lt * 8 + wave) * 32 + (i)] =                        \
           __builtin_amdgcn_s_memtime();                                                                      \
     }                                                                                                        \
   } while (0)
@@ -52,7 +52,7 @@
 };
 
 template <class S, int K, int D, bool LRELU, int PL = 0>
-__global__ __launch_bounds__(512) void conv1d_wino8_kernel(Conv1dArgs a) {
+__global__ __launch_bounds__(512) void conv1d_wino8_kernel(Conv1dArgs args) {
   constexpr bool XB = (PL & kPlaneXB16) != 0, YB = (PL & kPlaneYB16) != 0;
   using C = Wino8Cfg<S, K, D, XB>;
   constexpr int NP = S::NP;
@@ -62,9 +62,6 @@
 #ifndef WINO8_PD
 #define WINO8_PD 3
 #endif
-#ifndef WINO8_EARLY_W
-#define WINO8_EARLY_W 0
-#endif
 #ifndef WINO8_PD1
 #define WINO8_PD1 4
 #endif
@@ -85,41 +82,64 @@
 #endif
   __shared__ __attribute__((aligned(16))) unsigned char tsm[C::TSM];
   __shared__ __attribute__((aligned(16))) unsigned char rsm[2 * C::RSZ];
-  __shared__ float wbias[128];
-
-  const int tid = threadIdx.x;
-  const int lane = tid & 63;
-  const int wave = __builtin_amdgcn_readfirstlane(tid >> 6);
+  __shared__ float wbias[2][128];
+
+  (void)args;
+  using KArgs = const __attribute__((address_space(4))) Conv1dArgs;
+  using KByte = const __attribute__((address_space(4))) char;
+  KArgs* const ka0 = (KArgs*)__builtin_amdgcn_kernarg_segment_ptr();
+  KArgs* ka = ka0;
+  auto args_setup = [&] {
+    unsigned zero;
+    asm volatile("s_mov_b32 %0, 0" : "=s"(zero));
+    ka = (KArgs*)((KByte*)ka0 + zero);
+  };
+  const int wave = __builtin_amdgcn_readfirstlane((int)threadIdx.x >> 6);
   const int wm = wave & 3;
   const int grp = wave >> 2;
-  const int half = lane >> 5;
-  const int l32 = lane & 31;
-  const int bx = blockIdx.x, mt = blockIdx.y, b = blockIdx.z;
-  const int t0 = bx * C::TW;
-  const int Tin = a.Tin;
-  const int Cin = a.Cin;
-  const int nc = a.n_chunks;
-  const int ex = H3 ? amax_exp(a.amax_in, b) + kWinoBtShift : 0;
-  const float xscale = H3 ? ldexpf(1.f, -ex) : 1.f;
-  const float slope = a.in_slope;
-  const char* xb = static_cast<const char*>(plane_at<XB>(a.x, (size_t)b * (a.x_bstride ? a.x_bstride : (int64_t)Cin * Tin)));
+  int tid = 0, lane = 0, half = 0, l32 = 0;
+  auto lane_setup = [&] {
+    int ln;
+    asm volatile("v_mbcnt_lo_u32_b32 %0, -1, 0\n\tv_mbcnt_hi_u32_b32 %0, -1, %0" : "=v"(ln));
+    lane = ln;
+    tid = wave * 64 + ln;
+    half = ln >> 5;
+    l32 = ln & 31;
+  };
+  const int Tin = ka->Tin;
+  const int Cin = ka->Cin;
+  const int nc = ka->n_chunks;
+  const float slope = ka->in_slope;
   const unsigned chb = (unsigned)Tin * (unsigned)C::ES;
 
-  const int roff = C::RT_ROFF ? (((t0 - C::PAD) % 8) + 8) % 8 : C::ROFF;
-  const int ta = t0 - C::PAD - roff;
+  const int G = (int)gridDim.x, wg = (int)blockIdx.x;
+  const int ntx = (ka->Tout + C::TW - 1) / C::TW, nmt = (ka->Cout + 127) / 128;
+  const int ntl = wino_tiles_of(ka->wino_tiles, G, wg);
+  const bool xpf = nc >= 2 && (nc & 1) == 0;
+  int lt = 0, t0 = 0, mt = 0, b = 0, ex = 0, exn = 0, roff = C::ROFF, ta = 0;
+  float xscale = 1.f;
+  const char* xb = nullptr;
+  auto tile_roff = [&](int t0_) { return C::RT_ROFF ? (((t0_ - C::PAD) % 8) + 8) % 8 : C::ROFF; };
+  auto tile_plane = [&](int b_) {
+    return static_cast<const char*>(plane_at<XB>(ka->x, (size_t)b_ * (ka->x_bstride ? ka->x_bstride : (int64_t)Cin * Tin)));
+  };
+  const char* xbn = nullptr;
+  int tan = 0;
+  bool pfn = false;
+
 #ifndef WINO8_ASM_DMA
 #define WINO8_ASM_DMA 1
 #endif
-  auto dma = [&](int c, int rb, int k0 = 0, int k1 = 64) {
+  auto dma = [&](const char* xbt, int tat, int c, int rb, int k0 = 0, int k1 = 64) {
     const int c0 = c * 16;
-    const rsrc_t rx = make_rsrc(xb + (size_t)c0 * chb, (unsigned)(Cin - c0) * chb);
+    const rsrc_t rx = make_rsrc(xbt + (size_t)c0 * chb, (unsigned)(Cin - c0) * chb);
     for (int i = wm + 4 * k0; i < C::NDMA && i < wm + 4 * k1; i += 4) {
       const int f = i * 64 + lane;
       constexpr int UPR = C::RPITCH / C::AL;
-      const int ch = f / UPR, t = ta + C::AL * (f - ch * UPR);
+      const int ch = f / UPR, t = tat + C::AL * (f - ch * UPR);
       const unsigned vo = (ch < 16 && t >= 0 && t < Tin) ? (unsigned)ch * chb + (unsigned)t * (unsigned)C::ES : OOB_OFF;
       if (WINO8_ASM_DMA) {
-        lds_dma_b128(xb + (size_t)c0 * chb, (unsigned)(Cin - c0) * chb, vo, rsm + rb * C::RSZ + i * 1024);
+        lds_dma_b128(xbt + (size_t)c0 * chb, (unsigned)(Cin - c0) * chb, vo, rsm + rb * C::RSZ + i * 1024);
       } else {
         __builtin_amdgcn_raw_ptr_buffer_load_lds(
             rx, (__attribute__((address_space(3))) void*)(rsm + rb * C::RSZ + i * 1024), 16, (int)vo, 0, 0, 0);
@@ -137,19 +157,26 @@
 #define WINO8_TG_B1 0
 #endif
   constexpr int TG = S::NP == 1 ? WINO8_TG_B1 : 0;
-  const int e = lane * 4 + wm;
-  const int u = WINO8_DENSE ? (grp == TG ? wm * 64 + lane
-                                         : (WINO8_SPREAD ? 256 + (e >> 1) : (wm == 0 ? 256 + lane : C::UNITS)))
-                            : wave * C::UPW + lane;
-  const bool uok = (WINO8_DENSE || lane < C::UPW) && u < C::UNITS;
+  int e = 0, u = 0, jp = 0, jrow0 = 0, jq0 = 0;
+  bool uok = false;
+  unsigned avoff = 0;
   constexpr bool SPREAD = WINO8_DENSE && WINO8_SPREAD;
-  const int jp = e & 1;
+  auto unit_setup = [&] {
+    e = lane * 4 + wm;
+    u = WINO8_DENSE ? (grp == TG ? wm * 64 + lane
+                                 : (WINO8_SPREAD ? 256 + (e >> 1) : (wm == 0 ? 256 + lane : C::UNITS)))
+                    : wave * C::UPW + lane;
+    uok = (WINO8_DENSE || lane < C::UPW) && u < C::UNITS;
+    jp = e & 1;
+    jrow0 = u >> 2;
+    jq0 = u & 3;
+    avoff = (unsigned)lane * 16u;
+  };
   float tkeep[7], jraw[7];
   constexpr int NU = (C::ROFF + 6) / 4 + 1;
   f32x4 jraw4[XB ? 1 : NU];
   u32x2_t jraw8[XB ? NU : 1];
   auto piece = [&](int j) { return SPREAD && grp != TG ? 2 * jp + j : j; };
-  const int jrow0 = u >> 2, jq0 = u & 3;
 #ifndef WINO8_REMAT
 #define WINO8_REMAT 0
 #endif
@@ -232,54 +259,10 @@
     }
   };
 
-  const int mb = mt * 4 + wm;
-  const rsrc_t ra = make_rsrc(a.w + ((size_t)mb * nc * C::NS) * (NP * 256), 0xFFFFFFFFu);
-  const unsigned avoff = (unsigned)lane * 16u;
-
-#ifndef WINO8_NOXCH
-#define WINO8_NOXCH 0
-#endif
-  constexpr bool NX = WINO8_NOXCH != 0;
-  constexpr int NA = NX ? 7 : 4, NB = NX ? 1 : 2;
+  rsrc_t ra = make_rsrc(ka->w, 0xFFFFFFFFu);
+
+  constexpr int NA = 4, NB = 2;
   f32x16 acc[NA][NB];
-#pragma unroll
-  for (int p = 0; p < NA; ++p)
-#pragma unroll
-    for (int n = 0; n < NB; ++n) acc[p][n] = f32x16{};
-  WSTAMP(0);
-
-  float bpre = 0.f;
-  if (tid < 128) {
-    const int co = mt * 128 + tid;
-    if (co < a.Cout) {
-      bpre = a.bias[co];
-      const float cv = a.cvec ? a.cvec[(size_t)b * (a.cvec_bstride ? a.cvec_bstride : (int64_t)a.Cout) + co] : 0.f;
-      bpre = bpre + cv;
-    }
-  }
-  if (grp == 1) {
-    dma(0, 0);
-    if (nc > 1) dma(1, 1);
-  }
-  auto prologue = [&](auto wl_tag) {
-    constexpr int WL = decltype(wl_tag)::value;
-    if (grp == 1) {
-      if (nc > 1) asm volatile("s_waitcnt vmcnt(%0)" ::"n"(C::NDMA / 4 + WL) : "memory");
-      else asm volatile("s_waitcnt vmcnt(%0)" ::"n"(WL) : "memory");
-    }
-    WSTAMP(1);
-    if (tid < 128) wbias[tid] = bpre;
-    lds_sync();
-#pragma unroll
-    for (int j = 0; j < 4; ++j) {
-      job_load(0, j);
-      job_finish(0, j);
-    }
-    if (grp == 1) asm volatile("s_waitcnt vmcnt(0)" ::: "memory");
-    lds_sync();
-    WSTAMP(2);
-  };
-  if (!WINO8_EARLY_W) prologue(std::integral_constant<int, 0>{});
 
   auto run = [&](auto npg_tag, auto p0_tag, auto g1_tag) {
     constexpr int NPG = decltype(npg_tag)::value;
@@ -299,12 +282,11 @@
     for (int v = 0; v < PD; ++v)
 #pragma unroll
       for (int q = 0; q < NP; ++q) ar[v][q] = bload4(ra, avoff, aoff(0, v) + (unsigned)q * 1024u);
-    if (WINO8_EARLY_W) prologue(std::integral_constant<int, PD * NP>{});
     auto read_b = [&](const unsigned char* tl, int v, f32x4 (*dst)[NP]) {
       const int p = P0 + v % NPG, c = v / NPG;
 #pragma unroll
       for (int n = 0; n < NB; ++n) {
-        const unsigned char* ptr = tl + p * C::PLANE + ((NX ? grp : n) * 32 + l32 + c * D) * S::ROWB + 16 * half;
+        const unsigned char* ptr = tl + p * C::PLANE + (n * 32 + l32 + c * D) * S::ROWB + 16 * half;
 #pragma unroll
         for (int q = 0; q < NP; ++q) dst[n][q] = *reinterpret_cast<const f32x4*>(ptr + 32 * q);
       }
@@ -322,7 +304,10 @@
           ar[PD][q] = (WINO_ABLATE & 4) ? ar[0][q]
                                         : bload4(ra, avoff, ((WINO_ABLATE & 64) ? 0u : aoff(ck, v + PD)) + (unsigned)q * 1024u);
         if (v + 1 < NV) read_b(tl, v + 1, bnext);
-        if ((WINO_ABLATE & 32) == 0 && G1 && ck + 2 < nc && v < 3) dma(ck + 2, tb, 2 * v, v == 2 ? 64 : 2 * v + 2);
+        if ((WINO_ABLATE & 32) == 0 && G1 && v < 3) {
+          const bool own = ck + 2 < nc;
+          if (own || pfn) dma(own ? xb : xbn, own ? ta : tan, own ? ck + 2 : ck + 2 - nc, tb, 2 * v, v == 2 ? 64 : 2 * v + 2);
+        }
         __builtin_amdgcn_sched_barrier(0);
         const int p = v % NPG;
 #pragma unroll
@@ -360,218 +345,256 @@
       lds_sync();
     }
   };
-#ifndef WINO8_PRIO
-#define WINO8_PRIO 0
-#endif
-  if (WINO8_PRIO == 1 && grp == 1) __builtin_amdgcn_s_setprio(1);
-  if (WINO8_PRIO == 2 && grp == 0) __builtin_amdgcn_s_setprio(1);
-  if constexpr (NX) {
-    if (grp == 0) run(std::integral_constant<int, 7>{}, std::integral_constant<int, 0>{}, std::false_type{});
-    else run(std::integral_constant<int, 7>{}, std::integral_constant<int, 0>{}, std::true_type{});
-  } else {
+  for (int it = 0; it < ntl; ++it) {
+    args_setup();
+    lane_setup();
+    unit_setup();
+    lt = wino_linear_tile(G, wg, it);
+    {
+      const WinoTile tc = wino_tile_at(lt, ntx, nmt);
+      t0 = tc.bx * C::TW;
+      mt = tc.mt;
+      b = tc.b;
+    }
+    ex = it > 0 ? exn : (H3 ? amax_exp(ka->amax_in, b, lane) + kWinoBtShift : 0);
+    xscale = H3 ? ldexpf(1.f, -ex) : 1.f;
+    xb = tile_plane(b);
+    roff = tile_roff(t0);
+    ta = t0 - C::PAD - roff;
+    ra = make_rsrc(ka->w + ((size_t)(mt * 4 + wm) * nc * C::NS) * (NP * 256), 0xFFFFFFFFu);
+    const bool pre = xpf && it > 0;
+    const bool more_tiles = it + 1 < ntl;
+    pfn = xpf && more_tiles;
+    int bn = 0, mtn = 0;
+    if (more_tiles) {
+      const WinoTile tn = wino_tile_at(lt + G, ntx, nmt);
+      bn = tn.b;
+      mtn = tn.mt;
+      xbn = tile_plane(tn.b);
+      tan = tn.bx * C::TW - C::PAD - tile_roff(tn.bx * C::TW);
+    }
+    float* const wb = wbias[it & 1];
+#pragma unroll
+    for (int p = 0; p < NA; ++p)
+#pragma unroll
+      for (int n = 0; n < NB; ++n) acc[p][n] = f32x16{};
+    WSTAMP(0);
+
+    float bpre = 0.f;
+    if (it == 0 && tid < 128) {
+      const int co = mt * 128 + tid;
+      if (co < ka->Cout) {
+        bpre = ka->bias[co];
+        const float cv = ka->cvec ? ka->cvec[(size_t)b * (ka->cvec_bstride ? ka->cvec_bstride : (int64_t)ka->Cout) + co] : 0.f;
+        bpre = bpre + cv;
+      }
+    }
+    if (grp == 1 && !pre) {
+      dma(xb, ta, 0, 0);
+      if (nc > 1) dma(xb, ta, 1, 1);
+      if (nc > 1) asm volatile("s_waitcnt vmcnt(%0)" ::"n"(C::NDMA / 4) : "memory");
+      else asm volatile("s_waitcnt vmcnt(0)" ::: "memory");
+    }
+    WSTAMP(1);
+    if (it == 0 && tid < 128) wb[tid] = bpre;
+    lds_sync();
+#pragma unroll
+    for (int j = 0; j < 4; ++j) {
+      job_load(0, j);
+      job_finish(0, j);
+    }
+    if (grp == 1 && !pre) asm volatile("s_waitcnt vmcnt(0)" ::: "memory");
+    lds_sync();
+    WSTAMP(2);
+
     if (grp == 0) run(std::integral_constant<int, 4>{}, std::integral_constant<int, 0>{}, std::false_type{});
     else run(std::integral_constant<int, 3>{}, std::integral_constant<int, 4>{}, std::true_type{});
-  }
-
-#ifndef WINO8_EPI_PF
-#define WINO8_EPI_PF 0
-#endif
-  if constexpr (WINO8_EPI_PF && D == 1) {
-    if (a.res || a.zmode >= 2) {
+
+    if (WINO_ABLATE & 16) {
+      float sum = 0.f;
+#pragma unroll
+      for (int p = 0; p < NA; ++p)
+#pragma unroll
+        for (int n = 0; n < NB; ++n)
+#pragma unroll
+          for (int r = 0; r < 16; ++r) sum += acc[p][n][r];
+      if (sum == 1234.5f) ka->y[tid] = sum;
+      continue;
+    }
+    const float sc = H3 ? ldexpf(1.f, ex + ka->w_exp) : 1.f;
+    const int nk = grp;
+    lane_setup();
+    float mnx = 0.f, bnx = 0.f;
+    if (more_tiles) {
+      if (H3 && ka->amax_in) mnx = __uint_as_float(ka->amax_in[(size_t)bn * 64 + lane]);
+      if (tid < 128) {
+        const int co = mtn * 128 + tid;
+        if (co < ka->Cout) {
+          bnx = ka->bias[co];
+          const float cv = ka->cvec ? ka->cvec[(size_t)bn * (ka->cvec_bstride ? ka->cvec_bstride : (int64_t)ka->Cout) + co] : 0.f;
+          bnx = bnx + cv;
+        }
+      }
+    }
+    float y[4][16];
+    float yp[2][4][16];
+#pragma unroll
+    for (int n = 0; n < 2; ++n)
+#pragma unroll
+      for (int r = 0; r < 16; ++r) {
+        if (grp == 0) {
+          const float m0 = acc[0][n][r], m1 = acc[1][n][r], m2 = acc[2][n][r], m3 = acc[3][n][r];
+          const float s12 = m1 + m2, d12 = m1 - m2;
+          yp[n][0][r] = (m0 + s12) + m3;
+          yp[n][1][r] = fmaf(2.f, m3, d12);
+          yp[n][2][r] = fmaf(4.f, m3, s12);
+          yp[n][3][r] = fmaf(8.f, m3, d12);
+        } else {
+          const float m4 = acc[0][n][r], m5 = acc[1][n][r], m6 = acc[2][n][r];
+          yp[n][0][r] = m4 + m5;
+          yp[n][1][r] = fmaf(-2.f, m4, 0.5f * m5);
+          yp[n][2][r] = fmaf(4.f, m4, 0.25f * m5);
+          yp[n][3][r] = fmaf(-8.f, m4, 0.125f * m5) + m6;
+        }
+      }
+    WSTAMP(20);
+    f32x4* xch = reinterpret_cast<f32x4*>(tsm);
+    lds_sync();
+#pragma unroll
+    for (int h = 0; h < 2; ++h) {
+#pragma unroll
+      for (int r = 0; r < 8; ++r) {
+        f32x4 v;
+#pragma unroll
+        for (int i = 0; i < 4; ++i) v[i] = grp == 0 ? yp[1][i][8 * h + r] : yp[0][i][8 * h + r];
+        xch[((wm * 2 + grp) * 8 + r) * 64 + lane] = v;
+      }
+      lds_sync();
+#pragma unroll
+      for (int r = 0; r < 8; ++r) {
+        const f32x4 other = xch[((wm * 2 + (1 - grp)) * 8 + r) * 64 + lane];
+#pragma unroll
+        for (int i = 0; i < 4; ++i) y[i][8 * h + r] = (grp == 0 ? yp[0][i][8 * h + r] : yp[1][i][8 * h + r]) + other[i];
+      }
+      lds_sync();
+    }
+
+    if (more_tiles) {
+      exn = H3 ? (ka->amax_in ? amax_exp_of(mnx) : 0) + kWinoBtShift : 0;
+      if (tid < 128) wbias[(it + 1) & 1][tid] = bnx;
+    }
+    WSTAMP(21);
+    const int zm = ka->zmode <= 1 ? 0 : ka->zmode;
+    const int cobase = mt * 128 + wm * 32;
+    auto finish = [&](auto res_tag, auto zm_tag) {
+      constexpr bool RES = decltype(res_tag)::value;
+      constexpr int ZM = decltype(zm_tag)::value;
+      const int Cout = ka->Cout;
+      const int Tout = ka->Tout;
       constexpr unsigned YES = PlaneT<YB>::ES;
-      constexpr int LPR = C::TW * (int)YES / 128;
-      const unsigned plane = (unsigned)a.Cout * (unsigned)a.Tout * YES;
-      const size_t item = (size_t)b * (a.o_bstride ? a.o_bstride : (int64_t)a.Cout * a.Tout);
-      const void* pres = a.res ? plane_at<YB>(a.res, item) : nullptr;
-      const void* pz = a.zmode >= 2 ? plane_at<YB>(a.z, item) : nullptr;
-#pragma unroll
-      for (int i = 0; i < (128 * LPR + 511) / 512; ++i) {
-        const int l = tid + 512 * i;
-        const int co = mt * 128 + l / LPR, ln = l % LPR;
-        const int t = t0 + ln * (128 / (int)YES);
-        const unsigned vo = (l < 128 * LPR && co < a.Cout && t < a.Tout) ? ((unsigned)co * (unsigned)a.Tout + (unsigned)t) * YES : OOB_OFF;
-        if (pres) l2_touch_dma(pres, plane, vo, rsm);
-        if (pz) l2_touch_dma(pz, plane, vo, rsm + 256);
-      }
-    }
-  }
-
-  if (WINO_ABLATE & 16) {
-    float sum = 0.f;
-#pragma unroll
-    for (int p = 0; p < NA; ++p)
-#pragma unroll
-      for (int n = 0; n < NB; ++n)
-#pragma unroll
-        for (int r = 0; r < 16; ++r) sum += acc[p][n][r];
-    if (sum == 1234.5f) a.y[threadIdx.x] = sum;
-    return;
-  }
-  const float sc = H3 ? ldexpf(1.f, ex + a.w_exp) : 1.f;
-  const int nk = grp;
-  float y[4][16];
-  if constexpr (NX) {
-#pragma unroll
-    for (int r = 0; r < 16; ++r) {
-      const float m0 = acc[0][0][r], m1 = acc[1][0][r], m2 = acc[2][0][r], m3 = acc[3][0][r];
-      const float m4 = acc[4][0][r], m5 = acc[5][0][r], m6 = acc[6][0][r];
-      const float s12 = m1 + m2, d12 = m1 - m2;
-      y[0][r] = ((m0 + s12) + m3) + (m4 + m5);
-      y[1][r] = fmaf(2.f, m3, d12) + fmaf(-2.f, m4, 0.5f * m5);
-      y[2][r] = fmaf(4.f, m3, s12) + fmaf(4.f, m4, 0.25f * m5);
-      y[3][r] = fmaf(8.f, m3, d12) + (fmaf(-8.f, m4, 0.125f * m5) + m6);
-    }
-    WSTAMP(20);
-  } else {
-  float yp[2][4][16];
-#pragma unroll
-  for (int n = 0; n < 2; ++n)
-#pragma unroll
-    for (int r = 0; r < 16; ++r) {
-      if (grp == 0) {
-        const float m0 = acc[0][n][r], m1 = acc[1][n][r], m2 = acc[2][n][r], m3 = acc[3][n][r];
-        const float s12 = m1 + m2, d12 = m1 - m2;
-        yp[n][0][r] = (m0 + s12) + m3;
-        yp[n][1][r] = fmaf(2.f, m3, d12);
-        yp[n][2][r] = fmaf(4.f, m3, s12);
-        yp[n][3][r] = fmaf(8.f, m3, d12);
+      const unsigned plane = (unsigned)Cout * (unsigned)Tout * YES;
+      const size_t item = (size_t)b * (ka->o_bstride ? ka->o_bstride : (int64_t)Cout * Tout);
+      const rsrc_t rres = make_rsrc(RES ? plane_at<YB>(ka->res, item) : ka->bias, RES ? plane : 0u);
+      const rsrc_t rz = make_rsrc(ZM >= 2 ? plane_at<YB>(ka->z, item) : ka->bias, ZM >= 2 ? plane : 0u);
+      const rsrc_t rout = make_rsrc(plane_at<YB>(ka->zmode == 0 ? ka->y : ka->z, item), plane);
+      const float oslope = ka->out_slope;
+      const float zdiv = ka->zdiv;
+      float vmax = 0.f;
+      if constexpr (D == 1) {
+        const int t = t0 + 4 * (nk * 32 + l32);
+        const int nvalid = Tout - t < 4 ? (Tout - t > 0 ? Tout - t : 0) : 4;
+        const bool full = nvalid == 4 && (Tout & 3) == 0;
+        constexpr int GR = (RES && ZM >= 2) ? 8 : 16;
+#pragma unroll
+        for (int r0 = 0; r0 < 16; r0 += GR) {
+          float bias[GR];
+          unsigned voff[GR];
+          WinoIn gin[GR];
+#pragma unroll
+          for (int k = 0; k < GR; ++k) {
+            const int r = r0 + k;
+            const unsigned co = (unsigned)(cobase + (r & 3) + 8 * (r >> 2) + 4 * half);
+            bias[k] = wb[co - (unsigned)(mt * 128)];
+            voff[k] = nvalid > 0 ? (co * (unsigned)Tout + (unsigned)t) * YES : OOB_OFF;
+            gin[k] = wino_gather<RES, ZM, YB>(rres, rz, voff[k], full, nvalid);
+          }
+#pragma unroll
+          for (int k = 0; k < GR; ++k) {
+            const int r = r0 + k;
+            const f32x4 yv = {y[0][r], y[1][r], y[2][r], y[3][r]};
+            const f32x4 v = wino_apply<RES, ZM, H3>(yv, bias[k], oslope, zdiv, gin[k], nvalid, vmax, sc);
+            wino_store<YB>(rout, v, voff[k], full, nvalid);
+          }
+        }
       } else {
-        const float m4 = acc[0][n][r], m5 = acc[1][n][r], m6 = acc[2][n][r];
-        yp[n][0][r] = m4 + m5;
-        yp[n][1][r] = fmaf(-2.f, m4, 0.5f * m5);
-        yp[n][2][r] = fmaf(4.f, m4, 0.25f * m5);
-        yp[n][3][r] = fmaf(-8.f, m4, 0.125f * m5) + m6;
-      }
-    }
-  WSTAMP(20);
-  f32x4* xch = reinterpret_cast<f32x4*>(tsm);
-  lds_sync();
-#pragma unroll
-  for (int h = 0; h < 2; ++h) {
-#pragma unroll
-    for (int r = 0; r < 8; ++r) {
-      f32x4 v;
-#pragma unroll
-      for (int i = 0; i < 4; ++i) v[i] = grp == 0 ? yp[1][i][8 * h + r] : yp[0][i][8 * h + r];
-      xch[((wm * 2 + grp) * 8 + r) * 64 + lane] = v;
-    }
-    lds_sync();
-#pragma unroll
-    for (int r = 0; r < 8; ++r) {
-      const f32x4 other = xch[((wm * 2 + (1 - grp)) * 8 + r) * 64 + lane];
-#pragma unroll
-      for (int i = 0; i < 4; ++i) y[i][8 * h + r] = (grp == 0 ? yp[0][i][8 * h + r] : yp[1][i][8 * h + r]) + other[i];
-    }
-    lds_sync();
-  }
-  }
-
-  WSTAMP(21);
-  const int zm = a.zmode <= 1 ? 0 : a.zmode;
-  const int cobase = mt * 128 + wm * 32;
-  auto finish = [&](auto res_tag, auto zm_tag) {
-    constexpr bool RES = decltype(res_tag)::value;
-    constexpr int ZM = decltype(zm_tag)::value;
-    const int Cout = a.Cout;
-    const int Tout = a.Tout;
-    constexpr unsigned YES = PlaneT<YB>::ES;
-    const unsigned plane = (unsigned)Cout * (unsigned)Tout * YES;
-    const size_t item = (size_t)b * (a.o_bstride ? a.o_bstride : (int64_t)Cout * Tout);
-    const rsrc_t rres = make_rsrc(RES ? plane_at<YB>(a.res, item) : a.bias, RES ? plane : 0u);
-    const rsrc_t rz = make_rsrc(ZM >= 2 ? plane_at<YB>(a.z, item) : a.bias, ZM >= 2 ? plane : 0u);
-    const rsrc_t rout = make_rsrc(plane_at<YB>(a.zmode == 0 ? a.y : a.z, item), plane);
-    const float oslope = a.out_slope;
-    const float zdiv = a.zdiv;
-    float vmax = 0.f;
-    if constexpr (D == 1) {
-      const int t = t0 + 4 * (nk * 32 + l32);
-      const int nvalid = Tout - t < 4 ? (Tout - t > 0 ? Tout - t : 0) : 4;
-      const bool full = nvalid == 4 && (Tout & 3) == 0;
-      constexpr int GR = (RES && ZM >= 2) ? 8 : 16;
-#pragma unroll
-      for (int r0 = 0; r0 < 16; r0 += GR) {
-        float bias[GR];
-        unsigned voff[GR];
-        WinoIn gin[GR];
-#pragma unroll
-        for (int k = 0; k < GR; ++k) {
-          const int r = r0 + k;
-          const unsigned co = (unsigned)(cobase + (r & 3) + 8 * (r >> 2) + 4 * half);
-          bias[k] = wbias[co - (unsigned)(mt * 128)];
-          voff[k] = nvalid > 0 ? (co * (unsigned)Tout + (unsigned)t) * YES : OOB_OFF;
-          gin[k] = wino_gather<RES, ZM, YB>(rres, rz, voff[k], full, nvalid);
-        }
-#pragma unroll
-        for (int k = 0; k < GR; ++k) {
-          const int r = r0 + k;
-          const f32x4 yv = {y[0][r], y[1][r], y[2][r], y[3][r]};
-          const f32x4 v = wino_apply<RES, ZM, H3>(yv, bias[k], oslope, zdiv, gin[k], nvalid, vmax, sc);
-          wino_store<YB>(rout, v, voff[k], full, nvalid);
-        }
-      }
+        float* tile = reinterpret_cast<float*>(tsm) + wm * (16 * C::PITCH);
+        const int nn = nk * 32 + l32;
+        const int jj = nn / D, rho = nn - (nn / D) * D;
+        const int tl = 4 * lane;
+        const int t = t0 + tl;
+        const int lim = (C::TW < Tout - t0 ? C::TW : Tout - t0) - tl;
+        const int nvalid = lim < 4 ? (lim > 0 ? lim : 0) : 4;
+        const bool full = nvalid == 4 && (Tout & 3) == 0;
+#pragma unroll
+        for (int ps = 0; ps < 2; ++ps) {
+          if (jj < C::J) {
+#pragma unroll
+            for (int r = 8 * ps; r < 8 * ps + 8; ++r) {
+              const int rl = (r & 3) + 8 * ((r >> 2) - 2 * ps) + 4 * half;
+#pragma unroll
+              for (int i = 0; i < 4; ++i) tile[rl * C::PITCH + rho + D * (4 * jj + i)] = y[i][r];
+            }
+          }
+          lds_sync();
+          float bias[8];
+          unsigned voff[8];
+          WinoIn gin[8];
+#pragma unroll
+          for (int rr = 0; rr < 8; ++rr) {
+            const int co = cobase + 16 * ps + grp * 8 + rr;
+            bias[rr] = wb[co - mt * 128];
+            voff[rr] = nvalid > 0 ? ((unsigned)co * (unsigned)Tout + (unsigned)t) * YES : OOB_OFF;
+            gin[rr] = wino_gather<RES, ZM, YB>(rres, rz, voff[rr], full, nvalid);
+          }
+#pragma unroll
+          for (int rr = 0; rr < 8; ++rr) {
+            const f32x4 yv = *reinterpret_cast<const f32x4*>(tile + (grp * 8 + rr) * C::PITCH + tl);
+            const f32x4 v = wino_apply<RES, ZM, H3>(yv, bias[rr], oslope, zdiv, gin[rr], nvalid, vmax, sc);
+            wino_store<YB>(rout, v, voff[rr], full, nvalid);
+          }
+          lds_sync();
+        }
+      }
+      if (H3 && ka->amax_out) publish_amax(ka->amax_out, b, vmax, lane);
+      WSTAMP(22);
+    };
+    using BT = std::true_type;
+    using BF = std::false_type;
+    using Z0 = std::integral_constant<int, 0>;
+    using Z2 = std::integral_constant<int, 2>;
+    using Z3 = std::integral_constant<int, 3>;
+    if (ka->res) {
+      if (zm == 0) finish(BT{}, Z0{});
+      else if (zm == 2) finish(BT{}, Z2{});
+      else finish(BT{}, Z3{});
     } else {
-      float* tile = reinterpret_cast<float*>(tsm) + wm * (16 * C::PITCH);
-      const int nn = nk * 32 + l32;
-      const int jj = nn / D, rho = nn - (nn / D) * D;
-      const int tl = 4 * lane;
-      const int t = t0 + tl;
-      const int lim = (C::TW < Tout - t0 ? C::TW : Tout - t0) - tl;
-      const int nvalid = lim < 4 ? (lim > 0 ? lim : 0) : 4;
-      const bool full = nvalid == 4 && (Tout & 3) == 0;
-#pragma unroll
-      for (int ps = 0; ps < 2; ++ps) {
-        if (jj < C::J) {
-#pragma unroll
-          for (int r = 8 * ps; r < 8 * ps + 8; ++r) {
-            const int rl = (r & 3) + 8 * ((r >> 2) - 2 * ps) + 4 * half;
-#pragma unroll
-            for (int i = 0; i < 4; ++i) tile[rl * C::PITCH + rho + D * (4 * jj + i)] = y[i][r];
-          }
-        }
-        lds_sync();
-        float bias[8];
-        unsigned voff[8];
-        WinoIn gin[8];
-#pragma unroll
-        for (int rr = 0; rr < 8; ++rr) {
-          const int co = cobase + 16 * ps + grp * 8 + rr;
-          bias[rr] = wbias[co - mt * 128];
-          voff[rr] = nvalid > 0 ? ((unsigned)co * (unsigned)Tout + (unsigned)t) * YES : OOB_OFF;
-          gin[rr] = wino_gather<RES, ZM, YB>(rres, rz, voff[rr], full, nvalid);
-        }
-#pragma unroll
-        for (int rr = 0; rr < 8; ++rr) {
-          const f32x4 yv = *reinterpret_cast<const f32x4*>(tile + (grp * 8 + rr) * C::PITCH + tl);
-          const f32x4 v = wino_apply<RES, ZM, H3>(yv, bias[rr], oslope, zdiv, gin[rr], nvalid, vmax, sc);
-          wino_store<YB>(rout, v, voff[rr], full, nvalid);
-        }
-        lds_sync();
-      }
-    }
-    if (H3 && a.amax_out) publish_amax(a.amax_out, b, vmax);
-    WSTAMP(22);
-  };
-  using BT = std::true_type;
-  using BF = std::false_type;
-  using Z0 = std::integral_constant<int, 0>;
-  using Z2 = std::integral_constant<int, 2>;
-  using Z3 = std::integral_constant<int, 3>;
-  if (a.res) {
-    if (zm == 0) finish(BT{}, Z0{});
-    else if (zm == 2) finish(BT{}, Z2{});
-    else finish(BT{}, Z3{});
-  } else {
-    if (zm == 0) finish(BF{}, Z0{});
-    else if (zm == 2) finish(BF{}, Z2{});
-    else finish(BF{}, Z3{});
+      if (zm == 0) finish(BF{}, Z0{});
+      else if (zm == 2) finish(BF{}, Z2{});
+      else finish(BF{}, Z3{});
+    }
   }
 }
 
 namespace wino8_detail {
 template <class S, int K, int D>
-void launch_d(const Conv1dArgs& a, int B, hipStream_t s) {
+void launch_d(const Conv1dArgs& args, int B, hipStream_t s) {
   using C = Wino8Cfg<S, K, D>;
-  const dim3 grid(ceil_div(a.Tout, C::TW), ceil_div(a.Cout, 128), B);
+  const int64_t n_tiles = (int64_t)ceil_div(args.Tout, C::TW) * ceil_div(args.Cout, 128) * B;
+  TTS_REQUIRE(n_tiles >= 1 && n_tiles < (int64_t(1) << 31), 3, "conv1d(winograd8): too many tiles");
+  TTS_REQUIRE(args.wino_wgs >= 1, 1, "conv1d(winograd8): Conv1dArgs::wino_wgs (the workgroup cap) is not set");
+  Conv1dArgs a = args;
+  a.wino_tiles = (int)n_tiles;
+  const dim3 grid(wino_grid(a.wino_tiles, a.wino_wgs));
   if (a.planes != 0) {
     constexpr bool OK = std::is_same<S, SchemeB1>::value;
     TTS_REQUIRE(OK && a.planes == (kPlaneXB16 | kPlaneYB16) && a.Tin % 8 == 0, 3,
diff --git a/tts-3_amd/csrc/wino_tiles.hpp b/tts-3_amd/csrc/wino_tiles.hpp
--- /dev/null
+++ b/tts-3_amd/csrc/wino_tiles.hpp
@@ -0,0 +1,28 @@
+#pragma once
+
+#if defined(__HIPCC__)
+#define TTS_WINO_HD __host__ __device__ inline
+#else
+#define TTS_WINO_HD inline
+#endif
+
+namespace tts {
+
+struct WinoTile {
+  int bx;
+  int mt;
+  int b;
+};
+
+TTS_WINO_HD int wino_grid(int n_tiles, int cap) { return cap < 1 ? 1 : (n_tiles < cap ? n_tiles : cap); }
+
+TTS_WINO_HD int wino_tiles_of(int n_tiles, int G, int w) { return w < n_tiles ? (n_tiles - 1 - w) / G + 1 : 0; }
+
+TTS_WINO_HD int wino_linear_tile(int G, int w, int it) { return w + it * G; }
+
+TTS_WINO_HD WinoTile wino_tile_at(int lt, int ntx, int nmt) {
+  const int r = lt / ntx;
+  return WinoTile{lt - r * ntx, r % nmt, r / nmt};
+}
+
+}
diff --git a/tts-3_amd/tests_native/wino_tiles_check.cpp b/tts-3_amd/tests_native/wino_tiles_check.cpp
--- /dev/null
+++ b/tts-3_amd/tests_native/wino_tiles_check.cpp
@@ -0,0 +1,65 @@
+#include <cstdio>
+#include <cstdlib>
+#include <vector>
+
+#include "wino_tiles.hpp"
+
+namespace {
+int fails = 0;
+void fail(const char* what, int ntx, int nmt, int B, int G, int w, int it) {
+  if (++fails <= 20) std::fprintf(stderr, "FAIL %s: ntx %d nmt %d B %d G %d w %d it %d\n", what, ntx, nmt, B, G, w, it);
+}
+
+void check(int ntx, int nmt, int B, int cap) {
+  const int n = ntx * nmt * B;
+  const int G = tts::wino_grid(n, cap);
+  if (G < 1 || G > n || G > (cap < 1 ? 1 : cap)) fail("grid", ntx, nmt, B, G, 0, 0);
+  std::vector<unsigned char> seen((size_t)n, 0);
+  int lo = n, hi = 0;
+  for (int w = 0; w < G; ++w) {
+    const int cnt = tts::wino_tiles_of(n, G, w);
+    lo = cnt < lo ? cnt : lo;
+    hi = cnt > hi ? cnt : hi;
+    for (int it = 0; it < cnt; ++it) {
+      const int lt = tts::wino_linear_tile(G, w, it);
+      if (lt != w + it * G || lt < 0 || lt >= n) {
+        fail("linear tile", ntx, nmt, B, G, w, it);
+        continue;
+      }
+      const tts::WinoTile t = tts::wino_tile_at(lt, ntx, nmt);
+      if (t.bx < 0 || t.bx >= ntx || t.mt < 0 || t.mt >= nmt || t.b < 0 || t.b >= B ||
+          t.bx + ntx * (t.mt + nmt * t.b) != lt)
+        fail("order", ntx, nmt, B, G, w, it);
+      if (seen[(size_t)lt]++) fail("visited twice", ntx, nmt, B, G, w, it);
+    }
+    if ((long long)w + (long long)cnt * G < n) fail("count short", ntx, nmt, B, G, w, cnt);
+  }
+  for (int lt = 0; lt < n; ++lt)
+    if (!seen[(size_t)lt]) fail("never visited", ntx, nmt, B, G, -1, lt);
+  if (hi - lo > 1 || lo < 1) fail("balance", ntx, nmt, B, G, lo, hi);
+}
+}
+
+int main() {
+  long long cases = 0;
+  for (int nmt = 1; nmt <= 3; ++nmt)
+    for (int B = 1; B <= 5; ++B)
+      for (int ntx = 1; ntx * nmt * B <= 2000; ++ntx) {
+        const int step = (nmt == 1 && B == 1) ? 1 : 7;
+        if (ntx % step != 0 && ntx > 3) continue;
+        for (int G = 1; G <= 300; ++G) {
+          check(ntx, nmt, B, G);
+          ++cases;
+        }
+      }
+  check(5, 2, 3, 0);
+  check(5, 2, 3, -4);
+  check(5, 2, 3, 1 << 30);
+  check(1, 1, 1, 1 << 30);
+  if (fails) {
+    std::fprintf(stderr, "%d failures\n", fails);
+    return 1;
+  }
+  std::printf("winograd tile partition OK (%lld cases)\n", cases + 4);
+  return 0;
+}
```
